# Alisah-Ozcan/HEonGPU

Measured on AMD Instinct MI355X. Metric: homomorphic mults/sec (CKKS N=2^16, L=16) + NTT GB/s vs HBM roofline, higher is better.
Workload: dtype u64

## Files before the change

### heongpu_amd/csrc/context.cpp

```cpp
#include "context.hpp"
#include <cerrno>
#include <climits>
#include <cstdlib>
#include "host_params.hpp"
#include <algorithm>
#include <cmath>
#include <cstdlib>
#include <cstring>
#include <stdexcept>

namespace hegpu {

using host::inv_mod_prime;
using host::mul_mod;

typedef std::vector<u64> vec;

static void append(vec& dst, const vec& src) { dst.insert(dst.end(), src.begin(), src.end()); }

void Context::build_host()
{
    n = ((u64) 1) << n_power;
    Qp_size = Q_size + P_size;
    const int Q = Q_size, P = P_size, Qp = Qp_size;
// ... 393 lines not shown
            host["plain_ntt_tables"] = host::power_table_bitrev(ppsi, t, n_power);
            host["plain_intt_tables"] = host::power_table_bitrev(inv_mod_prime(ppsi, t), t, n_power);
            host["n_plain_inverse"] = vec{inv_mod_prime(n % t, t)};
            vec loc;
            const u64 m = 2 * n;
            u64 pos = 1;
            auto brev = [&](u64 v) {
                u64 r = 0;
                for (int b = 0; b < n_power; b++) r |= ((v >> b) & 1) << (n_power - 1 - b);
                return r;
            };
            for (u64 i = 0; i < n / 2; i++) {
                loc.push_back(brev((pos - 1) >> 1));
                pos = (pos * 3) & (m - 1);
            }
            for (u64 i = n / 2; i < n; i++) {
                loc.push_back(brev((m - pos - 1) >> 1));
                pos = (pos * 3) & (m - 1);
            }
            host["encoding_location"] = loc;
        }

        {
            u64 Q_mod_t = 1;
            for (int i = 0; i < Q; i++) Q_mod_t = mul_mod(Q_mod_t, primes[i] % t, t);
            hv.Q_mod_t = Q_mod_t;
            hv.upper_threshold = (t + 1) >> 1;
            host["Q_mod_t"] = vec{hv.Q_mod_t};
            host["upper_threshold"] = vec{hv.upper_threshold};
            vec inc;
            for (int i = 0; i < Q; i++) inc.push_back(primes[i] - t);
            host["upper_halfincrement"] = inc;
            std::vector<u64> big{1};
            for (int i = 0; i < Q; i++) {
                unsigned __int128 carry = 0;
                for (u64& w : big) {
                    unsigned __int128 v = (unsigned __int128) w * primes[i] + carry;
                    w = (u64) v;
                    carry = v >> 64;
                }
                if (carry) big.push_back((u64) carry);
            }
            {
                unsigned __int128 rem = 0;
                for (size_t k = big.size(); k-- > 0;) {
                    unsigned __int128 cur = (rem << 64) | big[k];
                    big[k] = (u64) (cur / t);
                    rem = cur % t;
                }
            }
            vec cdiv;
            for (int i = 0; i < Q; i++) {
                unsigned __int128 rem = 0;
                for (size_t k = big.size(); k-- > 0;) rem = ((rem << 64) | big[k]) % primes[i];
                cdiv.push_back((u64) rem);
            }
            host["coeff_div_plain_modulus"] = cdiv;
            vec Qi_t, Qi_gamma, Qi_inverse;
            for (int i = 0; i < Q; i++) {
                u64 a = 1, b = 1, c = 1;
                for (int j = 0; j < Q; j++)
                    if (j != i) {
                        a = mul_mod(a, primes[j] % t, t);
                        b = mul_mod(b, primes[j] % gamma, gamma);
                        c = mul_mod(c, inv_mod_prime(primes[j] % primes[i], primes[i]), primes[i]);
                    }
                Qi_t.push_back(a);
                Qi_gamma.push_back(b);
                Qi_inverse.push_back(c);
            }
            host["Qi_t"] = Qi_t;
            host["Qi_gamma"] = Qi_gamma;
            host["Qi_inverse"] = Qi_inverse;
            u64 mt_ = 1, mg_ = 1;
            for (int i = 0; i < Q; i++) {
                mt_ = mul_mod(mt_, inv_mod_prime(primes[i] % t, t), t);
                mg_ = mul_mod(mg_, inv_mod_prime(primes[i] % gamma, gamma), gamma);
            }
            hv.mulq_inv_t = t - mt_;
            hv.mulq_inv_gamma = gamma - mg_;
            hv.inv_gamma = inv_mod_prime(gamma % t, t);
            host["mulq_inv_t"] = vec{hv.mulq_inv_t};
            host["mulq_inv_gamma"] = vec{hv.mulq_inv_gamma};
            host["inv_gamma"] = vec{hv.inv_gamma};
        }
    }
}

template <typename T>
static hipError_t to_device(const std::vector<T>& h, T** d)
{
    *d = nullptr;
    if (h.empty()) return hipSuccess;
    hipError_t e = hipMalloc((void**) d, h.size() * sizeof(T));
    if (e != hipSuccess) return e;
    return hipMemcpy(*d, h.data(), h.size() * sizeof(T), hipMemcpyHostToDevice);
}

static hipError_t build_plan(NttPlan& p, const vec& mods, const vec& fwd, const vec& inv, const vec& ninv,
                             int n_power, bool fp_on)
{
    const u64 n = ((u64) 1) << n_power;
    const int cnt = (int) mods.size();
    std::vector<Mod> hm(cnt);
    std::vector<ulonglong2> htw((size_t) cnt * n), hitw((size_t) cnt * n), hn(cnt), hw(cnt);
    const u64 rows = n / 256, perB = rows * 15 * 16;
    std::vector<ulonglong2> htwB((size_t) cnt * perB), hitwB((size_t) cnt * perB);
    std::vector<double> htwB8((size_t) cnt * perB, 0.0);
    for (int k = 0; k < cnt; k++) {
        const u64 q = mods[k];
        hm[k] = make_mod(q);
        static_assert(FP_MAX_MODULUS_BITS == 50, "the bounds in fpmod.cuh, ntt.hip and tests/fp_model.py are derived for q < 2^50");
        hm[k].fp = (fp_on && hm[k].bit <= FP_MAX_MODULUS_BITS && (q >> FP_MAX_MODULUS_BITS) == 0) ? 1 : 0;
        for (u64 j = 0; j < n; j++) {
            const u64 w = fwd[k * n + j], iw = inv[k * n + j];
            if (hm[k].fp) {
                const double wd = (double) w, wi = wd / (double) q;
                u64 a, b;
                memcpy(&a, &wd, 8);
                memcpy(&b, &wi, 8);
                htw[k * n + j] = make_ulonglong2(a, b);
            } else {
                htw[k * n + j] = make_ulonglong2(w, shoup_companion(w, q));
            }
            if (hm[k].fp) {
                const double wd = (double) iw, wi = wd / (double) q;
                u64 a, b;
                memcpy(&a, &wd, 8);
                memcpy(&b, &wi, 8);
                hitw[k * n + j] = make_ulonglong2(a, b);
            } else {
                hitw[k * n + j] = make_ulonglong2(iw, shoup_companion(iw, q));
            }
        }
        for (u64 c = 0; c < rows; c++)
            for (int st = 0; st < 4; st++)
                for (int b = 0; b < (1 << st); b++)
                    for (int j = 0; j < 16; j++) {
                        const u64 src = ((((rows + c) * 16 + j) << st) + b);
                        const u64 dst = k * perB + (c * 15 + ((1 << st) - 1 + b)) * 16 + j;
                        htwB[dst] = htw[k * n + src];
                        hitwB[dst] = hitw[k * n + src];
                        if (hm[k].fp) htwB8[dst] = (double) fwd[k * n + src];
                    }
        const u64 w1n = host::mul_mod(inv[k * n + 1], ninv[k], q);
        if (hm[k].fp) {
            auto pair = [&](u64 v) {
                const double vd = (double) v, vi = vd / (double) q;
                u64 a, b;
                memcpy(&a, &vd, 8);
                memcpy(&b, &vi, 8);
                return make_ulonglong2(a, b);
            };
            hn[k] = pair(ninv[k]);
            hw[k] = pair(w1n);
        } else {
            hn[k] = make_ulonglong2(ninv[k], shoup_companion(ninv[k], q));
            hw[k] = make_ulonglong2(w1n, shoup_companion(w1n, q));
        }
    }
    p.count = cnt;
    p.has_fp = p.has_int = 0;
    for (int k = 0; k < cnt; k++) (hm[k].fp ? p.has_fp : p.has_int) = 1;
    p.fp.assign(cnt, 0);
    for (int k = 0; k < cnt; k++) p.fp[k] = hm[k].fp ? 1 : 0;
    p.bits.assign(cnt, 0);
    for (int k = 0; k < cnt; k++) p.bits[k] = (unsigned char) hm[k].bit;
    u64 qmax = 0;
    for (int k = 0; k < cnt; k++) qmax = mods[k] > qmax ? mods[k] : qmax;
    p.lazy_q_max = (~0ull - 2 * qmax) / (4ull * (u64) n_power);
    hipError_t e;
    if ((e = to_device(hm, &p.mods)) != hipSuccess) return e;
    if ((e = to_device(htw, &p.tw)) != hipSuccess) return e;
    if ((e = to_device(hitw, &p.itw)) != hipSuccess) return e;
    if ((e = to_device(htwB, &p.twB)) != hipSuccess) return e;
    if ((e = to_device(hitwB, &p.itwB)) != hipSuccess) return e;
    if ((e = to_device(htwB8, &p.twB8)) != hipSuccess) return e;
    if ((e = to_device(hn, &p.ninv)) != hipSuccess) return e;
    return to_device(hw, &p.w1ninv);
}

static void free_plan(NttPlan& p)
{
    if (p.mods) (void) hipFree(p.mods);
    if (p.tw) (void) hipFree(p.tw);
    if (p.itw) (void) hipFree(p.itw);
    if (p.twB) (void) hipFree(p.twB);
    if (p.itwB) (void) hipFree(p.itwB);
    if (p.twB8) (void) hipFree(p.twB8);
    if (p.ninv) (void) hipFree(p.ninv);
    if (p.w1ninv) (void) hipFree(p.w1ninv);
    p = NttPlan();
}

hipError_t Context::upload()
{
    if (uploaded) return hipSuccess;
    for (int k = 0; k < DRBG_GAUSS_MAX; k++)
        gauss_cdt.t[k] = (u64) (erf(((double) k + 0.5) / (3.2 * 1.4142135623730951)) * 9223372036854775808.0);
    hipError_t e = hipGetDevice(&device);
    if (e != hipSuccess) return e;
    if ((e = build_plan(plan_qp, host["modulus"], host["ntt_table"], host["intt_table"], host["n_inverse"],
                        n_power, fp_ntt)) != hipSuccess)
        return e;
    const struct { const char* name; const u64** slot; const int** ints; } rows[] = {
        {"psi_half", &tab.psi_half}, {"last_q_modinv", &tab.last_q_modinv}, {"half", &tab.half},
        {"half_mod", &tab.half_mod}, {"factor", &tab.factor},
        {"m2_md_W0", &tab.m2_md_W0}, {"m2_md_G", &tab.m2_md_G}, {"m2_md_C", &tab.m2_md_C},
        {"rescaled_last_q_modinv", &tab.rescaled_last_q_modinv}, {"rescaled_half_mod", &tab.rescaled_half_mod},
        {"rescaled_half", &tab.rescaled_half}, {"mod_raise_half_mod", &tab.mod_raise_half_mod},
        {"base_change_matrix_Bsk", &behz.base_change_matrix_Bsk},
        {"inv_punctured_prod_mod_base_array", &behz.inv_punctured_prod_mod_base_array},
        {"base_change_matrix_m_tilde", &behz.base_change_matrix_m_tilde},
        {"inv_m_tilde_mod_Bsk", &behz.inv_m_tilde_mod_Bsk}, {"prod_q_mod_Bsk", &behz.prod_q_mod_Bsk},
        {"inv_prod_q_mod_Bsk", &behz.inv_prod_q_mod_Bsk}, {"base_change_matrix_q", &behz.base_change_matrix_q},
        {"base_change_matrix_msk", &behz.base_change_matrix_msk},
        {"inv_punctured_prod_mod_B_array", &behz.inv_punctured_prod_mod_B_array},
        {"behz_mtilde_inv_punct", &behz.mtilde_inv_punct}, {"behz_t_inv_punct", &behz.t_inv_punct},
        {"behz_invq_inv_punct_B", &behz.invq_inv_punct_B}, {"behz_msk_mod_q", &behz.msk_mod_q},
        {"behz_fc_matrix", &behz.fc_matrix}, {"behz_fc_c1", &behz.fc_c1}, {"behz_ff_matrix", &behz.ff_matrix},
        {"behz_ff_tc", &behz.ff_tc}, {"behz_ff_q_matrix", &behz.ff_q_matrix},
        {"behz_ff_msk_matrix", &behz.ff_msk_matrix}, {"behz_ff_prod_B", &behz.ff_prod_B},
        {"behz_ff_neg_prod_B", &behz.ff_neg_prod_B}, {"prod_B_mod_q", &behz.prod_B_mod_q},
        {"Mi", &tab.Mi}, {"Mi_inv", &tab.Mi_inv}, {"upper_half_threshold", &tab.upper_half_threshold},
        {"decryption_modulus", &tab.decryption_modulus}, {"special_fft_roots_table", &tab.special_fft_roots_table},
        {"special_ifft_roots_table", &tab.special_ifft_roots_table},
        {"coeff_div_plain_modulus", &tab.coeff_div_plain_modulus}, {"upper_halfincrement", &tab.upper_halfincrement},
        {"Qi_t", &tab.Qi_t}, {"Qi_gamma", &tab.Qi_gamma}, {"Qi_inverse", &tab.Qi_inverse},
        {"m2_Mi_inv", &tab.m2_Mi_inv}, {"m2_matrix", &tab.m2_matrix}, {"m2_prod", &tab.m2_prod},
        {"m2_matrix_mg", &tab.m2_matrix_mg}, {"m2_negprod_mg", &tab.m2_negprod_mg},
        {"new_prime_locations", nullptr, &tab.new_prime_locations},
        {"new_input_locations", nullptr, &tab.new_input_locations}, {"m2_I_j", nullptr, &tab.m2_I_j},
        {"m2_I_location", nullptr, &tab.m2_I_location}, {"encoding_location", nullptr, &tab.encoding_location},
        {"reverse_order", nullptr, &tab.reverse_order}, {"mpc_refresh_order", nullptr, &tab.mpc_refresh_order},
    };
    for (const auto& r : rows) {
        auto it = host.find(r.name);
        if (it == host.end()) continue;
        if (r.slot) {
            u64* d = nullptr;
            if ((e = to_device(it->second, &d)) != hipSuccess) return e;
            dev[r.name] = d;
            *r.slot = d;
        } else {
            std::vector<int> v(it->second.begin(), it->second.end());
            int* d = nullptr;
            if ((e = to_device(v, &d)) != hipSuccess) return e;
            dev[r.name] = d;
            *r.ints = d;
        }
    }
    if (scheme == SCHEME_BFV) {
        if ((e = build_plan(plan_merge, host["q_Bsk_merge_modulus"], host["q_Bsk_merge_ntt_tables"],
                            host["q_Bsk_merge_intt_tables"], host["q_Bsk_n_inverse"], n_power, fp_ntt)) != hipSuccess)
            return e;
        if (host.count("plain_modulus2") &&
            (e = build_plan(plan_plain, host["plain_modulus2"], host["plain_ntt_tables"], host["plain_intt_tables"],
                            host["n_plain_inverse"], n_power, fp_ntt)) != hipSuccess)
            return e;
        behz.ibase = plan_merge.mods;
        behz.obase = plan_merge.mods + Q_size;
        behz.m_tilde = make_mod(((u64) 1) << 32);
        behz.plain = make_mod(plain_modulus);
        behz.inv_prod_q_mod_m_tilde = hv.inv_prod_q_mod_m_tilde;
        behz.inv_prod_B_mod_m_sk = hv.inv_prod_B_mod_m_sk;
        behz.ibase_size = Q_size;
        behz.obase_size = bsk_size;
        behz.split = behz_split;
    }
    uploaded = true;
    return hipDeviceSynchronize();
}

namespace {
struct OptDesc {
    enum Rule { PLAIN, NOT_1_OR_3, BEFORE_UPLOAD, MIRROR_BEHZ };
    const char* name;
    const char* env;
    int lo, hi;
    int ContextHost::*i;
    bool ContextHost::*b;
    Rule rule;
    constexpr OptDesc(const char* nm, const char* ev, int l, int h, int ContextHost::*m, Rule r = PLAIN)
        : name(nm), env(ev), lo(l), hi(h), i(m), b(nullptr), rule(r) {}
    constexpr OptDesc(const char* nm, const char* ev, bool ContextHost::*m, Rule r = PLAIN)
        : name(nm), env(ev), lo(0), hi(1), i(nullptr), b(m), rule(r) {}
};
typedef ContextHost H;
const OptDesc kOptions[] = {
    {"fused_row_mac", "HEGPU_FUSED_ROW_MAC", -1, 1, &H::fused_row_mac},
    {"fused_moddown", "HEGPU_FUSED_MODDOWN", &H::fused_moddown},
    {"col_multi", "HEGPU_COL_MULTI", -1, 1, &H::col_multi},
    {"single_pass", "HEGPU_SINGLE_PASS", -1, 1, &H::single_pass},
    {"ntt_galois", "HEGPU_NTT_GALOIS", &H::ntt_galois},
    {"galois_scatter", "HEGPU_GALOIS_SCATTER", &H::galois_scatter},
    {"fuse_inverse", "HEGPU_FUSE_INVERSE", &H::fuse_inverse},
    {"copy_along", "HEGPU_COPY_ALONG", &H::copy_along},
    {"digit_split", "HEGPU_DIGIT_SPLIT", -1, 4, &H::digit_split, OptDesc::NOT_1_OR_3},
    {"fp_ntt", "HEGPU_FP_NTT", &H::fp_ntt, OptDesc::BEFORE_UPLOAD},
    {"behz_split", "HEGPU_BEHZ_SPLIT", -1, 1, &H::behz_split, OptDesc::MIRROR_BEHZ},
    {"fused_tensor", "HEGPU_FUSED_TENSOR", &H::fused_tensor},
    {"moddown_in_mac", "HEGPU_MODDOWN_IN_MAC", &H::moddown_in_mac},
    {"wide_access", "HEGPU_WIDE_ACCESS", &H::wide_access},
};
const OptDesc* find_option(const char* name)
{
    for (const OptDesc& o : kOptions)
        if (name && !strcmp(o.name, name)) return &o;
    return nullptr;
}
}

int Context::set_option(const char* name, int value)
{
    const OptDesc* d = find_option(name);
    if (!d) return 1;
    if (value < d->lo || value > d->hi || (d->rule == OptDesc::NOT_1_OR_3 && (value == 1 || value == 3))) return 2;
    if (d->rule == OptDesc::BEFORE_UPLOAD && uploaded) return 3;
    if (d->i) this->*d->i = value;
    else this->*d->b = value != 0;
    if (d->rule == OptDesc::MIRROR_BEHZ) behz.split = value;
    return 0;
}

int Context::get_option(const char* name, int* value) const
{
    const OptDesc* d = find_option(name);
    if (!d || !value) return 1;
    *value = d->i ? this->*d->i : (int) (this->*d->b);
    return 0;
}

bool env_long(const char* name, long* out)
{
    const char* e = getenv(name);
    if (!e || !*e) return false;
    char* end = nullptr;
    errno = 0;
    const long v = strtol(e, &end, 10);
    if (errno || end == e || *end) return false;
    *out = v;
    return true;
}

void Context::seed_options_from_env()
{
    for (const OptDesc& o : kOptions) {
        long v;
        if (env_long(o.env, &v) && v >= INT_MIN && v <= INT_MAX)
            (void) set_option(o.name, (int) v);
    }
}

void Context::release_device()
{
    free_plan(plan_qp);
    free_plan(plan_merge);
    free_plan(plan_plain);
    for (auto& kv : dev)
        if (kv.second) (void) hipFree(kv.second);
    dev.clear();
    uploaded = false;
}

Context::~Context()
{
    if (uploaded) release_device();
}

NttArgs Context::ntt_args(int table_set) const
{
    const NttPlan& p = table_set == 2 ? plan_plain : (table_set ? plan_merge : plan_qp);
    NttArgs a{};
    a.mods = p.mods;
    a.tw = p.tw;
    a.itw = p.itw;
    a.twB = p.twB;
    a.itwB = p.itwB;
    a.twB8 = p.twB8;
    a.ninv = p.ninv;
    a.w1ninv = p.w1ninv;
    a.n_power = n_power;
    a.mod_count = p.count;
    a.col_multi = col_multi;
    a.single_pass = single_pass;
    a.plan_has_fp = p.has_fp;
    a.plan_has_int = p.has_int;
    a.lazy_q_max = p.lazy_q_max;
    return a;
}

ModDown Context::moddown(int depth, bool rescale) const
{
    const int l = Q_size - depth;
    if (!rescale)
        return {plan_qp.mods, tab.half, tab.half_mod, tab.last_q_modinv, n_power, Qp_size - depth, l, Qp_size, Q_size,
                P_size};
    const int row = triangle_offset(Q_size - 1, depth);
    return {plan_qp.mods, tab.rescaled_half + depth, tab.rescaled_half_mod + row, tab.rescaled_last_q_modinv + row,
            n_power, l, l - 1, l, l - 1, 1};
}

}
```

### heongpu_amd/csrc/context.hpp

```cpp
#pragma once
#include "modarith.cuh"
#include "ntt.hpp"
#include "rns.hpp"
#include <map>
#include <string>
#include "drbg.hpp"
#include <vector>

namespace hegpu {

bool env_long(const char* name, long* out);


enum Scheme { SCHEME_BFV = 1, SCHEME_CKKS = 2 };

inline int triangle_offset(int first, int depth)
{
    int location = 0;
    for (int i = 0; i < depth; i++) location += first - i;
    return location;
}

struct NttPlan {
    Mod* mods = nullptr;
    ulonglong2* tw = nullptr;
    ulonglong2* itw = nullptr;
    ulonglong2* twB = nullptr;
    ulonglong2* itwB = nullptr;
    double* twB8 = nullptr;
    ulonglong2* ninv = nullptr;
    ulonglong2* w1ninv = nullptr;
    int count = 0;
    int has_fp = 0, has_int = 0;
    std::vector<unsigned char> fp;
    std::vector<unsigned char> bits;
    u64 lazy_q_max = 0;
};

struct DevTables {
    const u64 *psi_half, *last_q_modinv, *half, *half_mod, *factor;
    const u64 *m2_md_W0, *m2_md_G, *m2_md_C, *m2_Mi_inv, *m2_matrix, *m2_prod, *m2_matrix_mg, *m2_negprod_mg;
    const int *m2_I_j, *m2_I_location;
    const u64 *rescaled_last_q_modinv, *rescaled_half_mod, *rescaled_half;
    const u64* mod_raise_half_mod;
    const u64 *Mi, *Mi_inv, *upper_half_threshold, *decryption_modulus, *special_fft_roots_table, *special_ifft_roots_table;
    const int *new_prime_locations, *new_input_locations, *reverse_order, *mpc_refresh_order;
    const u64 *coeff_div_plain_modulus, *upper_halfincrement, *Qi_t, *Qi_gamma, *Qi_inverse;
    const int* encoding_location;
};

struct ContextHost {
    int scheme = 0;
    int n_power = 0;
    u64 n = 0;
    int Q_size = 0, P_size = 0, Qp_size = 0;
    int bsk_size = 0;
    u64 plain_modulus = 0;
    std::vector<u64> primes;
    std::map<std::string, std::vector<u64>> host;
    struct HostVals {
        u64 half = 0;
        std::vector<u64> rescaled_half;
        u64 mod_raise_half = 0;
        std::vector<u64> new_prime_locations;
        u64 Q_mod_t = 0, upper_threshold = 0, gamma = 0, mulq_inv_t = 0, mulq_inv_gamma = 0, inv_gamma = 0;
        u64 inv_prod_q_mod_m_tilde = 0, inv_prod_B_mod_m_sk = 0;
    } hv;
    struct M2Level {
        int d = 0, rc = 0;
        int off_digits = 0;
        int off_mi = 0;
        int off_matrix = 0;
        int off_prod = 0;
    };
    std::vector<M2Level> m2_levels;
    int m2_width = 0;
    int fused_row_mac = -1;
    bool fused_moddown = true;
    int col_multi = -1;
    int single_pass = -1;
    bool ntt_galois = true;
    bool galois_scatter = true;
    int digit_split = -1;
    bool copy_along = true;
    bool fuse_inverse = true;
    bool moddown_in_mac = true;
    bool wide_access = true;
    bool fused_tensor = true;
    bool fp_ntt = true;
    int behz_split = -1;
};

struct Context : ContextHost {
    void seed_options_from_env();
    int set_option(const char* name, int value);
    int get_option(const char* name, int* value) const;
    GaussCdt gauss_cdt{};

    bool uploaded = false;
    int device = -1;
    NttPlan plan_qp;
    NttPlan plan_merge;
    NttPlan plan_plain;
    std::map<std::string, void*> dev;
    DevTables tab{};
    BehzDev behz{};

    ~Context();
    void build_host();
    hipError_t upload();
    void release_device();

    NttArgs ntt_args(int table_set) const;
    ModDown moddown(int depth, bool rescale = false) const;
};

}
```

### heongpu_amd/csrc/ntt.hip

```cpp
#include "ntt.hpp"
#include <atomic>
#define HEGPU_FP_TU ntt
#include "fpmod.cuh"

namespace hegpu {

#define NTT_THREADS 256

#ifdef NTT_ABLATION_HEADER
#include NTT_ABLATION_HEADER
#else
__device__ __forceinline__ u64 gld(const u64* p) { return *p; }
__device__ __forceinline__ void gst(u64* p, u64 v) { *p = v; }
#define NTT_ABLATE_BFLY(x, y, w)
#define NTT_ABLATE_FPBFLY(x, y, w)
#define NTT_ABLATE_TW(load, root0, s) (load)
#define NTT_FP_TW(t, i, c) ((t)[i])
#endif

__device__ __forceinline__ u64 csub(u64 x, u64 m) { return (x >= m) ? x - m : x; }

typedef unsigned long long u64x2_t __attribute__((ext_vector_type(2)));
struct ConstTw {
    const u64x2_t __attribute__((address_space(4)))* p;
// ... 81 lines not shown
    return FpSched{m, b > b_out_max};
}
template <int LOGR, typename TW>
__device__ __forceinline__ void fp_ct_radix(double (&x)[1 << LOGR], TW tw, u32 root0,
                                            const FC& c, unsigned before, bool at_end)
{
#pragma unroll
    for (int s = 0; s < LOGR; s++) {
        FP_STAGE(c, 31 - __builtin_clz(root0) + s);
        if ((before >> s) & 1u) {
#pragma unroll
            for (int k = 0; k < (1 << LOGR); k++) x[k] = fp_reduce(x[k], c);
        }
        const int half = (1 << LOGR) >> (s + 1);
#pragma unroll
        for (int b = 0; b < (1 << s); b++) {
            const ulonglong2 w = NTT_ABLATE_TW(NTT_FP_TW(tw, (root0 << s) + b, c), root0, s);
#pragma unroll
            for (int j = 0; j < half; j++) fp_ct_bfly(x[b * 2 * half + j], x[b * 2 * half + j + half], w, c);
        }
    }
    FP_STAGE(c, 31 - __builtin_clz(root0) + LOGR);
    if (at_end) {
#pragma unroll
        for (int k = 0; k < (1 << LOGR); k++) x[k] = fp_reduce(x[k], c);
    }
}
template <int S1> struct FpColSched {
    static constexpr FpSched s = fp_sched(S1, FP_UNREDUCED_IN, FP_HANDOVER);
    static constexpr unsigned a_before = s.before & ((1u << (S1 - 4)) - 1u);
    static constexpr unsigned b_before = (s.before >> (S1 - 4)) & 15u;
    static constexpr bool b_at_end = s.at_end;
};
__device__ __forceinline__ void fp_ct_radix16_tb(double (&x)[16], const ulonglong2* __restrict__ tb, const FC& c)
{
#pragma unroll
    for (int s = 0; s < 4; s++) {
        const int half = 8 >> s;
        if (s > 0) FP_STAGE(c, (c).stage + 1);
#pragma unroll
        for (int b = 0; b < (1 << s); b++) {
            const ulonglong2 w = NTT_ABLATE_TW(NTT_FP_TW(tb, ((1 << s) - 1 + b) * 16, c), (u32) b, s);
#pragma unroll
            for (int j = 0; j < half; j++) fp_ct_bfly(x[b * 2 * half + j], x[b * 2 * half + j + half], w, c);
        }
    }
    FP_STAGE(c, (c).stage + 1);
#pragma unroll
    for (int k = 0; k < 16; k++) x[k] = fp_canon(x[k], c);
}

__device__ __forceinline__ void fp_ct_radix16_tb8(double (&x)[16], const double* __restrict__ tb, const FC& c)
{
#pragma unroll
    for (int s = 0; s < 4; s++) {
        const int half = 8 >> s;
        if (s > 0) __builtin_amdgcn_sched_barrier(0);
        if (s > 0) FP_STAGE(c, (c).stage + 1);
#pragma unroll
        for (int b = 0; b < (1 << s); b++) {
            const double wd = tb[((1 << s) - 1 + b) * 16];
            const ulonglong2 w = make_ulonglong2(as_bits(wd), as_bits(wd * c.qi));
#pragma unroll
            for (int j = 0; j < half; j++) fp_ct_bfly(x[b * 2 * half + j], x[b * 2 * half + j + half], w, c);
        }
    }
    FP_STAGE(c, (c).stage + 1);
#pragma unroll
    for (int k = 0; k < 16; k++) x[k] = fp_canon(x[k], c);
}

struct QC {
    u64 q;
    u64 q4;
    u32 nq0, nq1;
};
__device__ __forceinline__ QC make_qc(u64 q)
{
    QC c;
    c.q = q;
    c.q4 = 4 * q;
    u64 nq = 0 - q;
    c.nq0 = (u32) nq;
    c.nq1 = (u32) (nq >> 32);
    return c;
}

__device__ __forceinline__ u64 shoup_lazy(u64 y, ulonglong2 w, const QC& c)
{
    const u32 y0 = (u32) y, y1 = (u32) (y >> 32);
    const u32 w0 = (u32) w.x, w1 = (u32) (w.x >> 32), p0 = (u32) w.y, p1 = (u32) (w.y >> 32);
    const u64 A = (u64) y0 * p1;
    const u64 B = (u64) y1 * p0 + (u32) A;
    const u64 qh = (u64) y1 * p1 + (A >> 32) + (B >> 32);
    const u32 h0 = (u32) qh, h1 = (u32) (qh >> 32);
    u64 acc = (u64) y0 * w0;
    acc += (u64) h0 * c.nq0;
    const u32 hi = y0 * w1 + y1 * w0 + h0 * c.nq1 + h1 * c.nq0;
    return acc + ((u64) hi << 32);
}

__device__ __forceinline__ u64 shoup_full(u64 y, ulonglong2 w, const QC& c)
{
    u64 r = shoup_lazy(y, w, c);
    r = csub(r, 2 * c.q);
    return csub(r, c.q);
}

struct CsSched { unsigned c8, c4; };
__host__ __device__ constexpr CsSched cs_sched(int stages, int room, int exit_b = 8)
{
    CsSched r{0u, 0u};
    int b = 8;
    for (int s = 0; s < stages; s++) {
        const int need = (s == stages - 1 && exit_b < room) ? exit_b - 4 : room - 4;
        if (b > need && b > 8) {
            r.c8 |= 1u << s;
            b = 8;
        }
        if (b > need) {
            r.c4 |= 1u << s;
            b = 4;
        }
        b += 4;
    }
    return r;
}
static_assert(cs_sched(8, 8).c8 == 0u && cs_sched(8, 8).c4 == 0xFFu, "61-bit moduli: a correction in every stage");
static_assert(cs_sched(8, 16).c8 == 0xD4u && cs_sched(8, 16).c4 == 0x80u, "60-bit moduli: stages 2, 4, 6, 7 / 7");
static_assert(cs_sched(5, 16).c8 == 0x14u && cs_sched(5, 16).c4 == 0x10u, "N = 2^13 column pass: stages 2, 4 / 4");
static_assert(cs_sched(8, 16, 12).c8 == 0xD4u && cs_sched(8, 16, 12).c4 == 0u, "60-bit digit, exit 12 q: stages 2, 4, 6, 7 / none");
static_assert(cs_sched(8, 16, 16).c8 == 0x54u && cs_sched(8, 16, 16).c4 == 0u, "60-bit digit, exit 16 q: stages 2, 4, 6 / none");
static_assert(cs_sched(8, 8, 8).c8 == 0u && cs_sched(8, 8, 8).c4 == 0xFFu, "61-bit digit: the schedule has no slack, only the chain goes");
__device__ __forceinline__ void ct_bfly_cs(u64& x, u64& y, ulonglong2 w, const QC& c, int cs)
{
    NTT_ABLATE_BFLY(x, y, w);
    u64 u = x;
    if (cs & 2) u = csub(u, 2 * c.q4);
    if (cs & 1) u = csub(u, c.q4);
    u64 t = shoup_lazy(y, w, c);
    x = u + t;
    y = u + c.q4 - t;
}
#define NTT_CS_EVERY 0xFFFFFFFFu

__device__ __forceinline__ void gs_bfly(u64& x, u64& y, ulonglong2 w, const QC& c)
{
    NTT_ABLATE_BFLY(x, y, w);
    u64 s = x + y;
    u64 d = x + c.q4 - y;
    x = csub(s, c.q4);
    y = shoup_lazy(d, w, c);
}

template <int LOGR, bool LAZY, unsigned C8 = 0u, unsigned C4 = NTT_CS_EVERY, typename TW>
__device__ __forceinline__ void ct_radix(u64 (&x)[1 << LOGR], TW tw,
                                         u32 root0, const QC& c)
{
#pragma unroll
    for (int s = 0; s < LOGR; s++) {
        const int half = (1 << LOGR) >> (s + 1);
        const int cs = LAZY ? 0 : (int) (((C8 >> s) & 1u) * 2u + ((C4 >> s) & 1u));
#pragma unroll
        for (int b = 0; b < (1 << s); b++) {
            ulonglong2 w = NTT_ABLATE_TW(tw[(root0 << s) + b], root0, s);
#pragma unroll
            for (int j = 0; j < half; j++)
                ct_bfly_cs(x[b * 2 * half + j], x[b * 2 * half + j + half], w, c, cs);
        }
    }
}

template <bool LAZY, unsigned C8 = 0u, unsigned C4 = NTT_CS_EVERY>
__device__ __forceinline__ void ct_radix16_tb(u64 (&x)[16], const ulonglong2* __restrict__ tb, const QC& c)
{
#pragma unroll
    for (int s = 0; s < 4; s++) {
        const int half = 8 >> s;
        const int cs = LAZY ? 0 : (int) (((C8 >> s) & 1u) * 2u + ((C4 >> s) & 1u));
#pragma unroll
        for (int b = 0; b < (1 << s); b++) {
            ulonglong2 w = tb[((1 << s) - 1 + b) * 16];
#pragma unroll
            for (int j = 0; j < half; j++)
                ct_bfly_cs(x[b * 2 * half + j], x[b * 2 * half + j + half], w, c, cs);
        }
    }
}

template <int LOGR>
__device__ __forceinline__ void gs_radix(u64 (&x)[1 << LOGR], const ulonglong2* __restrict__ tw,
                                         u32 root0, const QC& c)
{
#pragma unroll
    for (int s = LOGR - 1; s >= 0; s--) {
        const int half = (1 << LOGR) >> (s + 1);
#pragma unroll
        for (int b = 0; b < (1 << s); b++) {
            ulonglong2 w = NTT_ABLATE_TW(tw[(root0 << s) + b], root0, s);
#pragma unroll
            for (int j = 0; j < half; j++)
                gs_bfly(x[b * 2 * half + j], x[b * 2 * half + j + half], w, c);
        }
    }
}

__device__ __forceinline__ void gs_radix16_tb(u64 (&x)[16], const ulonglong2* __restrict__ tb, const QC& c)
{
#pragma unroll
    for (int s = 3; s >= 0; s--) {
        const int half = 8 >> s;
#pragma unroll
        for (int b = 0; b < (1 << s); b++) {
            ulonglong2 w = tb[((1 << s) - 1 + b) * 16];
#pragma unroll
            for (int j = 0; j < half; j++)
                gs_bfly(x[b * 2 * half + j], x[b * 2 * half + j + half], w, c);
        }
    }
}

template <int LOGR>
__device__ __forceinline__ void gs_radix_last(u64 (&x)[1 << LOGR], const ulonglong2* __restrict__ tw,
                                              u32 root0, ulonglong2 ninv, ulonglong2 w1ninv, const QC& c)
{
#pragma unroll
    for (int s = LOGR - 1; s >= 1; s--) {
        const int half = (1 << LOGR) >> (s + 1);
#pragma unroll
        for (int b = 0; b < (1 << s); b++) {
            ulonglong2 w = NTT_ABLATE_TW(tw[(root0 << s) + b], root0, s);
#pragma unroll
            for (int j = 0; j < half; j++)
                gs_bfly(x[b * 2 * half + j], x[b * 2 * half + j + half], w, c);
        }
    }
    const int half = (1 << LOGR) >> 1;
#pragma unroll
    for (int j = 0; j < half; j++) {
        u64 s = x[j] + x[j + half];
        u64 d = x[j] + c.q4 - x[j + half];
        x[j] = shoup_full(s, ninv, c);
        x[j + half] = shoup_full(d, w1ninv, c);
    }
}

struct PolySel {
    u64 in_off, out_off;
    int mod;
    int digit;
    int item, j;
};

__device__ __forceinline__ int udiv16(int x, unsigned magic)
{
    return magic ? (int) __umulhi((unsigned) x, magic) : x;
}

__device__ __forceinline__ PolySel select_poly(const NttArgs& a, int poly)
{
    PolySel s;
    if (a.group_span) {
        const int k = udiv16(poly, a.mg_group_span), r = poly - k * a.group_span;
        if (a.polys_per_item) {
            const int per_item = udiv16(a.polys_per_item, a.mg_mod_count);
            const int it = udiv16(r, a.mg_per_item), d = r - it * per_item;
            poly = it * a.polys_per_item + d * a.mod_count + k;
        } else {
            poly = r * a.mod_count + k;
        }
    }
    int item = 0, j = poly;
    if (a.polys_per_item) {
        item = udiv16(poly, a.mg_polys_per_item);
        j = poly - item * a.polys_per_item;
    }
    int k = j - udiv16(j, a.mg_mod_count) * a.mod_count;
    if (a.mod_order) k = a.mod_order[k];
    s.mod = a.mod_offset + k;
    u64 slot = a.poly_order ? (u64) a.poly_order[j] : (u64) j;
    s.digit = a.decomp_mods ? udiv16(j, a.mg_decomp_mods) : -1;
    u64 in_slot = a.decomp_mods ? (u64) s.digit * (a.decomp_in_mul ? a.decomp_in_mul : 1) + a.decomp_in_add : slot;
    if (a.decomp_out_mul) slot = (u64) s.digit * a.decomp_out_mul + (u64) (j - s.digit * a.decomp_mods);
    s.in_off = (u64) item * a.in_item_stride + (in_slot << a.n_power);
    s.out_off = (u64) item * a.out_item_stride + (slot << a.n_power);
    s.item = item;
    s.j = j;
    return s;
}

__device__ __forceinline__ int col_phys(int e) { return e ^ (((e >> 8) & 1) << 4); }
__device__ __forceinline__ int row_phys(int e) { return e ^ (((e >> 5) & 7) << 1); }

__device__ __forceinline__ void wave_lds_fence()
{
    __builtin_amdgcn_fence(__ATOMIC_RELEASE, "wavefront");
    __builtin_amdgcn_wave_barrier();
    __builtin_amdgcn_fence(__ATOMIC_ACQUIRE, "wavefront");
}

#define COL_LDS_ELEMS 4096
#define ROW_LDS_ELEMS 4096

__device__ __forceinline__ bool fwd_stages_lazy(const Mod& md, u64 lazy_q_max) { return md.q <= lazy_q_max; }
#define NTT_ROW_LAZY_MAX_Q 0x0666666666666666ull
__device__ __forceinline__ bool row_stages_lazy(const Mod& md, u64 lazy_q_max) { return md.q <= lazy_q_max || md.q <= NTT_ROW_LAZY_MAX_Q; }
__device__ __forceinline__ bool stages_room16(const Mod& md) { return md.bit <= 60; }

template <int S1, bool DECOMP, bool LAZY, bool SREG = false, int ROOM = 8>
__device__ __forceinline__ void fwd_col_body(const NttArgs& a, const PolySel& ps, const Mod& md, u64* lds,
                                             const u64* sreg = nullptr, ulonglong2* twl = nullptr)
{
    constexpr CsSched CS = cs_sched(S1, ROOM);
    constexpr int R = 1 << S1;
    constexpr int CT = 4096 / R;
    constexpr int NSA = S1 - 4;
    constexpr int RA = 1 << NSA;
    constexpr int G = 16 / RA;
    int t = threadIdx.x;
    if constexpr (SREG) asm volatile("" : "+v"(t));
    const QC qc = make_qc(md.q);
    const ulonglong2* __restrict__ tw = a.tw + ((u64) ps.mod << a.n_power);
    const u64* __restrict__ src = a.in + ps.in_off + blockIdx.x * CT;
    u64* __restrict__ dst = a.out + ps.out_off + blockIdx.x * CT;

    const u64 half_qP = (a.half_on && !SREG) ? a.mods[a.half_src_mod].q : 0;
    const u64 half_hm = a.half_on ? (SREG ? ld_const_u64(a.half_mod + ps.mod) : a.half_mod[ps.mod]) : 0;
    auto digit_q = [&]() { return SREG ? ld_const_u64(&a.mods[ps.digit].q) : a.mods[ps.digit].q; };
    u64 x[16];
    const int col = t % CT, r1 = t / CT;
    u64 v[16];
    if constexpr (NSA > 0) {
#pragma unroll
        for (int g = 0; g < G; g++) {
            const int L = t + NTT_THREADS * g;
            const int c = L % CT, rb = L / CT;
#pragma unroll
            for (int k = 0; k < RA; k++) v[g * RA + k] = SREG ? sreg[g * RA + k] : gld(&src[(u64) (rb + 16 * k) * 256 + c]);
        }
    } else {
#pragma unroll
        for (int k = 0; k < 16; k++) v[k] = SREG ? sreg[k] : gld(&src[(u64) k * 256 + col]);
    }
    if (DECOMP && a.half_on) {
#pragma unroll
        for (int k = 0; k < 16; k++) v[k] = sub_mod(reduce64(SREG ? v[k] : add_mod(v[k], a.half, half_qP), md), half_hm, md.q);
    } else if (DECOMP && !LAZY && digit_q() > 8 * md.q) {
#pragma unroll
        for (int k = 0; k < 16; k++) v[k] = reduce64(v[k], md);
    }
    if constexpr (NSA > 0) {
        ulonglong2 mine;
        if constexpr (SREG) mine = tw[t];
#pragma unroll
        for (int g = 0; g < G; g++) {
            const int L = t + NTT_THREADS * g;
            const int c = L % CT, rb = L / CT;
            u64 y[RA];
#pragma unroll
            for (int k = 0; k < RA; k++) y[k] = v[g * RA + k];
            if constexpr (SREG) ct_radix<NSA, LAZY, CS.c8, CS.c4>(y, const_tw(tw), 1u, qc);
            else ct_radix<NSA, LAZY, CS.c8, CS.c4>(y, tw, 1u, qc);
#pragma unroll
            for (int k = 0; k < RA; k++) lds[col_phys((rb + 16 * k) * CT + c)] = y[k];
        }
        if constexpr (SREG) twl[t] = mine;
        __syncthreads();
#pragma unroll
        for (int k = 0; k < 16; k++) x[k] = lds[col_phys((16 * r1 + k) * CT + col)];
        if (SREG) __syncthreads();
    } else {
#pragma unroll
        for (int k = 0; k < 16; k++) x[k] = v[k];
    }
    if constexpr (SREG && NSA > 0) ct_radix<4, LAZY, (CS.c8 >> NSA), (CS.c4 >> NSA)>(x, twl, (u32) (RA + r1), qc);
    else ct_radix<4, LAZY, (CS.c8 >> NSA), (CS.c4 >> NSA)>(x, tw, (u32) (RA + r1), qc);
#pragma unroll
    for (int k = 0; k < 16; k++) gst(&dst[(u64) (16 * r1 + k) * 256 + col], x[k]);
}

template <int S1, bool DECOMP, bool WIDE, bool SREG = false>
__device__ __forceinline__ void fwd_col_body_fp(const NttArgs& a, const PolySel& ps, const Mod& md, u64* lds,
                                                ulonglong2* twl, const u64* sreg = nullptr)
{
    constexpr int R = 1 << S1;
    constexpr int CT = 4096 / R;
    constexpr int NSA = S1 - 4;
    constexpr int RA = 1 << NSA;
    constexpr int G = 16 / RA;
    const int t = threadIdx.x;
    const FC fc = make_fc(md.q, FP_SITE(DECOMP ? FPS_FWD_COL_DECOMP : FPS_FWD_COL, S1 - 4));
    const ulonglong2* __restrict__ tw = a.tw + ((u64) ps.mod << a.n_power);
    const u64* __restrict__ src = a.in + ps.in_off + blockIdx.x * CT;
    u64* __restrict__ dst = a.out + ps.out_off + blockIdx.x * CT;

    double c32 = 0.0, c32i = 0.0;
    if constexpr (DECOMP && WIDE) {
        c32 = (double) reduce64(1ull << 32, md);
        c32i = c32 * fc.qi;
    }
    const u64 half_qP = (DECOMP && a.half_on && !SREG) ? a.mods[a.half_src_mod].q : 0;
    const double half_hm =
        (DECOMP && a.half_on) ? fp_from_u64(SREG ? ld_const_u64(a.half_mod + ps.mod) : a.half_mod[ps.mod]) : 0.0;
    auto digit_q = [&]() { return SREG ? ld_const_u64(&a.mods[ps.digit].q) : a.mods[ps.digit].q; };
    const bool in_small = S1 != 7 && DECOMP && !WIDE && !a.half_on && digit_q() <= md.q + (md.q >> 6);
    typedef FpColSched<S1> CS;
    auto load_all = [&](auto& y, auto addr, int si0) {
        constexpr int CNT = sizeof(y) / sizeof(y[0]);
        FP_STAGE(fc, FP_STAGE_INPUT);
        if constexpr (SREG && !WIDE) {
            if (in_small) {
#pragma unroll
                for (int k = 0; k < CNT; k++) y[k] = as_f64(sreg[si0 + k]);
            } else {
#pragma unroll
                for (int k = 0; k < CNT; k++) y[k] = fp_reduce(as_f64(sreg[si0 + k]), fc);
            }
        } else {
            u64 v[CNT];
#pragma unroll
            for (int k = 0; k < CNT; k++) {
                v[k] = SREG ? sreg[si0 + k] : *addr(k);
                if constexpr (SREG) asm volatile("" : "+v"(v[k]));
            }
            if (!SREG && DECOMP && a.half_on) {
#pragma unroll
                for (int k = 0; k < CNT; k++) v[k] = add_mod(v[k], a.half, half_qP);
            }
#pragma unroll
            for (int k = 0; k < CNT; k++) {
                if constexpr (DECOMP && WIDE) y[k] = fp_mul(fp_from_u32((u32) (v[k] >> 32)), c32, c32i, fc) + fp_from_u32((u32) v[k]);
                else if constexpr (DECOMP) y[k] = in_small ? fp_from_u64(v[k]) : fp_reduce(fp_from_u64(v[k]), fc);
                else y[k] = fp_from_u64(v[k]);
            }
        }
        if (DECOMP && a.half_on) {
#pragma unroll
            for (int k = 0; k < CNT; k++) y[k] = fp_reduce(y[k] - half_hm, fc);
        }
#pragma unroll
        for (int k = 0; k < CNT; k++) FP_AUDIT_VAL(fc, FPM_SUM, y[k]);
    };

    double x[16];
    const int col = t % CT, r1 = t / CT;
    if constexpr (NSA > 0) {
        const ulonglong2 mine = tw[t];
#pragma unroll
        for (int g = 0; g < G; g++) {
            const int L = t + NTT_THREADS * g;
            const int c = L % CT, rb = L / CT;
            double y[RA];
            load_all(y, [&](int k) { return &src[(u64) (rb + 16 * k) * 256 + c]; }, g * RA);
            if constexpr (SREG) fp_ct_radix<NSA>(y, const_tw(tw), 1u, fc, CS::a_before, false);
            else fp_ct_radix<NSA>(y, tw, 1u, fc, CS::a_before, false);
#pragma unroll
            for (int k = 0; k < RA; k++) lds[col_phys((rb + 16 * k) * CT + c)] = as_bits(y[k]);
        }
        twl[t] = mine;
        __syncthreads();
#pragma unroll
        for (int k = 0; k < 16; k++) x[k] = as_f64(lds[col_phys((16 * r1 + k) * CT + col)]);
        if (SREG) __syncthreads();
        fp_ct_radix<4>(x, twl, (u32) (RA + r1), fc, CS::b_before, CS::b_at_end);
    } else {
        load_all(x, [&](int k) { return &src[(u64) k * 256 + col]; }, 0);
        fp_ct_radix<4>(x, tw, (u32) (RA + r1), fc, CS::b_before, CS::b_at_end);
    }
#pragma unroll
    for (int k = 0; k < 16; k++) {
        if constexpr (SREG) __builtin_nontemporal_store(as_bits(x[k]), &dst[(u64) (16 * r1 + k) * 256 + col]);
        else dst[(u64) (16 * r1 + k) * 256 + col] = as_bits(x[k]);
    }
}

template <int S1, bool DECOMP>
__global__ __launch_bounds__(NTT_THREADS) void ntt_fwd_col(NttArgs a)
{
    __shared__ u64 lds[(S1 > 4) ? COL_LDS_ELEMS : 1];
    __shared__ ulonglong2 twl[(S1 > 4) ? 256 : 1];
    int poly = blockIdx.y;
    if (DECOMP && a.only_int && a.int_slot_count > 0) {
        const int cnt = a.int_slot_count, digits = a.polys_per_item / a.decomp_mods;
        const int per_item = digits * cnt;
        const int item = poly / per_item, r = poly - item * per_item;
        const int digit = r / cnt, w = r - digit * cnt;
        poly = item * a.polys_per_item + digit * a.decomp_mods + a.int_slots[w];
    }
    const PolySel ps = select_poly(a, poly);
    if (DECOMP && a.skip_identity && ps.mod == ps.digit) return;
    const Mod md = a.mods[ps.mod];
    if (DECOMP && a.only_int && md.fp) return;
    if (DECOMP && a.copy_src) {
        constexpr int CT = 4096 >> S1;
        const int t = threadIdx.x, col = t % CT, r1 = t / CT;
        const u64 limb = ((u64) (ps.digit * a.copy_part_limbs + (ps.j - ps.digit * a.decomp_mods)) << a.n_power) +
                         blockIdx.x * CT;
        const u64* __restrict__ cs = a.copy_src + (u64) ps.item * a.copy_src_item_stride + limb;
        u64* __restrict__ cd = a.copy_dst + (u64) ps.item * a.copy_dst_item_stride + limb;
        u64 c[16];
#pragma unroll
        for (int k = 0; k < 16; k++) c[k] = cs[(u64) (16 * r1 + k) * 256 + col];
#pragma unroll
        for (int k = 0; k < 16; k++) cd[(u64) (16 * r1 + k) * 256 + col] = c[k];
    }
    if (md.fp) {
        if (DECOMP && a.mods[a.half_on ? a.half_src_mod : ps.digit].bit > 52)
            fwd_col_body_fp<S1, DECOMP, true>(a, ps, md, lds, twl);
        else fwd_col_body_fp<S1, DECOMP, false>(a, ps, md, lds, twl);
    } else if (fwd_stages_lazy(md, a.lazy_q_max)) fwd_col_body<S1, DECOMP, true>(a, ps, md, lds);
    else if (S1 > 4 && stages_room16(md)) fwd_col_body<S1, DECOMP, false, false, (S1 > 4 ? 16 : 8)>(a, ps, md, lds);
    else fwd_col_body<S1, DECOMP, false>(a, ps, md, lds);
}

__device__ __forceinline__ void row_store_all(const NttArgs& a, const PolySel& ps, const Mod& md, u64* __restrict__ p,
                                              u64 e0, const u64* lds, int row, int i0)
{
    if (!a.epi.on) {
#pragma unroll
        for (int k = 0; k < 16; k++) gst(&p[e0 + 16 * k], lds[row_phys(row * 256 + i0 + 16 * k)]);
        return;
    }
    const NttEpilogue& ep = a.epi;
    const int part = udiv16(ps.j, ep.mg_limbs), limb = ps.j - part * ep.limbs;
    const u64* __restrict__ ks = ep.ks + ep.ks_item_stride * ps.item + ((u64) (part * ep.ks_part_limbs + limb) << a.n_power) + e0;
    const u64 off = ((u64) (part * ep.limbs + limb) << a.n_power);
    const bool with_ct = ep.ct && (!ep.ct_parts || part < ep.ct_parts);
    const u64* ct = with_ct ? ep.ct + ep.ct_item_stride * ps.item + off + e0 : nullptr;
    u64* out = ep.out + ep.out_item_stride * ps.item + off;
    const u64 inv = ep.inv[ps.mod];
#pragma unroll
    for (int h = 0; h < 2; h++) {
        u64 kv[8], cv[8];
#pragma unroll
        for (int k = 0; k < 8; k++) kv[k] = ks[16 * (8 * h + k)];
        if (with_ct) {
#pragma unroll
            for (int k = 0; k < 8; k++) cv[k] = ct[16 * (8 * h + k)];
        }
        u64 r[8];
#pragma unroll
        for (int k = 0; k < 8; k++)
            r[k] = mul_barrett(sub_mod(kv[k], lds[row_phys(row * 256 + i0 + 16 * (8 * h + k))], md.q), inv, md);
        if (with_ct) {
#pragma unroll
            for (int k = 0; k < 8; k++) r[k] = add_mod(cv[k], r[k], md.q);
        }
        if (ep.galois_inv) {
#pragma unroll
            for (int k = 0; k < 8; k++) {
                const u32 e = (u32) e0 + 16 * (8 * h + k);
                const u32 ex = ((2u * (__brev(e) >> (32 - a.n_power)) + 1u) * ep.galois_inv) & ((2u << a.n_power) - 1u);
                out[__brev((ex - 1u) >> 1) >> (32 - a.n_power)] = r[k];
            }
        } else {
#pragma unroll
            for (int k = 0; k < 8; k++) out[e0 + 16 * (8 * h + k)] = r[k];
        }
    }
}

template <bool LAZY, int ROOM = 8>
__device__ __forceinline__ void fwd_row_body(const NttArgs& a, const PolySel& ps, const Mod& md, u64* lds)
{
    constexpr CsSched CS = cs_sched(8, ROOM);
    const int t = threadIdx.x;
    const QC qc = make_qc(md.q);
    const int s1 = a.n_power - 8;
    const ulonglong2* __restrict__ tw = a.tw + ((u64) ps.mod << a.n_power);
    u64* __restrict__ p = a.out + ps.out_off + (u64) blockIdx.x * 4096;

    const int row = t >> 4, i0 = t & 15;
    const u32 crow = blockIdx.x * 16 + row;
    u64 x[16];
#pragma unroll
    for (int k = 0; k < 16; k++) x[k] = gld(&p[row * 256 + i0 + 16 * k]);
    ct_radix<4, LAZY, CS.c8, CS.c4>(x, tw, (1u << s1) + crow, qc);
#pragma unroll
    for (int k = 0; k < 16; k++) lds[row_phys(row * 256 + i0 + 16 * k)] = x[k];
    wave_lds_fence();
#pragma unroll
    for (int k = 0; k < 8; k++) {
        ulonglong2 v = *reinterpret_cast<const ulonglong2*>(&lds[row_phys(row * 256 + 16 * i0 + 2 * k)]);
        x[2 * k] = v.x;
        x[2 * k + 1] = v.y;
    }
    ct_radix16_tb<LAZY, (CS.c8 >> 4), (CS.c4 >> 4)>(x, a.twB + ((u64) ps.mod * (15u << (a.n_power - 4))) + ((u64) crow * 15 * 16 + i0), qc);
    if (LAZY) {
#pragma unroll
        for (int k = 0; k < 16; k++) x[k] = reduce64(x[k], md);
    } else {
#pragma unroll
        for (int k = 0; k < 16; k++) x[k] = csub(csub(csub(x[k], qc.q4), 2 * qc.q), qc.q);
    }
    wave_lds_fence();
#pragma unroll
    for (int k = 0; k < 8; k++)
        *reinterpret_cast<ulonglong2*>(&lds[row_phys(row * 256 + 16 * i0 + 2 * k)]) =
            make_ulonglong2(x[2 * k], x[2 * k + 1]);
    wave_lds_fence();
    row_store_all(a, ps, md, a.out + ps.out_off, (u64) blockIdx.x * 4096 + row * 256 + i0, lds, row, i0);
}

__device__ __forceinline__ void fwd_row_body_fp(const NttArgs& a, const PolySel& ps, const Mod& md, u64* lds)
{
    const int t = threadIdx.x;
    const FC fc = make_fc(md.q, FP_SITE(FPS_FWD_ROW, a.n_power - 12));
    const int s1 = a.n_power - 8;
    const ulonglong2* __restrict__ tw = a.tw + ((u64) ps.mod << a.n_power);
    u64* __restrict__ p = a.out + ps.out_off + (u64) blockIdx.x * 4096;

    const int row = t >> 4, i0 = t & 15;
    const u32 crow = blockIdx.x * 16 + row;
    double x[16];
#pragma unroll
    for (int k = 0; k < 16; k++) x[k] = as_f64(p[row * 256 + i0 + 16 * k]);
    fp_ct_radix<4>(x, tw, (1u << s1) + crow, fc, 0u, true);
#pragma unroll
    for (int k = 0; k < 16; k++) lds[row_phys(row * 256 + i0 + 16 * k)] = as_bits(x[k]);
    wave_lds_fence();
#pragma unroll
    for (int k = 0; k < 8; k++) {
        ulonglong2 v = *reinterpret_cast<const ulonglong2*>(&lds[row_phys(row * 256 + 16 * i0 + 2 * k)]);
        x[2 * k] = as_f64(v.x);
        x[2 * k + 1] = as_f64(v.y);
    }
    fp_ct_radix16_tb8(x, a.twB8 + ((u64) ps.mod * (15u << (a.n_power - 4))) + ((u64) crow * 15 * 16 + i0), fc);
    wave_lds_fence();
#pragma unroll
    for (int k = 0; k < 8; k++)
        *reinterpret_cast<ulonglong2*>(&lds[row_phys(row * 256 + 16 * i0 + 2 * k)]) =
            make_ulonglong2(fp_to_u64(x[2 * k]), fp_to_u64(x[2 * k + 1]));
    wave_lds_fence();
    row_store_all(a, ps, md, a.out + ps.out_off, (u64) blockIdx.x * 4096 + row * 256 + i0, lds, row, i0);
}

__global__ __launch_bounds__(NTT_THREADS) void ntt_fwd_row(NttArgs a)
{
    __shared__ __attribute__((aligned(16))) u64 lds[ROW_LDS_ELEMS];
    const PolySel ps = select_poly(a, blockIdx.y);
    if (a.skip_identity && ps.mod == ps.digit) return;
    const Mod md = a.mods[ps.mod];
    if (md.fp) fwd_row_body_fp(a, ps, md, lds);
    else if (row_stages_lazy(md, a.lazy_q_max)) fwd_row_body<true>(a, ps, md, lds);
    else if (stages_room16(md)) fwd_row_body<false, 16>(a, ps, md, lds);
    else fwd_row_body<false>(a, ps, md, lds);
}

template <int S1>
__device__ __forceinline__ int single_pos(int row, int col)
{
    return (row >> 4) * 4096 + row_phys((row & 15) * 256 + col);
}

template <int S1, bool FP, bool LAZY, bool DECOMP = false>
__device__ __forceinline__ void fwd_single_body(const NttArgs& a, const PolySel& ps, const Mod& md, u64* limb)
{
    constexpr int R = 1 << S1;
    constexpr int CT = 4096 / R;
    constexpr int NSA = S1 - 4;
    constexpr int RA = 1 << NSA;
    constexpr int G = 16 / RA;
    const int t = threadIdx.x, g = t >> 8, tt = t & 255;
    const QC qc = make_qc(md.q);
    const FC fc = make_fc(md.q, FP_SITE(FPS_FWD_SINGLE, S1 - 4));
    const ulonglong2* __restrict__ tw = a.tw + ((u64) ps.mod << a.n_power);
    const u64* __restrict__ src = a.in + ps.in_off + g * CT;
    const int col = tt % CT, r1 = tt / CT;
    u64 dv[DECOMP ? 16 : 1];
    double dy[(DECOMP && FP) ? 16 : 1];
    if constexpr (DECOMP) {
        if constexpr (NSA > 0) {
#pragma unroll
            for (int gi = 0; gi < G; gi++) {
                const int L = tt + 256 * gi;
                const int c = L % CT, rb = L / CT;
#pragma unroll
                for (int k = 0; k < RA; k++) dv[gi * RA + k] = src[(u64) (rb + 16 * k) * 256 + c];
            }
        } else {
#pragma unroll
            for (int k = 0; k < 16; k++) dv[k] = src[(u64) k * 256 + col];
        }
        const u64 half_qP = a.half_on ? a.mods[a.half_src_mod].q : 0;
        if constexpr (FP) {
            FP_STAGE(fc, FP_STAGE_INPUT);
            if (a.half_on) {
#pragma unroll
                for (int k = 0; k < 16; k++) dv[k] = add_mod(dv[k], a.half, half_qP);
            }
            if (a.mods[a.half_on ? a.half_src_mod : ps.digit].bit > 52) {
                const double c32 = (double) reduce64(1ull << 32, md), c32i = c32 * fc.qi;
#pragma unroll
                for (int k = 0; k < 16; k++)
                    dy[k] = fp_mul(fp_from_u32((u32) (dv[k] >> 32)), c32, c32i, fc) + fp_from_u32((u32) dv[k]);
            } else {
#pragma unroll
                for (int k = 0; k < 16; k++) dy[k] = fp_reduce(fp_from_u64(dv[k]), fc);
            }
            if (a.half_on) {
                const double half_hm = fp_from_u64(a.half_mod[ps.mod]);
#pragma unroll
                for (int k = 0; k < 16; k++) dy[k] = fp_reduce(dy[k] - half_hm, fc);
            }
#pragma unroll
            for (int k = 0; k < 16; k++) FP_AUDIT_VAL(fc, FPM_SUM, dy[k]);
        } else {
            if (a.half_on) {
                const u64 half_hm = a.half_mod[ps.mod];
#pragma unroll
                for (int k = 0; k < 16; k++) dv[k] = sub_mod(reduce64(add_mod(dv[k], a.half, half_qP), md), half_hm, md.q);
            } else if (!LAZY && a.mods[ps.digit].q > 8 * md.q) {
#pragma unroll
                for (int k = 0; k < 16; k++) dv[k] = reduce64(dv[k], md);
            }
        }
    }
    if constexpr (FP) {
        double x[16];
        if constexpr (NSA > 0) {
#pragma unroll
            for (int gi = 0; gi < G; gi++) {
                const int L = tt + 256 * gi;
                const int c = L % CT, rb = L / CT;
                double y[RA];
#pragma unroll
                for (int k = 0; k < RA; k++) {
                    if constexpr (DECOMP) y[k] = dy[gi * RA + k];
                    else y[k] = fp_from_u64(gld(&src[(u64) (rb + 16 * k) * 256 + c]));
                }
                fp_ct_radix<NSA>(y, tw, 1u, fc, FpColSched<S1>::a_before, false);
#pragma unroll
                for (int k = 0; k < RA; k++) limb[single_pos<S1>(rb + 16 * k, g * CT + c)] = as_bits(y[k]);
            }
            __syncthreads();
#pragma unroll
            for (int k = 0; k < 16; k++) x[k] = as_f64(limb[single_pos<S1>(16 * r1 + k, g * CT + col)]);
        } else {
#pragma unroll
            for (int k = 0; k < 16; k++) {
                if constexpr (DECOMP) x[k] = dy[k];
                else x[k] = fp_from_u64(src[(u64) k * 256 + col]);
            }
        }
        fp_ct_radix<4>(x, tw, (u32) (RA + r1), fc, FpColSched<S1>::b_before, FpColSched<S1>::b_at_end);
#pragma unroll
        for (int k = 0; k < 16; k++) limb[single_pos<S1>(16 * r1 + k, g * CT + col)] = as_bits(x[k]);
    } else {
        u64 x[16];
        if constexpr (NSA > 0) {
#pragma unroll
            for (int gi = 0; gi < G; gi++) {
                const int L = tt + 256 * gi;
                const int c = L % CT, rb = L / CT;
                u64 y[RA];
#pragma unroll
                for (int k = 0; k < RA; k++) {
                    if constexpr (DECOMP) y[k] = dv[gi * RA + k];
                    else y[k] = gld(&src[(u64) (rb + 16 * k) * 256 + c]);
                }
                ct_radix<NSA, LAZY>(y, tw, 1u, qc);
#pragma unroll
                for (int k = 0; k < RA; k++) limb[single_pos<S1>(rb + 16 * k, g * CT + c)] = y[k];
            }
            __syncthreads();
#pragma unroll
            for (int k = 0; k < 16; k++) x[k] = limb[single_pos<S1>(16 * r1 + k, g * CT + col)];
        } else {
#pragma unroll
            for (int k = 0; k < 16; k++) {
                if constexpr (DECOMP) x[k] = dv[k];
                else x[k] = src[(u64) k * 256 + col];
            }
        }
        ct_radix<4, LAZY>(x, tw, (u32) (RA + r1), qc);
#pragma unroll
        for (int k = 0; k < 16; k++) limb[single_pos<S1>(16 * r1 + k, g * CT + col)] = x[k];
    }
    __syncthreads();
    u64* lds = limb + g * 4096;
    const int row = tt >> 4, i0 = tt & 15;
    const u32 crow = g * 16 + row;
    const ulonglong2* __restrict__ tb = a.twB + ((u64) ps.mod * (15u << (a.n_power - 4))) + ((u64) crow * 15 * 16 + i0);
    u64 r[16];
    if constexpr (FP) {
        double x[16];
#pragma unroll
        for (int k = 0; k < 16; k++) x[k] = as_f64(lds[row_phys(row * 256 + i0 + 16 * k)]);
        fp_ct_radix<4>(x, tw, (1u << S1) + crow, fc, 0u, true);
#pragma unroll
        for (int k = 0; k < 16; k++) lds[row_phys(row * 256 + i0 + 16 * k)] = as_bits(x[k]);
        wave_lds_fence();
#pragma unroll
        for (int k = 0; k < 8; k++) {
            ulonglong2 v = *reinterpret_cast<const ulonglong2*>(&lds[row_phys(row * 256 + 16 * i0 + 2 * k)]);
            x[2 * k] = as_f64(v.x);
            x[2 * k + 1] = as_f64(v.y);
        }
        fp_ct_radix16_tb8(x, a.twB8 + ((u64) ps.mod * (15u << (a.n_power - 4))) + ((u64) crow * 15 * 16 + i0), fc);
#pragma unroll
        for (int k = 0; k < 16; k++) r[k] = fp_to_u64(x[k]);
    } else {
        u64 x[16];
#pragma unroll
        for (int k = 0; k < 16; k++) x[k] = lds[row_phys(row * 256 + i0 + 16 * k)];
        ct_radix<4, LAZY>(x, tw, (1u << S1) + crow, qc);
#pragma unroll
        for (int k = 0; k < 16; k++) lds[row_phys(row * 256 + i0 + 16 * k)] = x[k];
        wave_lds_fence();
#pragma unroll
        for (int k = 0; k < 8; k++) {
            ulonglong2 v = *reinterpret_cast<const ulonglong2*>(&lds[row_phys(row * 256 + 16 * i0 + 2 * k)]);
            x[2 * k] = v.x;
            x[2 * k + 1] = v.y;
        }
        ct_radix16_tb<LAZY>(x, tb, qc);
        if (LAZY) {
#pragma unroll
            for (int k = 0; k < 16; k++) r[k] = reduce64(x[k], md);
        } else {
#pragma unroll
            for (int k = 0; k < 16; k++) r[k] = csub(csub(csub(x[k], qc.q4), 2 * qc.q), qc.q);
        }
    }
    wave_lds_fence();
#pragma unroll
    for (int k = 0; k < 8; k++)
        *reinterpret_cast<ulonglong2*>(&lds[row_phys(row * 256 + 16 * i0 + 2 * k)]) = make_ulonglong2(r[2 * k], r[2 * k + 1]);
    wave_lds_fence();
    row_store_all(a, ps, md, a.out + ps.out_off, (u64) g * 4096 + row * 256 + i0, lds, row, i0);
}

template <int S1, bool DECOMP = false>
__global__ __launch_bounds__(16 << S1, 4) void ntt_fwd_single(NttArgs a)
{
    extern __shared__ __attribute__((aligned(16))) u64 limb[];
    const PolySel ps = select_poly(a, blockIdx.x);
    if (DECOMP && a.skip_identity && ps.mod == ps.digit) return;
    const Mod md = a.mods[ps.mod];
    if (md.fp) fwd_single_body<S1, true, false, DECOMP>(a, ps, md, limb);
    else if (fwd_stages_lazy(md, a.lazy_q_max)) fwd_single_body<S1, false, true, DECOMP>(a, ps, md, limb);
    else fwd_single_body<S1, false, false, DECOMP>(a, ps, md, limb);
}

static_assert(ks_unreduced_exit(16, 60) == 16 && ks_unreduced_exit(17, 60) == 12 && ks_unreduced_exit(21, 60) == 12, "");
static_assert(ks_unreduced_exit(22, 60) == 8 && ks_unreduced_exit(32, 60) == 8 && ks_unreduced_exit(33, 60) == 0, "");
static_assert(ks_unreduced_exit(4, 61) == 16 && ks_unreduced_exit(8, 61) == 8 && ks_unreduced_exit(9, 61) == 0, "");

template <bool PAIR> __device__ __forceinline__ int ks_own0(int i0) { return PAIR ? 2 * i0 : i0; }
template <bool PAIR> __device__ __forceinline__ constexpr int ks_own(int k) { return PAIR ? 32 * (k >> 1) + (k & 1) : 16 * k; }
template <bool PAIR, bool NT = false>
__device__ __forceinline__ void ks_ld16(u64 (&v)[16], const u64* p)
{
    if constexpr (PAIR) {
#pragma unroll
        for (int m = 0; m < 8; m++) {
            const u64x2_t* q = reinterpret_cast<const u64x2_t*>(p + 32 * m);
            const u64x2_t w = NT ? __builtin_nontemporal_load(q) : *q;
            v[2 * m] = w.x;
            v[2 * m + 1] = w.y;
        }
    } else {
#pragma unroll
        for (int k = 0; k < 16; k++) v[k] = NT ? __builtin_nontemporal_load(&p[16 * k]) : p[16 * k];
    }
}
template <bool PAIR, bool NT = false>
__device__ __forceinline__ void ks_st16(u64* p, const u64 (&v)[16])
{
    if constexpr (PAIR) {
#pragma unroll
        for (int m = 0; m < 8; m++) {
            u64x2_t w;
            w.x = v[2 * m];
            w.y = v[2 * m + 1];
            u64x2_t* q = reinterpret_cast<u64x2_t*>(p + 32 * m);
            if constexpr (NT) __builtin_nontemporal_store(w, q);
            else *q = w;
        }
    } else {
#pragma unroll
        for (int k = 0; k < 16; k++) {
            if constexpr (NT) __builtin_nontemporal_store(v[k], &p[16 * k]);
            else p[16 * k] = v[k];
        }
    }
}
template <bool PAIR>
__device__ __forceinline__ void ks_own_read(u64 (&v)[16], const u64* lds, int row, int i0)
{
    if constexpr (PAIR) {
        int b = row * 256 + 2 * i0;
        asm volatile("" : "+v"(b));
#pragma unroll
        for (int m = 0; m < 8; m++) {
            const ulonglong2 w = *reinterpret_cast<const ulonglong2*>(&lds[(b ^ (2 * m)) + 32 * m]);
            v[2 * m] = w.x;
            v[2 * m + 1] = w.y;
        }
    } else {
#pragma unroll
        for (int k = 0; k < 16; k++) v[k] = lds[row_phys(row * 256 + i0 + 16 * k)];
    }
}

template <bool LAZY, int ROOM = 8, int EXIT = 0, bool PAIR = false>
__device__ __forceinline__ void ks_row_digit(u64 (&x)[16], const u64* __restrict__ p, u64* lds,
                                             const ulonglong2* twa, const ulonglong2* __restrict__ tb,
                                             const QC& qc, const Mod& md, int row, int i0)
{
    static_assert(EXIT == 0 || (!LAZY && (EXIT == 8 || ((EXIT == 12 || EXIT == 16) && ROOM == 16))), "exit bound");
    constexpr CsSched CS = cs_sched(8, ROOM, EXIT ? EXIT : 8);
#pragma unroll
    for (int k = 0; k < 16; k++) x[k] = gld(&p[row * 256 + i0 + 16 * k]);
#pragma unroll
    for (int s = 0; s < 4; s++) {
        const int half = 8 >> s;
        const int cs = LAZY ? 0 : (int) (((CS.c8 >> s) & 1u) * 2u + ((CS.c4 >> s) & 1u));
#pragma unroll
        for (int b = 0; b < (1 << s); b++) {
            const ulonglong2 w = twa[((1 << s) - 1 + b) * 16 + row];
#pragma unroll
            for (int j = 0; j < half; j++) ct_bfly_cs(x[b * 2 * half + j], x[b * 2 * half + j + half], w, qc, cs);
        }
    }
#pragma unroll
    for (int k = 0; k < 16; k++) lds[row_phys(row * 256 + i0 + 16 * k)] = x[k];
    wave_lds_fence();
#pragma unroll
    for (int k = 0; k < 8; k++) {
        ulonglong2 v = *reinterpret_cast<const ulonglong2*>(&lds[row_phys(row * 256 + 16 * i0 + 2 * k)]);
        x[2 * k] = v.x;
        x[2 * k + 1] = v.y;
    }
    ct_radix16_tb<LAZY, (CS.c8 >> 4), (CS.c4 >> 4)>(x, tb, qc);
    if (!LAZY && EXIT == 0) {
#pragma unroll
        for (int k = 0; k < 16; k++) x[k] = csub(csub(csub(x[k], qc.q4), 2 * qc.q), qc.q);
    }
    wave_lds_fence();
#pragma unroll
    for (int k = 0; k < 8; k++)
        *reinterpret_cast<ulonglong2*>(&lds[row_phys(row * 256 + 16 * i0 + 2 * k)]) =
            make_ulonglong2(x[2 * k], x[2 * k + 1]);
    wave_lds_fence();
    ks_own_read<PAIR>(x, lds, row, i0);
    wave_lds_fence();
}

struct KsIdx { int item, tile, slot; bool valid; int d0, d1; };
__host__ __device__ __forceinline__ unsigned ks_slots(const KsMacArgs& a, int kind)
{
    const int all = a.slot_count ? a.slot_count : a.rc;
    if (a.int_slot_count <= 0 || kind == 0) return (unsigned) all;
    return kind == 1 ? (unsigned) a.int_slot_count : (unsigned) (all - a.int_slot_count);
}
template <bool SPLIT, int KIND = 0>
__device__ __forceinline__ KsIdx ks_index(const KsMacArgs& a)
{
    const unsigned b = blockIdx.x, xcd = b & 7u, j = b >> 3;
    const unsigned splits = SPLIT ? (unsigned) a.splits : 1u;
    const unsigned units = (unsigned) a.items * splits;
    const unsigned tiles = 1u << (a.n_power - 12);
    const unsigned total = ks_slots(a, KIND) * tiles * units, chunk = (total + 7u) >> 3;
    const unsigned lin = xcd * chunk + j;
    const unsigned g = lin / units, unit = lin - g * units;
    const unsigned item = SPLIT ? unit / splits : unit, sp = SPLIT ? unit - item * splits : 0u;
    const unsigned nslots = ks_slots(a, KIND), gt = g / nslots;
    KsIdx r;
    r.valid = lin < total;
    r.item = (int) item;
    r.tile = (int) gt;
    int si = (int) (g - gt * nslots);
    if (KIND == 1 && a.int_slot_count > 0) {
        si = a.int_slots[r.valid ? si : 0];
    } else {
        si += a.slot_first;
        if (KIND == 2 && a.int_slot_count > 0) {
#pragma unroll
            for (int q = 0; q < 8; q++)
                if (q < a.int_slot_count && a.int_slots[q] <= si) si++;
        }
    }
    r.slot = si;
    r.d0 = SPLIT ? (int) (sp * (unsigned) a.digits / splits) : 0;
    r.d1 = SPLIT ? (int) ((sp + 1) * (unsigned) a.digits / splits) : a.digits;
    return r;
}

template <bool PAIR = false>
__device__ __forceinline__ void ks_tail_scatter(const KsMacArgs& a, int item, int slot, int p, u64 e0, const u64 (&r)[16])
{
    const KsMacArgs::Tail& e = a.tail;
    u64* out = e.out + e.out_item_stride * item + ((u64) (p * e.limbs + slot) << a.n_power);
    if (e.galois_inv) {
#pragma unroll
        for (int k = 0; k < 16; k++) {
            const u32 el = (u32) e0 + ks_own<PAIR>(k);
            const u32 ex = ((2u * (__brev(el) >> (32 - a.n_power)) + 1u) * e.galois_inv) & ((2u << a.n_power) - 1u);
            out[__brev((ex - 1u) >> 1) >> (32 - a.n_power)] = r[k];
        }
    } else {
        ks_st16<PAIR>(out + e0, r);
    }
}
template <bool PAIR = false>
__device__ __forceinline__ void ks_tail_store(const KsMacArgs& a, int item, int slot, int p, u64 e0, const Mod& md, u64 inv,
                                              const u64 (&acc)[16], const u64 (&tv)[16], bool with_ct, const u64 (&cv)[16])
{
    u64 r[16];
#pragma unroll
    for (int k = 0; k < 16; k++) r[k] = mul_barrett(sub_mod(acc[k], tv[k], md.q), inv, md);
    if (with_ct) {
#pragma unroll
        for (int k = 0; k < 16; k++) r[k] = add_mod(cv[k], r[k], md.q);
    }
    ks_tail_scatter<PAIR>(a, item, slot, p, e0, r);
}
template <bool PAIR = false>
__device__ __forceinline__ void ks_tail_store_fp(const KsMacArgs& a, int item, int slot, int p, u64 e0, const FC& fc, double inv,
                                                 const double (&acc)[16], const double (&tv)[16], bool with_ct,
                                                 const u64 (&cv)[16])
{
    double m[16];
#pragma unroll
    for (int k = 0; k < 16; k++) {
        FP_STAGE(fc, FP_STAGE_OUT);
        const double d = fp_reduce(acc[k], fc) - tv[k];
        FP_STAGE(fc, FP_STAGE_TAIL);
        FP_AUDIT_VAL(fc, FPM_SUM, d);
        m[k] = fp_mul_nc(d, inv, fc);
    }
    FP_STAGE(fc, FP_STAGE_OUT);
    if (with_ct) {
#pragma unroll
        for (int k = 0; k < 16; k++) m[k] += fp_from_u64(cv[k]);
    }
    u64 r[16];
#pragma unroll
    for (int k = 0; k < 16; k++) r[k] = fp_to_u64(fp_canon(m[k], fc));
    ks_tail_scatter<PAIR>(a, item, slot, p, e0, r);
}
__device__ __forceinline__ const u64* ks_tail_T(const KsMacArgs& a, int item, int slot, int tile, int p)
{
    return a.tail.T + a.tail.T_item_stride * item + ((u64) (p * a.rc + slot) << a.n_power) + (u64) tile * 4096;
}
template <bool PAIR = false>
__device__ __forceinline__ bool ks_tail_ct(const KsMacArgs& a, int item, int slot, int p, u64 e0, u64 (&cv)[16])
{
    const KsMacArgs::Tail& e = a.tail;
    if (!e.ct || (e.ct_parts && p >= e.ct_parts)) return false;
    const u64* c = e.ct + e.ct_item_stride * item + ((u64) (p * e.limbs + slot) << a.n_power) + e0;
    ks_ld16<PAIR>(cv, c);
    return true;
}

#define KS_TW_LDS_BYTES ((15 * 256 + 15 * 16) * 8)
template <bool SPLIT, bool MD = false, bool PAIR = false>
__device__ __forceinline__ void ks_row_mac_int_body(const KsMacArgs& a, const KsIdx& ki, const Mod& md, int midx,
                                                    u64* lds, void* twbuf)
{
    const int t = threadIdx.x;
    const int item = ki.item, tile = ki.tile, slot = ki.slot;
    const QC qc = make_qc(md.q);
    const int s1 = a.n_power - 8;
    const ulonglong2* __restrict__ tw = a.tw + ((u64) midx << a.n_power);
    const int row = t >> 4, i0 = t & 15;
    const u32 crow = tile * 16 + row;
    const ulonglong2* __restrict__ tb = a.twB + ((u64) midx * (15u << (a.n_power - 4))) + ((u64) crow * 15 * 16 + i0);
    const u64 n = (u64) 1 << a.n_power;
    const u64* __restrict__ pin = a.in + a.in_item_stride * item + ((u64) slot << a.n_power) + (u64) tile * 4096;
    const u64* __restrict__ pk = a.key + ((u64) midx << a.n_power) + (u64) tile * 4096 + row * 256 + ks_own0<PAIR>(i0);
    const u64 dig_off = (u64) a.rc << a.n_power;
    const u64 key_off1 = (u64) a.key_limbs << a.n_power, key_off2 = (u64) a.key_limbs << (a.n_power + 1);
    const bool lazy = row_stages_lazy(md, a.lazy_q_max) && md.q <= ~0ull / (u64) a.digits;
    const bool room16 = stages_room16(md);
    const int ex = a.unreduced_exit;
    ulonglong2* twa = reinterpret_cast<ulonglong2*>(twbuf);
    if (i0 < 15) {
        const int s = (i0 >= 7) ? 3 : (i0 >= 3) ? 2 : (i0 >= 1) ? 1 : 0;
        twa[i0 * 16 + row] = tw[((((u32) 1 << s1) + crow) << s) + (i0 - ((1 << s) - 1))];
    }
    wave_lds_fence();

    const int item_s = MD ? __builtin_amdgcn_readfirstlane(item) : 0, slot_s = MD ? __builtin_amdgcn_readfirstlane(slot) : 0;
    const int tile_s = MD ? __builtin_amdgcn_readfirstlane(tile) : 0, midx_s = MD ? __builtin_amdgcn_readfirstlane(midx) : 0;
    u64 h0[16], l0[16], h1[16], l1[16];
#pragma unroll
    for (int k = 0; k < 16; k++) h0[k] = l0[k] = h1[k] = l1[k] = 0;
    for (int i = ki.d0; i < ki.d1; i++) {
        u64 x[16];
        const u64* p = pin + dig_off * i;
        if (a.skip_identity && i == midx) {
            const u64* pi = a.ident + a.ident_item_stride * item + ((u64) i << a.n_power) + (u64) tile * 4096;
            if constexpr (PAIR) {
                ks_ld16<true>(x, pi + row * 256 + 2 * i0);
            } else {
#pragma unroll
                for (int k = 0; k < 16; k++) x[k] = gld(&pi[row * 256 + i0 + 16 * k]);
            }
        } else if (lazy) {
            ks_row_digit<true, 8, 0, PAIR>(x, p, lds, twa, tb, qc, md, row, i0);
        } else if (room16) {
            if (ex == 16) ks_row_digit<false, 16, 16, PAIR>(x, p, lds, twa, tb, qc, md, row, i0);
            else if (ex == 12) ks_row_digit<false, 16, 12, PAIR>(x, p, lds, twa, tb, qc, md, row, i0);
            else if (ex == 8) ks_row_digit<false, 16, 8, PAIR>(x, p, lds, twa, tb, qc, md, row, i0);
            else ks_row_digit<false, 16, 0, PAIR>(x, p, lds, twa, tb, qc, md, row, i0);
        } else {
            if (ex) ks_row_digit<false, 8, 8, PAIR>(x, p, lds, twa, tb, qc, md, row, i0);
            else ks_row_digit<false, 8, 0, PAIR>(x, p, lds, twa, tb, qc, md, row, i0);
        }
        const u64* k0 = pk + key_off2 * i;
        const u64* k1 = k0 + key_off1;
        if constexpr (PAIR) {
#pragma unroll
            for (int m = 0; m < 8; m++) {
                const ulonglong2 v0 = *reinterpret_cast<const ulonglong2*>(k0 + 32 * m);
                const ulonglong2 v1 = *reinterpret_cast<const ulonglong2*>(k1 + 32 * m);
                acc128(h0[2 * m], l0[2 * m], x[2 * m], v0.x);
                acc128(h1[2 * m], l1[2 * m], x[2 * m], v1.x);
                acc128(h0[2 * m + 1], l0[2 * m + 1], x[2 * m + 1], v0.y);
                acc128(h1[2 * m + 1], l1[2 * m + 1], x[2 * m + 1], v1.y);
            }
        } else {
#pragma unroll
            for (int k = 0; k < 16; k++) {
                acc128(h0[k], l0[k], x[k], k0[16 * k]);
                acc128(h1[k], l1[k], x[k], k1[16 * k]);
            }
        }
    }
    if constexpr (MD) {
        u64 acc0[16], acc1[16];
#pragma unroll
        for (int k = 0; k < 16; k++) {
            acc0[k] = reduce128(h0[k], l0[k], md);
            acc1[k] = reduce128(h1[k], l1[k], md);
        }
        int tt = threadIdx.x;
        asm volatile("" : "+v"(tt));
        const int trow = tt >> 4, ti0 = tt & 15;
        const u64 e0 = (u64) tile_s * 4096 + trow * 256 + ks_own0<PAIR>(ti0);
        const u64 inv = a.tail.inv[midx_s];
        const bool lazy_t = row_stages_lazy(md, a.lazy_q_max);
        const ulonglong2* __restrict__ ttb = a.twB + ((u64) midx_s * (15u << (a.n_power - 4))) + ((u64) (tile_s * 16 + trow) * 15 * 16 + ti0);
        auto part = [&](int p, const u64 (&acc)[16]) {
            u64 cv[16], x[16];
            const bool with_ct = ks_tail_ct<PAIR>(a, item_s, slot_s, p, e0, cv);
            const u64* pT = ks_tail_T(a, item_s, slot_s, tile_s, p);
            if (lazy_t) {
                ks_row_digit<true, 8, 0, PAIR>(x, pT, lds, twa, ttb, qc, md, trow, ti0);
#pragma unroll
                for (int k = 0; k < 16; k++) x[k] = reduce64(x[k], md);
            } else if (room16) {
                ks_row_digit<false, 16, 0, PAIR>(x, pT, lds, twa, ttb, qc, md, trow, ti0);
            } else {
                ks_row_digit<false, 8, 0, PAIR>(x, pT, lds, twa, ttb, qc, md, trow, ti0);
            }
            ks_tail_store<PAIR>(a, item_s, slot_s, p, e0, md, inv, acc, x, with_ct, cv);
        };
        __builtin_amdgcn_sched_barrier(0);
        part(0, acc0);
        __builtin_amdgcn_sched_barrier(0);
        part(1, acc1);
        return;
    }
    if constexpr (PAIR) {
        int tt = threadIdx.x;
        asm volatile("" : "+v"(tt));
        u64* pw = a.out + a.out_item_stride * item + ((u64) slot << a.n_power) + (u64) tile * 4096 + (tt >> 4) * 256 + 2 * (tt & 15);
#pragma unroll
        for (int m = 0; m < 8; m++) {
            *reinterpret_cast<ulonglong2*>(pw + 32 * m) =
                make_ulonglong2(reduce128(h0[2 * m], l0[2 * m], md), reduce128(h0[2 * m + 1], l0[2 * m + 1], md));
            *reinterpret_cast<ulonglong2*>(pw + dig_off + 32 * m) =
                make_ulonglong2(reduce128(h1[2 * m], l1[2 * m], md), reduce128(h1[2 * m + 1], l1[2 * m + 1], md));
        }
    } else {
        u64* po = (SPLIT ? const_cast<u64*>(pin) + dig_off * ki.d0 - (u64) tile * 4096
                         : a.out + a.out_item_stride * item + ((u64) slot << a.n_power)) +
                  (u64) tile * 4096 + row * 256 + i0;
#pragma unroll
        for (int k = 0; k < 16; k++) {
            po[16 * k] = reduce128(h0[k], l0[k], md);
            po[dig_off + 16 * k] = reduce128(h1[k], l1[k], md);
        }
    }
    (void) n;
}

template <bool SPLIT>
__global__ __launch_bounds__(NTT_THREADS, SPLIT ? 2 : 1) void ks_row_mac(KsMacArgs a)
{
    __shared__ __attribute__((aligned(16))) u64 lds[ROW_LDS_ELEMS];
    __shared__ ulonglong2 twa[15 * 16];
    const KsIdx ki = ks_index<SPLIT, SPLIT ? 0 : 1>(a);
    if (!ki.valid) return;
    const int midx = a.mod_order ? a.mod_order[ki.slot] : ki.slot;
    const Mod md = a.mods[midx];
    if (md.fp) return;
    ks_row_mac_int_body<SPLIT>(a, ki, md, midx, lds, twa);
}

template <bool SPLIT, bool PAIR = false>
__device__ __forceinline__ void ks_fp_row(double (&x)[16], const u64 (&xr)[16], const double* twl, u64* lds, const FC& fc,
                                          int s1, int row, int i0, int t)
{
    if constexpr (SPLIT) {
#pragma unroll
        for (int k = 0; k < 16; k++) x[k] = as_f64(xr[k]);
#pragma unroll
        for (int s = 0; s < 4; s++) {
            const int half = 8 >> s;
            FP_STAGE(fc, s1 + s);
#pragma unroll
            for (int b = 0; b < (1 << s); b++) {
                const double w = twl[15 * 256 + ((1 << s) - 1 + b) * 16 + row];
#pragma unroll
                for (int j = 0; j < half; j++) fp_ct_bfly(x[b * 2 * half + j], x[b * 2 * half + j + half], w, fc);
            }
        }
        FP_STAGE(fc, s1 + 4);
#pragma unroll
        for (int k = 0; k < 16; k++) x[k] = fp_reduce(x[k], fc);
#pragma unroll
        for (int k = 0; k < 16; k++) lds[row_phys(row * 256 + i0 + 16 * k)] = as_bits(x[k]);
        wave_lds_fence();
#pragma unroll
        for (int k = 0; k < 8; k++) {
            ulonglong2 v = *reinterpret_cast<const ulonglong2*>(&lds[row_phys(row * 256 + 16 * i0 + 2 * k)]);
            x[2 * k] = as_f64(v.x);
            x[2 * k + 1] = as_f64(v.y);
        }
#pragma unroll
        for (int s = 0; s < 4; s++) {
            const int half = 8 >> s;
            FP_STAGE(fc, s1 + 4 + s);
#pragma unroll
            for (int b = 0; b < (1 << s); b++) {
                const double w = twl[((1 << s) - 1 + b) * 256 + t];
#pragma unroll
                for (int j = 0; j < half; j++) fp_ct_bfly(x[b * 2 * half + j], x[b * 2 * half + j + half], w, fc);
            }
        }
    } else {
        int row_o = row, t_o = t;
        asm volatile("" : "+v"(row_o), "+v"(t_o));
        const double* twa = twl + 15 * 256 + row_o;
        const double* twb = twl + t_o;
        double wn[8], wc[8];
        wc[0] = twa[0];
        wn[0] = twa[16];
        wn[1] = twa[32];
        __builtin_amdgcn_sched_barrier(0);
#pragma unroll
        for (int k = 0; k < 16; k++) x[k] = as_f64(xr[k]);
#pragma unroll
        for (int s = 0; s < 4; s++) {
            const int half = 8 >> s;
            FP_STAGE(fc, s1 + s);
            if (s > 0) {
#pragma unroll
                for (int b = 0; b < (1 << s); b++) wc[b] = wn[b];
            }
            if (s < 3) {
                if (s > 0) {
#pragma unroll
                    for (int b = 0; b < (2 << s); b++) wn[b] = twa[((2 << s) - 1 + b) * 16];
                }
            } else {
                wn[0] = twb[0];
            }
            __builtin_amdgcn_sched_barrier(0);
#pragma unroll
            for (int b = 0; b < (1 << s); b++) {
                const double w = wc[b];
#pragma unroll
                for (int j = 0; j < half; j++) fp_ct_bfly(x[b * 2 * half + j], x[b * 2 * half + j + half], w, fc);
            }
        }
        FP_STAGE(fc, s1 + 4);
#pragma unroll
        for (int k = 0; k < 16; k++) x[k] = fp_reduce(x[k], fc);
#pragma unroll
        for (int k = 0; k < 16; k++) lds[row_phys(row * 256 + i0 + 16 * k)] = as_bits(x[k]);
        wave_lds_fence();
#pragma unroll
        for (int k = 0; k < 8; k++) {
            ulonglong2 v = *reinterpret_cast<const ulonglong2*>(&lds[row_phys(row * 256 + 16 * i0 + 2 * k)]);
            x[2 * k] = as_f64(v.x);
            x[2 * k + 1] = as_f64(v.y);
        }
#pragma unroll
        for (int s = 0; s < 4; s++) {
            const int half = 8 >> s;
            FP_STAGE(fc, s1 + 4 + s);
#pragma unroll
            for (int b = 0; b < (1 << s); b++) wc[b] = wn[b];
            if (s < 3) {
#pragma unroll
                for (int b = 0; b < (2 << s); b++) wn[b] = twb[((2 << s) - 1 + b) * 256];
            }
            __builtin_amdgcn_sched_barrier(0);
#pragma unroll
            for (int b = 0; b < (1 << s); b++) {
                const double w = wc[b];
#pragma unroll
                for (int j = 0; j < half; j++) fp_ct_bfly(x[b * 2 * half + j], x[b * 2 * half + j + half], w, fc);
            }
        }
    }
    wave_lds_fence();
#pragma unroll
    for (int k = 0; k < 8; k++)
        *reinterpret_cast<ulonglong2*>(&lds[row_phys(row * 256 + 16 * i0 + 2 * k)]) =
            make_ulonglong2(as_bits(x[2 * k]), as_bits(x[2 * k + 1]));
    wave_lds_fence();
    if constexpr (PAIR) {
        u64 xb[16];
        ks_own_read<true>(xb, lds, row, i0);
#pragma unroll
        for (int k = 0; k < 16; k++) x[k] = as_f64(xb[k]);
    } else {
#pragma unroll
        for (int k = 0; k < 16; k++) x[k] = as_f64(lds[row_phys(row * 256 + i0 + 16 * k)]);
    }
    wave_lds_fence();
}

template <bool SPLIT, bool MD = false, bool PAIR = false>
__device__ __forceinline__ void ks_row_mac_fp_body(const KsMacArgs& a, const KsIdx& ki, const Mod& md, int midx,
                                                   u64* lds, void* twbuf)
{
    const int t = threadIdx.x;
    const int item = ki.item, tile = ki.tile, slot = ki.slot;
    const FC fc = make_fc(md.q, FP_SITE(SPLIT ? FPS_KS_ROW_SPLIT : FPS_KS_ROW, a.n_power - 12));
    const int s1 = a.n_power - 8;
    const ulonglong2* __restrict__ tw = a.tw + ((u64) midx << a.n_power);
    const int row = t >> 4, i0 = t & 15;
    const u32 crow = tile * 16 + row;
    const double* __restrict__ tb8 = a.twB8 + ((u64) midx * (15u << (a.n_power - 4))) + ((u64) crow * 15 * 16 + i0);
    const u64* __restrict__ pin = a.in + a.in_item_stride * item + ((u64) slot << a.n_power) + (u64) tile * 4096;
    const u64* __restrict__ pk = a.key + ((u64) midx << a.n_power) + (u64) tile * 4096 + row * 256 + ks_own0<PAIR>(i0);
    const u64 dig_off = (u64) a.rc << a.n_power;
    const u64 key_off1 = (u64) a.key_limbs << a.n_power, key_off2 = (u64) a.key_limbs << (a.n_power + 1);

    double* twl = reinterpret_cast<double*>(twbuf);
#pragma unroll
    for (int k = 0; k < 15; k++) twl[k * 256 + t] = tb8[k * 16];
    if (i0 < 15) {
        const int s = (i0 >= 7) ? 3 : (i0 >= 3) ? 2 : (i0 >= 1) ? 1 : 0;
        const int b = i0 - ((1 << s) - 1);
        twl[15 * 256 + i0 * 16 + row] = as_f64(tw[((((u32) 1 << s1) + crow) << s) + b].x);
    }
    wave_lds_fence();

    const int item_s = MD ? __builtin_amdgcn_readfirstlane(item) : 0, slot_s = MD ? __builtin_amdgcn_readfirstlane(slot) : 0;
    const int tile_s = MD ? __builtin_amdgcn_readfirstlane(tile) : 0, midx_s = MD ? __builtin_amdgcn_readfirstlane(midx) : 0;
    double a0[16], a1[16];
#pragma unroll
    for (int k = 0; k < 16; k++) a0[k] = a1[k] = 0.0;
    int since = 0;
    for (int i = ki.d0; i < ki.d1; i++) {
        double x[16];
        const u64* p = pin + dig_off * i;
        const bool ident = a.skip_identity && i == midx;
        const u64* px = ident ? a.ident + a.ident_item_stride * item + ((u64) i << a.n_power) + (u64) tile * 4096 : p;
        u64 xr[16];
        if (PAIR && ident) {
            ks_ld16<PAIR, true>(xr, px + row * 256 + 2 * i0);
        } else {
#pragma unroll
            for (int k = 0; k < 16; k++) {
                if constexpr (!SPLIT) xr[k] = __builtin_nontemporal_load(&px[row * 256 + i0 + 16 * k]);
                else xr[k] = px[row * 256 + i0 + 16 * k];
            }
        }
        const u64* k0 = pk + key_off2 * i;
        const u64* k1 = k0 + key_off1;
        u64 kv0[16], kv1[16];
        if constexpr (PAIR) {
#pragma unroll
            for (int m = 0; m < 8; m++) {
                const ulonglong2 v0 = *reinterpret_cast<const ulonglong2*>(k0 + 32 * m);
                const ulonglong2 v1 = *reinterpret_cast<const ulonglong2*>(k1 + 32 * m);
                kv0[2 * m] = v0.x;
                kv0[2 * m + 1] = v0.y;
                kv1[2 * m] = v1.x;
                kv1[2 * m + 1] = v1.y;
            }
        } else {
#pragma unroll
            for (int k = 0; k < 16; k++) {
                kv0[k] = k0[16 * k];
                kv1[k] = k1[16 * k];
            }
        }
        if (ident) {
            FP_STAGE(fc, FP_STAGE_INPUT);
#pragma unroll
            for (int k = 0; k < 16; k++) x[k] = fp_reduce(fp_from_u64_ldexp(xr[k]), fc);
        } else {
            ks_fp_row<SPLIT, PAIR>(x, xr, twl, lds, fc, s1, row, i0, t);
        }
#pragma unroll
        for (int k = 0; k < 16; k++) {
            FP_STAGE(fc, FP_STAGE_PRODUCT);
            a0[k] += fp_mul_nc(fp_from_u64_ldexp(kv0[k]), x[k], fc);
            a1[k] += fp_mul_nc(fp_from_u64_ldexp(kv1[k]), x[k], fc);
            FP_STAGE(fc, FP_STAGE_SUMS + since);
            FP_AUDIT_VAL(fc, FPM_SUM, a0[k]);
            FP_AUDIT_VAL(fc, FPM_SUM, a1[k]);
        }
        if (++since == 3) {
            since = 0;
            FP_STAGE(fc, FP_STAGE_SUMS + 3);
#pragma unroll
            for (int k = 0; k < 16; k++) {
                a0[k] = fp_reduce(a0[k], fc);
                a1[k] = fp_reduce(a1[k], fc);
            }
        }
    }
    if constexpr (MD) {
        int tt = threadIdx.x;
        asm volatile("" : "+v"(tt));
        const int trow = tt >> 4, ti0 = tt & 15;
        const u64 e0 = (u64) tile_s * 4096 + trow * 256 + ks_own0<PAIR>(ti0);
        const double inv = fp_from_u64(a.tail.inv[midx_s]);
        auto part = [&](int p, const double (&acc)[16]) {
            const u64* pT = ks_tail_T(a, item_s, slot_s, tile_s, p);
            u64 tr[16], cv[16];
#pragma unroll
            for (int k = 0; k < 16; k++) tr[k] = __builtin_nontemporal_load(&pT[trow * 256 + ti0 + 16 * k]);
            const bool with_ct = ks_tail_ct<PAIR>(a, item_s, slot_s, p, e0, cv);
            double x[16];
            ks_fp_row<false, PAIR>(x, tr, twl, lds, fc, s1, trow, ti0, tt);
            ks_tail_store_fp<PAIR>(a, item_s, slot_s, p, e0, fc, inv, acc, x, with_ct, cv);
        };
        __builtin_amdgcn_sched_barrier(0);
        part(0, a0);
        __builtin_amdgcn_sched_barrier(0);
        part(1, a1);
        return;
    }
    u64* po = (SPLIT ? const_cast<u64*>(pin) + dig_off * ki.d0 - (u64) tile * 4096
                     : a.out + a.out_item_stride * item + ((u64) slot << a.n_power)) +
              (u64) tile * 4096 + row * 256 + ks_own0<PAIR>(i0);
    FP_STAGE(fc, FP_STAGE_OUT);
    if constexpr (PAIR) {
        u64 r0[16], r1[16];
#pragma unroll
        for (int k = 0; k < 16; k++) {
            r0[k] = fp_to_u64(fp_canon(a0[k], fc));
            r1[k] = fp_to_u64(fp_canon(a1[k], fc));
        }
        ks_st16<true, !SPLIT>(po, r0);
        ks_st16<true, !SPLIT>(po + dig_off, r1);
        return;
    }
#pragma unroll
    for (int k = 0; k < 16; k++) {
        if constexpr (!SPLIT) {
            __builtin_nontemporal_store(fp_to_u64(fp_canon(a0[k], fc)), &po[16 * k]);
            __builtin_nontemporal_store(fp_to_u64(fp_canon(a1[k], fc)), &po[dig_off + 16 * k]);
        } else {
            po[16 * k] = fp_to_u64(fp_canon(a0[k], fc));
            po[dig_off + 16 * k] = fp_to_u64(fp_canon(a1[k], fc));
        }
    }
}

template <bool SPLIT>
__global__ __launch_bounds__(NTT_THREADS) void ks_row_mac_fp(KsMacArgs a)
{
    __shared__ __attribute__((aligned(16))) u64 lds[ROW_LDS_ELEMS];
    __shared__ double twl[15 * 256 + 15 * 16];
    const KsIdx ki = ks_index<SPLIT, SPLIT ? 0 : 2>(a);
    if (!ki.valid) return;
    const int midx = a.mod_order ? a.mod_order[ki.slot] : ki.slot;
    const Mod md = a.mods[midx];
    if (!md.fp) return;
    ks_row_mac_fp_body<SPLIT>(a, ki, md, midx, lds, twl);
}

__global__ __launch_bounds__(NTT_THREADS) void ks_row_mac_fp_moddown(KsMacArgs a)
{
    __shared__ __attribute__((aligned(16))) u64 lds[ROW_LDS_ELEMS];
    __shared__ double twl[15 * 256 + 15 * 16];
    const KsIdx ki = ks_index<false, 2>(a);
    if (!ki.valid) return;
    const int midx = a.mod_order ? a.mod_order[ki.slot] : ki.slot;
    const Mod md = a.mods[midx];
    if (!md.fp) return;
    ks_row_mac_fp_body<false, true>(a, ki, md, midx, lds, twl);
}
__global__ __launch_bounds__(NTT_THREADS, 1) void ks_row_mac_moddown(KsMacArgs a)
{
    __shared__ __attribute__((aligned(16))) u64 lds[ROW_LDS_ELEMS];
    __shared__ ulonglong2 twa[15 * 16];
    const KsIdx ki = ks_index<false, 1>(a);
    if (!ki.valid) return;
    const int midx = a.mod_order ? a.mod_order[ki.slot] : ki.slot;
    const Mod md = a.mods[midx];
    if (md.fp) return;
    ks_row_mac_int_body<false, true>(a, ki, md, midx, lds, twa);
}

template <bool MD>
__global__ __launch_bounds__(NTT_THREADS, 2) void ks_pair_mac_fp(KsMacArgs a)
{
    __shared__ __attribute__((aligned(16))) u64 lds[ROW_LDS_ELEMS];
    __shared__ double twl[15 * 256 + 15 * 16];
    const KsIdx ki = ks_index<false, 2>(a);
    if (!ki.valid) return;
    const int midx = a.mod_order ? a.mod_order[ki.slot] : ki.slot;
    const Mod md = a.mods[midx];
    if (!md.fp) return;
    ks_row_mac_fp_body<false, MD, true>(a, ki, md, midx, lds, twl);
}
template <bool MD>
__global__ __launch_bounds__(NTT_THREADS, 2) void ks_pair_mac(KsMacArgs a)
{
    __shared__ __attribute__((aligned(16))) u64 lds[ROW_LDS_ELEMS];
    __shared__ ulonglong2 twa[15 * 16];
    const KsIdx ki = ks_index<false, 1>(a);
    if (!ki.valid) return;
    const int midx = a.mod_order ? a.mod_order[ki.slot] : ki.slot;
    const Mod md = a.mods[midx];
    if (md.fp) return;
    ks_row_mac_int_body<false, MD, true>(a, ki, md, midx, lds, twa);
}

__global__ __launch_bounds__(NTT_THREADS, 2) void ks_row_mac_split(KsMacArgs a)
{
    __shared__ __attribute__((aligned(16))) u64 lds[ROW_LDS_ELEMS];
    __shared__ double twl[15 * 256 + 15 * 16];
    const KsIdx ki = ks_index<true>(a);
    if (!ki.valid) return;
    const int midx = a.mod_order ? a.mod_order[ki.slot] : ki.slot;
    const Mod md = a.mods[midx];
    if (md.fp) ks_row_mac_fp_body<true>(a, ki, md, midx, lds, twl);
    else ks_row_mac_int_body<true>(a, ki, md, midx, lds, twl);
}

static std::atomic<unsigned long long> g_ks_forms[3];
void ks_row_mac_launch_counts(unsigned long long out[3])
{
    for (int i = 0; i < 3; i++) out[i] = g_ks_forms[i].load(std::memory_order_relaxed);
}

hipError_t ks_row_mac_launch(const KsMacArgs& a, int items, hipStream_t st)
{
    if (a.digits > 64 || items <= 0) return hipErrorInvalidValue;
    if (a.splits > 1 && a.digits < 2 * a.splits) return hipErrorInvalidValue;
    if (a.tail.on && (a.splits > 1 || !a.tail.out || !a.tail.T || !a.tail.inv)) return hipErrorInvalidValue;
    if (a.slot_first < 0 || a.slot_count < 0 || a.slot_first + (a.slot_count ? a.slot_count : a.rc) > a.rc)
        return hipErrorInvalidValue;
    KsMacArgs k = a;
    k.items = items;
    if (k.int_slot_count < 0 || k.int_slot_count > 8) k.int_slot_count = 0;
    const unsigned tiles = (1u << a.n_power) / 4096, units = (unsigned) items * (a.splits > 1 ? (unsigned) a.splits : 1u);
    auto grid_of = [&](int kind) { return dim3(8u * ((ks_slots(k, kind) * tiles * units + 7u) / 8u)); };
    auto pair_ok = [](const void* p, u64 stride) { return !(reinterpret_cast<uintptr_t>(p) & 15u) && !(stride & 1u); };
    const bool wide = a.wide && a.splits <= 1 && pair_ok(a.key, 0) &&
                      (a.tail.on ? pair_ok(a.tail.out, a.tail.out_item_stride) && pair_ok(a.tail.ct, a.tail.ct_item_stride)
                                 : pair_ok(a.out, a.out_item_stride)) &&
                      (!a.skip_identity || pair_ok(a.ident, a.ident_item_stride));
    g_ks_forms[a.splits > 1 ? 2 : wide ? 1 : 0].fetch_add(1, std::memory_order_relaxed);
    if (a.splits > 1) {
        hipLaunchKernelGGL(ks_row_mac_split, grid_of(0), dim3(NTT_THREADS), 0, st, k);
    } else if (wide) {
        if (!a.no_fp && ks_slots(k, 2) > 0) {
            if (a.tail.on) hipLaunchKernelGGL(ks_pair_mac_fp<true>, grid_of(2), dim3(NTT_THREADS), 0, st, k);
            else hipLaunchKernelGGL(ks_pair_mac_fp<false>, grid_of(2), dim3(NTT_THREADS), 0, st, k);
        }
        if (!a.no_int && ks_slots(k, 1) > 0) {
            if (a.tail.on) hipLaunchKernelGGL(ks_pair_mac<true>, grid_of(1), dim3(NTT_THREADS), 0, st, k);
            else hipLaunchKernelGGL(ks_pair_mac<false>, grid_of(1), dim3(NTT_THREADS), 0, st, k);
        }
    } else {
        if (!a.no_fp && ks_slots(k, 2) > 0) {
            if (a.tail.on) hipLaunchKernelGGL(ks_row_mac_fp_moddown, grid_of(2), dim3(NTT_THREADS), 0, st, k);
            else hipLaunchKernelGGL(ks_row_mac_fp<false>, grid_of(2), dim3(NTT_THREADS), 0, st, k);
        }
        if (!a.no_int && ks_slots(k, 1) > 0) {
            if (a.tail.on) hipLaunchKernelGGL(ks_row_mac_moddown, grid_of(1), dim3(NTT_THREADS), 0, st, k);
            else hipLaunchKernelGGL(ks_row_mac<false>, grid_of(1), dim3(NTT_THREADS), 0, st, k);
        }
    }
    return hipGetLastError();
}

__device__ __forceinline__ void fp_gs_bfly(double& x, double& y, ulonglong2 w, const FC& c)
{
    const double s = x + y, d = x - y;
    x = s;
    y = fp_mul(d, as_f64(w.x), as_f64(w.y), c);
    FP_AUDIT_VAL(c, FPM_SUM, s);
}

struct ArInt {
    typedef u64 T;
    QC qc;
    __device__ __forceinline__ explicit ArInt(const Mod& md) : qc(make_qc(md.q)) {}
    __device__ __forceinline__ T from_canon(u64 v) const { return v; }
    __device__ __forceinline__ T from_bits(u64 v) const { return v; }
    __device__ __forceinline__ u64 to_bits(T v) const { return v; }
    template <int LOGR>
    __device__ __forceinline__ void radix(T (&x)[1 << LOGR], const ulonglong2* __restrict__ tw, u32 root0) const
    {
        gs_radix<LOGR>(x, tw, root0, qc);
    }
    __device__ __forceinline__ void radix16_tb(T (&x)[16], const ulonglong2* __restrict__ tb) const { gs_radix16_tb(x, tb, qc); }
    template <int LOGR>
    __device__ __forceinline__ void radix_last(T (&x)[1 << LOGR], const ulonglong2* __restrict__ tw, ulonglong2 ninv,
                                               ulonglong2 w1ninv, u64 (&out)[1 << LOGR]) const
    {
        gs_radix_last<LOGR>(x, tw, 1u, ninv, w1ninv, qc);
#pragma unroll
        for (int k = 0; k < (1 << LOGR); k++) out[k] = x[k];
    }
};

struct ArFp {
    typedef double T;
    FC fc;
    int s1;
    __device__ __forceinline__ explicit ArFp(const Mod& md, int n_power) : fc(make_fc(md.q, FP_SITE(FPS_INV, n_power - 12))), s1(n_power - 8) {}
    __device__ __forceinline__ T from_canon(u64 v) const { return fp_from_u64(v); }
    __device__ __forceinline__ T from_bits(u64 v) const { return as_f64(v); }
    __device__ __forceinline__ u64 to_bits(T v) const { return as_bits(v); }
    template <int N>
    __device__ __forceinline__ void reduce_all(T (&x)[N]) const
    {
#pragma unroll
        for (int k = 0; k < N; k++) x[k] = fp_reduce(x[k], fc);
    }
    template <int LOGR>
    __device__ __forceinline__ void radix(T (&x)[1 << LOGR], const ulonglong2* __restrict__ tw, u32 root0) const
    {
        int done = 0;
#pragma unroll
        for (int s = LOGR - 1; s >= 0; s--) {
            const int half = (1 << LOGR) >> (s + 1);
            FP_STAGE(fc, 31 - __builtin_clz(root0) + s);
#pragma unroll
            for (int b = 0; b < (1 << s); b++) {
                const ulonglong2 w = tw[(root0 << s) + b];
#pragma unroll
                for (int j = 0; j < half; j++) fp_gs_bfly(x[b * 2 * half + j], x[b * 2 * half + j + half], w, fc);
            }
            if ((++done & 1) == 0 || s == 0) reduce_all(x);
        }
    }
    __device__ __forceinline__ void radix16_tb(T (&x)[16], const ulonglong2* __restrict__ tb) const
    {
#pragma unroll
        for (int s = 3; s >= 0; s--) {
            const int half = 8 >> s;
            FP_STAGE(fc, s1 + 4 + s);
#pragma unroll
            for (int b = 0; b < (1 << s); b++) {
                const ulonglong2 w = tb[((1 << s) - 1 + b) * 16];
#pragma unroll
                for (int j = 0; j < half; j++) fp_gs_bfly(x[b * 2 * half + j], x[b * 2 * half + j + half], w, fc);
            }
            if (s == 2 || s == 0) reduce_all(x);
        }
    }
    template <int LOGR>
    __device__ __forceinline__ void radix_last(T (&x)[1 << LOGR], const ulonglong2* __restrict__ tw, ulonglong2 ninv,
                                               ulonglong2 w1ninv, u64 (&out)[1 << LOGR]) const
    {
        int done = 0;
#pragma unroll
        for (int s = LOGR - 1; s >= 1; s--) {
            const int half = (1 << LOGR) >> (s + 1);
            FP_STAGE(fc, s);
#pragma unroll
            for (int b = 0; b < (1 << s); b++) {
                const ulonglong2 w = tw[(1u << s) + b];
#pragma unroll
                for (int j = 0; j < half; j++) fp_gs_bfly(x[b * 2 * half + j], x[b * 2 * half + j + half], w, fc);
            }
            if ((++done & 1) == 0) reduce_all(x);
        }
        constexpr int half = (1 << LOGR) >> 1;
        FP_STAGE(fc, 0);
#pragma unroll
        for (int j = 0; j < half; j++) {
            const double sum = x[j] + x[j + half], d = x[j] - x[j + half];
            out[j] = fp_to_u64(fp_canon(fp_mul(sum, as_f64(ninv.x), as_f64(ninv.y), fc), fc));
            out[j + half] = fp_to_u64(fp_canon(fp_mul(d, as_f64(w1ninv.x), as_f64(w1ninv.y), fc), fc));
        }
    }
};

template <typename AR, bool TO_LDS, bool TENSOR = false>
__device__ __forceinline__ void inv_row_part(const AR& ar, const NttArgs& a, int mod, int tt, u32 crow0,
                                             const u64* __restrict__ src, u64* __restrict__ dst, u64* lds,
                                             int tensor_part = 0)
{
    typedef typename AR::T T;
    const int s1 = a.n_power - 8;
    const ulonglong2* __restrict__ tw = a.itw + ((u64) mod << a.n_power);
    const int row = tt >> 4, i0 = tt & 15;
    const u32 crow = crow0 + row;
    if (TENSOR) {
        const Mod md = a.mods[mod];
        const u64 part_off = (u64) a.tensor_limbs << a.n_power;
        const u64* __restrict__ a0 = src, * __restrict__ a1 = src + part_off, * __restrict__ b0 = src + 2 * part_off,
                 * __restrict__ b1 = src + 3 * part_off;
#pragma unroll
        for (int k0 = 0; k0 < 16; k0 += 4) {
            u64 r[4];
            if (tensor_part == 1) {
                u64 va0[4], va1[4], vb0[4], vb1[4];
#pragma unroll
                for (int k = 0; k < 4; k++) {
                    const int e = row * 256 + i0 + 16 * (k0 + k);
                    va0[k] = a0[e]; va1[k] = a1[e]; vb0[k] = b0[e]; vb1[k] = b1[e];
                }
#pragma unroll
                for (int k = 0; k < 4; k++) {
                    u64 h1, l1, h2, l2;
                    mul64wide(va0[k], vb1[k], h1, l1);
                    mul64wide(va1[k], vb0[k], h2, l2);
                    const u64 lo = l1 + l2;
                    r[k] = reduce128(h1 + h2 + (lo < l1), lo, md);
                }
            } else {
                const u64* __restrict__ pa = tensor_part == 0 ? a0 : a1;
                const u64* __restrict__ pb = tensor_part == 0 ? b0 : b1;
                u64 va[4], vb[4];
#pragma unroll
                for (int k = 0; k < 4; k++) {
                    const int e = row * 256 + i0 + 16 * (k0 + k);
                    va[k] = pa[e]; vb[k] = pb[e];
                }
#pragma unroll
                for (int k = 0; k < 4; k++) r[k] = mul_barrett(va[k], vb[k], md);
            }
#pragma unroll
            for (int k = 0; k < 4; k++) lds[row_phys(row * 256 + i0 + 16 * (k0 + k))] = r[k];
        }
    } else {
#pragma unroll
        for (int k = 0; k < 16; k++) lds[row_phys(row * 256 + i0 + 16 * k)] = gld(&src[row * 256 + i0 + 16 * k]);
    }
    wave_lds_fence();
    T x[16];
#pragma unroll
    for (int k = 0; k < 8; k++) {
        ulonglong2 v = *reinterpret_cast<const ulonglong2*>(&lds[row_phys(row * 256 + 16 * i0 + 2 * k)]);
        x[2 * k] = ar.from_canon(v.x);
        x[2 * k + 1] = ar.from_canon(v.y);
    }
    ar.radix16_tb(x, a.itwB + ((u64) mod * (15u << (a.n_power - 4))) + ((u64) crow * 15 * 16 + i0));
    wave_lds_fence();
#pragma unroll
    for (int k = 0; k < 8; k++)
        *reinterpret_cast<ulonglong2*>(&lds[row_phys(row * 256 + 16 * i0 + 2 * k)]) =
            make_ulonglong2(ar.to_bits(x[2 * k]), ar.to_bits(x[2 * k + 1]));
    wave_lds_fence();
#pragma unroll
    for (int k = 0; k < 16; k++) x[k] = ar.from_bits(lds[row_phys(row * 256 + i0 + 16 * k)]);
    ar.template radix<4>(x, tw, (1u << s1) + crow);
    if constexpr (TO_LDS) {
#pragma unroll
        for (int k = 0; k < 16; k++) lds[row_phys(row * 256 + i0 + 16 * k)] = ar.to_bits(x[k]);
    } else {
#pragma unroll
        for (int k = 0; k < 16; k++) gst(&dst[row * 256 + i0 + 16 * k], ar.to_bits(x[k]));
    }
}

struct InvEpi {
    const u64* last;
    const u64* ct;
    u64* out;
    Mod md;
    u64 half, qP, hm, inv;
    int galois, n_power;
    bool pre;
};
__device__ __forceinline__ bool inv_epi_setup(const NttArgs& a, const PolySel& ps, InvEpi& e, bool& skip)
{
    skip = false;
    if (!a.iepi.on) return false;
    const NttInvEpilogue& ep = a.iepi;
    const int pc = ep.p_count ? ep.p_count : 1;
    const int part = udiv16(ps.j, ep.mg_slots), limb = ps.j - part * (ep.limbs + pc);
    if (limb >= ep.limbs) { skip = true; return true; }
    const u64 item_in = a.out_item_stride * ps.item;
    const u64 off = (u64) (part * ep.limbs + limb) << a.n_power;
    e.pre = ep.u != nullptr;
    e.last = e.pre ? ep.u + ep.u_item_stride * ps.item + off
                   : a.out + item_in + ((u64) (part * (ep.limbs + 1) + ep.limbs) << a.n_power);
    e.ct = (ep.ct && part < ep.add_parts) ? ep.ct + ep.ct_item_stride * ps.item + off : nullptr;
    e.out = ep.out + ep.out_item_stride * ps.item + off;
    e.md = a.mods[ps.mod];
    e.half = ep.half;
    e.qP = a.mods[ep.p_mod].q;
    e.hm = e.pre ? 0 : ep.half_mod[limb];
    e.inv = ep.inv[limb];
    e.galois = ep.galois_elt;
    e.n_power = a.n_power;
    return true;
}
template <int CNT, bool EPI, typename POS>
__device__ __forceinline__ void inv_store(const InvEpi& epr, u64* __restrict__ p, u32 e0, POS pos, const u64 (&o)[CNT])
{
    if constexpr (!EPI) {
#pragma unroll
        for (int k = 0; k < CNT; k++) gst(&p[pos(k)], o[k]);
        return;
    }
    const InvEpi* ep = &epr;
    u64 lv[CNT], cv[CNT], r[CNT];
#pragma unroll
    for (int k = 0; k < CNT; k++) lv[k] = ep->last[e0 + pos(k)];
    if (ep->ct) {
#pragma unroll
        for (int k = 0; k < CNT; k++) cv[k] = ep->ct[e0 + pos(k)];
    }
    if (!ep->pre) {
#pragma unroll
        for (int k = 0; k < CNT; k++) {
            u64 l = add_mod(lv[k], ep->half, ep->qP);
            l = reduce64(l, ep->md);
            lv[k] = sub_mod(l, ep->hm, ep->md.q);
        }
    }
#pragma unroll
    for (int k = 0; k < CNT; k++) r[k] = mul_barrett(sub_mod(o[k], lv[k], ep->md.q), ep->inv, ep->md);
    if (ep->ct) {
#pragma unroll
        for (int k = 0; k < CNT; k++) r[k] = add_mod(cv[k], r[k], ep->md.q);
    }
    if (ep->galois) {
#pragma unroll
        for (int k = 0; k < CNT; k++) {
            const u32 raw = (e0 + (u32) pos(k)) * (u32) ep->galois;
            ep->out[raw & ((1u << ep->n_power) - 1u)] = ((raw >> ep->n_power) & 1u) ? ep->md.q - r[k] : r[k];
        }
    } else {
#pragma unroll
        for (int k = 0; k < CNT; k++) ep->out[e0 + pos(k)] = r[k];
    }
}

template <int S1, typename AR, bool FROM_LDS, bool KEEP = false, bool EPI = false, bool STORE = true>
__device__ __forceinline__ void inv_col_part(const AR& ar, const NttArgs& a, int mod, int tt, int g, u64* __restrict__ p,
                                             u64* buf, u64 (&keep)[16], const InvEpi& ep = InvEpi(), u32 e0 = 0)
{
    typedef typename AR::T T;
    constexpr int R = 1 << S1;
    constexpr int CT = 4096 / R;
    constexpr int NSA = S1 - 4;
    constexpr int RA = 1 << NSA;
    constexpr int G = 16 / RA;
    const ulonglong2* __restrict__ tw = a.itw + ((u64) mod << a.n_power);
    const ulonglong2 ninv = a.ninv[mod], w1ninv = a.w1ninv[mod];
    const int col = tt % CT, r1 = tt / CT;
    auto pos = [&](int row, int c) -> int {
        if constexpr (FROM_LDS) return single_pos<S1>(row, g * CT + c);
        else return col_phys(row * CT + c);
    };
    T x[16];
#pragma unroll
    for (int k = 0; k < 16; k++)
        x[k] = ar.from_bits(FROM_LDS ? buf[pos(16 * r1 + k, col)] : gld(&p[(u64) (16 * r1 + k) * 256 + col]));
    if constexpr (NSA > 0) {
        ar.template radix<4>(x, tw, (u32) (RA + r1));
#pragma unroll
        for (int k = 0; k < 16; k++) buf[pos(16 * r1 + k, col)] = ar.to_bits(x[k]);
        __syncthreads();
#pragma unroll
        for (int gi = 0; gi < G; gi++) {
            const int L = tt + NTT_THREADS * gi;
            const int c = L % CT, rb = L / CT;
            T y[RA];
            u64 o[RA];
#pragma unroll
            for (int k = 0; k < RA; k++) y[k] = ar.from_bits(buf[pos(rb + 16 * k, c)]);
            ar.template radix_last<NSA>(y, tw, ninv, w1ninv, o);
            if constexpr (!STORE) {
            } else if constexpr (RA == 16) {
                u64 oa[8], ob[8];
#pragma unroll
                for (int k = 0; k < 8; k++) { oa[k] = o[k]; ob[k] = o[8 + k]; }
                inv_store<8, EPI>(ep, p, e0, [&](int k) { return (u32) ((rb + 16 * k) * 256 + c); }, oa);
                inv_store<8, EPI>(ep, p, e0, [&](int k) { return (u32) ((rb + 16 * (8 + k)) * 256 + c); }, ob);
            } else {
                inv_store<RA, EPI>(ep, p, e0, [&](int k) { return (u32) ((rb + 16 * k) * 256 + c); }, o);
            }
            if constexpr (KEEP) {
#pragma unroll
                for (int k = 0; k < RA; k++) keep[gi * RA + k] = o[k];
            }
        }
    } else {
        u64 o[16];
        ar.template radix_last<4>(x, tw, ninv, w1ninv, o);
        if constexpr (STORE) {
            u64 oa[8], ob[8];
#pragma unroll
            for (int k = 0; k < 8; k++) { oa[k] = o[k]; ob[k] = o[8 + k]; }
            inv_store<8, EPI>(ep, p, e0, [&](int k) { return (u32) (k * 256 + col); }, oa);
            inv_store<8, EPI>(ep, p, e0, [&](int k) { return (u32) ((8 + k) * 256 + col); }, ob);
        }
        if constexpr (KEEP) {
#pragma unroll
            for (int k = 0; k < 16; k++) keep[k] = o[k];
        }
    }
}

__global__ __launch_bounds__(NTT_THREADS) void ntt_inv_row(NttArgs a)
{
    __shared__ __attribute__((aligned(16))) u64 lds[ROW_LDS_ELEMS];
    const PolySel ps = select_poly(a, blockIdx.y);
    if (a.iepi.on && ps.j - udiv16(ps.j, a.iepi.mg_slots) * (a.iepi.limbs + (a.iepi.p_count ? a.iepi.p_count : 1)) >= a.iepi.limbs)
        return;
    const Mod md = a.mods[ps.mod];
    const u64* __restrict__ src = a.in + ps.in_off + (u64) blockIdx.x * 4096;
    u64* __restrict__ dst = a.out + ps.out_off + (u64) blockIdx.x * 4096;
    if (md.fp) inv_row_part<ArFp, false>(ArFp(md, a.n_power), a, ps.mod, threadIdx.x, blockIdx.x * 16, src, dst, lds);
    else inv_row_part<ArInt, false>(ArInt(md), a, ps.mod, threadIdx.x, blockIdx.x * 16, src, dst, lds);
}

__device__ __forceinline__ const u64* tensor_src(const NttArgs& a, const PolySel& ps, int& part)
{
    part = udiv16(ps.j, a.mg_tensor_limbs);
    const int limb = ps.j - part * a.tensor_limbs;
    return a.tensor_in + (u64) ps.item * a.tensor_item_stride + ((u64) limb << a.n_power);
}
__global__ __launch_bounds__(NTT_THREADS) void ntt_inv_row_tensor(NttArgs a)
{
    __shared__ __attribute__((aligned(16))) u64 lds[ROW_LDS_ELEMS];
    const PolySel ps = select_poly(a, blockIdx.y);
    const Mod md = a.mods[ps.mod];
    int part;
    const u64* __restrict__ src = tensor_src(a, ps, part) + (u64) blockIdx.x * 4096;
    u64* __restrict__ dst = a.out + ps.out_off + (u64) blockIdx.x * 4096;
    if (md.fp) inv_row_part<ArFp, false, true>(ArFp(md, a.n_power), a, ps.mod, threadIdx.x, blockIdx.x * 16, src, dst, lds, part);
    else inv_row_part<ArInt, false, true>(ArInt(md), a, ps.mod, threadIdx.x, blockIdx.x * 16, src, dst, lds, part);
}

template <int S1, bool EPI = false>
__global__ __launch_bounds__(NTT_THREADS) void ntt_inv_col(NttArgs a)
{
    constexpr int CT = 4096 >> S1;
    __shared__ u64 lds[(S1 > 4) ? COL_LDS_ELEMS : 1];
    const PolySel ps = select_poly(a, blockIdx.y);
    const Mod md = a.mods[ps.mod];
    if (a.only_int && md.fp) return;
    u64* __restrict__ p = a.out + ps.out_off + blockIdx.x * CT;
    u64 unused[16];
    if constexpr (EPI) {
        InvEpi epi;
        bool skip;
        inv_epi_setup(a, ps, epi, skip);
        if (skip) return;
        if (md.fp) inv_col_part<S1, ArFp, false, false, true>(ArFp(md, a.n_power), a, ps.mod, threadIdx.x, 0, p, lds, unused, epi, blockIdx.x * CT);
        else inv_col_part<S1, ArInt, false, false, true>(ArInt(md), a, ps.mod, threadIdx.x, 0, p, lds, unused, epi, blockIdx.x * CT);
    } else {
        if (md.fp) inv_col_part<S1, ArFp, false>(ArFp(md, a.n_power), a, ps.mod, threadIdx.x, 0, p, lds, unused);
        else inv_col_part<S1, ArInt, false>(ArInt(md), a, ps.mod, threadIdx.x, 0, p, lds, unused);
    }
}

template <int S1, bool EPI, bool TENSOR, typename AR>
__device__ __forceinline__ void inv_single_body(const AR& ar, const NttArgs& a, const PolySel& ps, u64* limb)
{
    constexpr int CT = 4096 >> S1;
    const int t = threadIdx.x, g = t >> 8, tt = t & 255;
    InvEpi epi;
    if constexpr (EPI) {
        bool skip;
        inv_epi_setup(a, ps, epi, skip);
        if (skip) return;
    }
    if constexpr (TENSOR) {
        int part;
        const u64* src = tensor_src(a, ps, part) + (u64) g * 4096;
        inv_row_part<AR, true, true>(ar, a, ps.mod, tt, g * 16, src, nullptr, limb + g * 4096, part);
    } else {
        inv_row_part<AR, true>(ar, a, ps.mod, tt, g * 16, a.in + ps.in_off + (u64) g * 4096, nullptr, limb + g * 4096);
    }
    __syncthreads();
    u64 unused[16];
    if constexpr (EPI) inv_col_part<S1, AR, true, false, true>(ar, a, ps.mod, tt, g, a.out + ps.out_off + g * CT, limb, unused, epi, g * CT);
    else inv_col_part<S1, AR, true>(ar, a, ps.mod, tt, g, a.out + ps.out_off + g * CT, limb, unused);
}

template <int S1, bool EPI = false, bool TENSOR = false>
__global__ __launch_bounds__(16 << S1, 4) void ntt_inv_single(NttArgs a)
{
    extern __shared__ __attribute__((aligned(16))) u64 limb[];
    const PolySel ps = select_poly(a, blockIdx.x);
    const Mod md = a.mods[ps.mod];
    if (md.fp) inv_single_body<S1, EPI, TENSOR>(ArFp(md, a.n_power), a, ps, limb);
    else inv_single_body<S1, EPI, TENSOR>(ArInt(md), a, ps, limb);
}

template <int S1, bool ALL>
__device__ __forceinline__ void fwd_col_multi_body(const NttArgs& a, u64* lds, ulonglong2* twl)
{
    constexpr int R = 1 << S1;
    constexpr int CT = 4096 / R;
    constexpr int NSA = S1 - 4;
    constexpr int RA = 1 << NSA;
    constexpr int G = 16 / RA;
    const int t = threadIdx.x;
    const int rc = a.decomp_mods;
    const int digits = udiv16(a.polys_per_item, a.mg_decomp_mods);
    const int item = udiv16(blockIdx.y, a.mg_per_item), digit = blockIdx.y - item * digits;
    const u64 in_slot = (u64) digit * (a.decomp_in_mul ? a.decomp_in_mul : 1) + a.decomp_in_add;
    const u64* __restrict__ src = a.in + (u64) item * a.in_item_stride + (in_slot << a.n_power) + blockIdx.x * CT;
    u64 sreg[16];
    const int smod = a.half_on ? a.half_src_mod : digit;
    if (a.src_inv && a.mods[smod].fp) {
        const Mod im = a.mods[smod];
        inv_col_part<S1, ArFp, false, true, false, !ALL>(ArFp(im, a.n_power), a, smod, t, 0, const_cast<u64*>(src), lds, sreg);
        __syncthreads();
    } else if constexpr (NSA > 0) {
#pragma unroll
        for (int g = 0; g < G; g++) {
            const int L = t + NTT_THREADS * g;
            const int c = L % CT, rb = L / CT;
#pragma unroll
            for (int k = 0; k < RA; k++) sreg[g * RA + k] = src[(u64) (rb + 16 * k) * 256 + c];
        }
    } else {
#pragma unroll
        for (int k = 0; k < 16; k++) sreg[k] = src[(u64) k * 256 + (t % CT)];
    }
    const Mod smd = a.mods[a.half_on ? a.half_src_mod : digit];
    if (a.half_on) {
#pragma unroll
        for (int k = 0; k < 16; k++) sreg[k] = add_mod(sreg[k], a.half, smd.q);
    }
    const bool wide = smd.bit > 52;
    if (!wide) {
#pragma unroll
        for (int k = 0; k < 16; k++) sreg[k] = as_bits(fp_from_u64(sreg[k]));
    } else {
#pragma unroll
        for (int k = 0; k < 16; k++) asm volatile("" : "+v"(sreg[k]));
    }
    auto target = [&](int k) {
        PolySel ps;
        ps.mod = a.mod_offset + (a.mod_order ? ld_const_i32(a.mod_order + k) : k);
        ps.digit = digit;
        ps.item = item;
        ps.j = digit * rc + k;
        ps.in_off = 0;
        ps.out_off = (u64) item * a.out_item_stride +
                     ((u64) (a.decomp_out_mul ? digit * a.decomp_out_mul + k : ps.j) << a.n_power);
        return ps;
    };
    int done = 0;
    for (int k = 0; k < rc; k++) {
        const PolySel ps = target(k);
        if (a.skip_identity && ps.mod == digit) continue;
        const Mod md = ld_const_mod(a.mods + ps.mod);
        if (!md.fp) continue;
        ulonglong2* tl = twl + ((S1 > 4) ? 256 * (done & 1) : 0);
        done++;
        if (wide) fwd_col_body_fp<S1, true, true, true>(a, ps, md, lds, tl, sreg);
        else fwd_col_body_fp<S1, true, false, true>(a, ps, md, lds, tl, sreg);
    }
    if constexpr (ALL) {
        if (!wide) {
#pragma unroll
            for (int k = 0; k < 16; k++) sreg[k] = fp_to_u64(as_f64(sreg[k]));
        }
        for (int w = 0; w < a.int_slot_count; w++) {
            const PolySel ps = target(a.int_slots[w]);
            if (a.skip_identity && ps.mod == digit) continue;
            const Mod md = ld_const_mod(a.mods + ps.mod);
            ulonglong2* tl = twl + 256 * (done & 1);
            done++;
            if (fwd_stages_lazy(md, a.lazy_q_max)) fwd_col_body<S1, true, true, true>(a, ps, md, lds, sreg, tl);
            else if (stages_room16(md)) fwd_col_body<S1, true, false, true, 16>(a, ps, md, lds, sreg, tl);
            else fwd_col_body<S1, true, false, true>(a, ps, md, lds, sreg, tl);
        }
    }
}

template <int S1>
__global__ __launch_bounds__(NTT_THREADS) void ntt_fwd_col_multi(NttArgs a)
{
    __shared__ u64 lds[(S1 > 4) ? COL_LDS_ELEMS : 1];
    __shared__ ulonglong2 twl[(S1 > 4) ? 512 : 1];
    fwd_col_multi_body<S1, false>(a, lds, twl);
}

template <int S1>
__global__ __launch_bounds__(NTT_THREADS) void ntt_fwd_col_decomp_all(NttArgs a)
{
    __shared__ u64 lds[COL_LDS_ELEMS];
    __shared__ ulonglong2 twl[512];
    fwd_col_multi_body<S1, true>(a, lds, twl);
}

template <int S1>
static bool use_col_multi(const NttArgs& a, int batch)
{
    constexpr int CT = 4096 >> S1;
    if (!a.decomp_mods || a.col_multi == 0 || batch % a.decomp_mods) return false;
    if (a.copy_src) return false;
    if (a.col_multi == 1) return true;
    return (long) (256 / CT) * (batch / a.decomp_mods) >= 2048;
}

template <int S1>
static void launch_col_multi(const NttArgs& a, int batch, hipStream_t st)
{
    constexpr int CT = 4096 >> S1;
    if constexpr (S1 == 8) {
        if (a.plan_has_fp && a.plan_has_int && a.int_slot_count > 0 && a.int_slot_count <= 8) {
            hipLaunchKernelGGL((ntt_fwd_col_decomp_all<S1>), dim3(256 / CT, batch / a.decomp_mods), dim3(NTT_THREADS), 0, st, a);
            return;
        }
    }
    if (a.plan_has_fp)
        hipLaunchKernelGGL((ntt_fwd_col_multi<S1>), dim3(256 / CT, batch / a.decomp_mods), dim3(NTT_THREADS), 0, st, a);
    if ((a.plan_has_int || !a.plan_has_fp) && !(a.plan_has_fp && a.int_slot_count < 0)) {
        NttArgs c = a;
        c.group_span = 0;
        c.mg_group_span = 0;
        c.only_int = a.plan_has_fp;
        int polys = batch;
        if (c.only_int && a.int_slot_count > 0) polys = batch / a.decomp_mods * a.int_slot_count;
        else c.int_slot_count = 0;
        hipLaunchKernelGGL((ntt_fwd_col<S1, true>), dim3(256 / CT, polys), dim3(NTT_THREADS), 0, st, c);
    }
}

static bool use_single_pass(const NttArgs& a, int batch)
{
    if (a.single_pass == 1) return true;
    if (a.single_pass == 0) return false;
    const int s1 = a.n_power - 8;
    if (s1 <= 4) return true;
    if (s1 == 5) return batch >= 64;
    if (batch < 48) return false;
    const long rounds = ((long) batch + 255) / 256;
    return (long) batch * 4 >= rounds * 256 * 3;
}

template <int S1>
static void launch_fwd_col_only(const NttArgs& a, int batch, hipStream_t st)
{
    constexpr int CT = 4096 >> S1;
    if (use_col_multi<S1>(a, batch)) launch_col_multi<S1>(a, batch, st);
    else if (a.decomp_mods)
        hipLaunchKernelGGL((ntt_fwd_col<S1, true>), dim3(256 / CT, batch), dim3(NTT_THREADS), 0, st, a);
    else
        hipLaunchKernelGGL((ntt_fwd_col<S1, false>), dim3(256 / CT, batch), dim3(NTT_THREADS), 0, st, a);
}

template <int S1>
static void launch_fwd(const NttArgs& a, int batch, hipStream_t st)
{
    constexpr int CT = 4096 >> S1;
    if constexpr (S1 <= 6) {
        if (!a.decomp_mods && use_single_pass(a, batch)) {
            static const hipError_t attr = hipFuncSetAttribute((const void*) ntt_fwd_single<S1>,
                                                               hipFuncAttributeMaxDynamicSharedMemorySize, 8 << (S1 + 8));
            (void) attr;
            hipLaunchKernelGGL((ntt_fwd_single<S1>), dim3(batch), dim3(16 << S1), (size_t) 8 << (S1 + 8), st, a);
            return;
        }
        if (a.decomp_mods && a.single_decomp_ok && !a.copy_src && !a.src_inv && !use_col_multi<S1>(a, batch) &&
            use_single_pass(a, batch)) {
            static const hipError_t attr_d = hipFuncSetAttribute((const void*) ntt_fwd_single<S1, true>,
                                                                 hipFuncAttributeMaxDynamicSharedMemorySize, 8 << (S1 + 8));
            (void) attr_d;
            NttArgs c = a;
            c.group_span = 0;
            c.mg_group_span = 0;
            hipLaunchKernelGGL((ntt_fwd_single<S1, true>), dim3(batch), dim3(16 << S1), (size_t) 8 << (S1 + 8), st, c);
            return;
        }
    }
    if (use_col_multi<S1>(a, batch)) {
        launch_col_multi<S1>(a, batch, st);
    } else if (a.decomp_mods) {
        NttArgs c = a;
        c.group_span = 0;
        c.mg_group_span = 0;
        hipLaunchKernelGGL((ntt_fwd_col<S1, true>), dim3(256 / CT, batch), dim3(NTT_THREADS), 0, st, c);
    } else
        hipLaunchKernelGGL((ntt_fwd_col<S1, false>), dim3(256 / CT, batch), dim3(NTT_THREADS), 0, st, a);
    NttArgs b = a;
    b.in = a.out;
    b.in_item_stride = a.out_item_stride;
    hipLaunchKernelGGL(ntt_fwd_row, dim3((1u << a.n_power) / 4096, batch), dim3(NTT_THREADS), 0, st, b);
}

template <int S1>
static void launch_inv(const NttArgs& a, int batch, hipStream_t st)
{
    constexpr int CT = 4096 >> S1;
    if constexpr (S1 <= 6) {
        if (use_single_pass(a, batch) && !a.poly_order) {
            static const hipError_t attr = hipFuncSetAttribute((const void*) ntt_inv_single<S1, false>,
                                                               hipFuncAttributeMaxDynamicSharedMemorySize, 8 << (S1 + 8));
            static const hipError_t attr_e = hipFuncSetAttribute((const void*) ntt_inv_single<S1, true>,
                                                                 hipFuncAttributeMaxDynamicSharedMemorySize, 8 << (S1 + 8));
            static const hipError_t attr_t = hipFuncSetAttribute((const void*) ntt_inv_single<S1, false, true>,
                                                                 hipFuncAttributeMaxDynamicSharedMemorySize, 8 << (S1 + 8));
            (void) attr;
            (void) attr_e;
            (void) attr_t;
            if (a.tensor_in)
                hipLaunchKernelGGL((ntt_inv_single<S1, false, true>), dim3(batch), dim3(16 << S1), (size_t) 8 << (S1 + 8), st, a);
            else if (a.iepi.on)
                hipLaunchKernelGGL((ntt_inv_single<S1, true>), dim3(batch), dim3(16 << S1), (size_t) 8 << (S1 + 8), st, a);
            else
                hipLaunchKernelGGL((ntt_inv_single<S1, false>), dim3(batch), dim3(16 << S1), (size_t) 8 << (S1 + 8), st, a);
            return;
        }
    }
    if (a.tensor_in) hipLaunchKernelGGL(ntt_inv_row_tensor, dim3((1u << a.n_power) / 4096, batch), dim3(NTT_THREADS), 0, st, a);
    else hipLaunchKernelGGL(ntt_inv_row, dim3((1u << a.n_power) / 4096, batch), dim3(NTT_THREADS), 0, st, a);
    NttArgs b = a;
    b.in = a.out;
    b.in_item_stride = a.out_item_stride;
    if (a.iepi.on) hipLaunchKernelGGL((ntt_inv_col<S1, true>), dim3(256 / CT, batch), dim3(NTT_THREADS), 0, st, b);
    else hipLaunchKernelGGL((ntt_inv_col<S1, false>), dim3(256 / CT, batch), dim3(NTT_THREADS), 0, st, b);
}

static unsigned magic16(int d) { return d <= 1 ? 0u : (unsigned) ((0x100000000ull + (unsigned) d - 1) / (unsigned) d); }
static void fill_magics(NttArgs& g)
{
    g.mg_group_span = magic16(g.group_span);
    g.mg_mod_count = magic16(g.mod_count);
    g.mg_per_item = magic16(g.mod_count ? g.polys_per_item / g.mod_count : 0);
    g.mg_polys_per_item = magic16(g.polys_per_item);
    g.mg_decomp_mods = magic16(g.decomp_mods);
    g.epi.mg_limbs = magic16(g.epi.limbs);
    g.iepi.mg_slots = magic16(g.iepi.limbs + (g.iepi.p_count ? g.iepi.p_count : 1));
    g.mg_tensor_limbs = magic16(g.tensor_limbs);
}

bool ntt_decomp_uses_multi(const NttArgs& a, int batch)
{
    if (!a.plan_has_fp) return false;
    switch (a.n_power - 8) {
        case 4: return use_col_multi<4>(a, batch);
        case 5: return use_col_multi<5>(a, batch);
        case 6: return use_col_multi<6>(a, batch);
        case 7: return use_col_multi<7>(a, batch);
        case 8: return use_col_multi<8>(a, batch);
    }
    return false;
}

hipError_t ntt_launch_inv_rows(const NttArgs& a, int batch, hipStream_t st)
{
    if (batch <= 0) return hipSuccess;
    if (a.n_power < 12 || a.n_power > 16 || batch > 65535) return hipErrorInvalidValue;
    NttArgs g = a;
    g.group_span = 0;
    if (!a.poly_order && a.mod_count > 1 && batch % a.mod_count == 0 &&
        (!a.polys_per_item || a.polys_per_item % a.mod_count == 0))
        g.group_span = batch / a.mod_count;
    fill_magics(g);
    hipLaunchKernelGGL(ntt_inv_row, dim3((1u << a.n_power) / 4096, batch), dim3(NTT_THREADS), 0, st, g);
    if (a.plan_has_int) {
        NttArgs b = g;
        b.in = g.out;
        b.in_item_stride = g.out_item_stride;
        b.only_int = 1;
        switch (a.n_power - 8) {
#define CASE(S) case S: hipLaunchKernelGGL((ntt_inv_col<S, false>), dim3(256 / (4096 >> S), batch), dim3(NTT_THREADS), 0, st, b); break;
            CASE(4) CASE(5) CASE(6) CASE(7) CASE(8)
#undef CASE
        }
    }
    return hipGetLastError();
}

hipError_t ntt_launch_fwd_col(const NttArgs& a, int batch, hipStream_t st)
{
    if (batch <= 0) return hipSuccess;
    if (a.n_power < 12 || a.n_power > 16 || batch > 65535 || a.poly_order) return hipErrorInvalidValue;
    if (a.src_inv && !ntt_decomp_uses_multi(a, batch)) return hipErrorInvalidValue;
    NttArgs g = a;
    g.group_span = 0;
    if (!a.decomp_mods && a.mod_count > 1 && batch % a.mod_count == 0 &&
        (!a.polys_per_item || a.polys_per_item % a.mod_count == 0))
        g.group_span = batch / a.mod_count;
    fill_magics(g);
    switch (a.n_power - 8) {
        case 4: launch_fwd_col_only<4>(g, batch, st); break;
        case 5: launch_fwd_col_only<5>(g, batch, st); break;
        case 6: launch_fwd_col_only<6>(g, batch, st); break;
        case 7: launch_fwd_col_only<7>(g, batch, st); break;
        case 8: launch_fwd_col_only<8>(g, batch, st); break;
    }
    return hipGetLastError();
}

hipError_t ntt_launch(const NttArgs& a, int batch, bool inverse, hipStream_t st)
{
    if (batch <= 0) return hipSuccess;
    if (a.n_power < 12 || a.n_power > 16) return hipErrorInvalidValue;
    if (a.decomp_mods && (inverse || a.poly_order || !a.polys_per_item)) return hipErrorInvalidValue;
    if (a.src_inv && (!a.decomp_mods || batch > 65535 || !ntt_decomp_uses_multi(a, batch))) return hipErrorInvalidValue;
    if (a.copy_src && (!a.decomp_mods || inverse)) return hipErrorInvalidValue;
    if (a.tensor_in && (!inverse || a.poly_order || a.iepi.on || a.polys_per_item != 3 * a.tensor_limbs || batch % a.polys_per_item))
        return hipErrorInvalidValue;
    if (a.iepi.on && (!inverse || a.poly_order || batch % a.polys_per_item ||
                      a.polys_per_item != 2 * (a.iepi.limbs + (a.iepi.p_count ? a.iepi.p_count : 1)) ||
                      ((a.iepi.p_count > 1) != (a.iepi.u != nullptr))))
        return hipErrorInvalidValue;
    if (batch > 65535) {
        const int unit = a.polys_per_item ? a.polys_per_item : a.mod_count;
        if ((!a.polys_per_item && a.poly_order) || (batch % unit) || unit > 65535) return hipErrorInvalidValue;
        int done = 0;
        while (done < batch) {
            int chunk = batch - done;
            int maxc = (65535 / unit) * unit;
            if (chunk > maxc) chunk = maxc;
            NttArgs c = a;
            if (a.polys_per_item) {
                const u64 items_done = (u64) (done / unit);
                c.in = a.in + items_done * a.in_item_stride;
                c.out = a.out + items_done * a.out_item_stride;
                if (a.epi.on) {
                    c.epi.ks = a.epi.ks + items_done * a.epi.ks_item_stride;
                    if (a.epi.ct) c.epi.ct = a.epi.ct + items_done * a.epi.ct_item_stride;
                    c.epi.out = a.epi.out + items_done * a.epi.out_item_stride;
                }
                if (a.iepi.on) {
                    if (a.iepi.ct) c.iepi.ct = a.iepi.ct + items_done * a.iepi.ct_item_stride;
                    c.iepi.out = a.iepi.out + items_done * a.iepi.out_item_stride;
                    if (a.iepi.u) c.iepi.u = a.iepi.u + items_done * a.iepi.u_item_stride;
                }
                if (a.copy_src) {
                    c.copy_src = a.copy_src + items_done * a.copy_src_item_stride;
                    c.copy_dst = a.copy_dst + items_done * a.copy_dst_item_stride;
                }
                if (a.tensor_in) c.tensor_in = a.tensor_in + items_done * a.tensor_item_stride;
            } else {
                c.in = a.in + ((u64) done << a.n_power);
                c.out = a.out + ((u64) done << a.n_power);
            }
            hipError_t e = ntt_launch(c, chunk, inverse, st);
            if (e != hipSuccess) return e;
            done += chunk;
        }
        return hipSuccess;
    }
    NttArgs g = a;
    g.group_span = 0;
    if (!a.poly_order && a.mod_count > 1 && batch % a.mod_count == 0 &&
        (!a.polys_per_item || a.polys_per_item % a.mod_count == 0))
        g.group_span = batch / a.mod_count;
    fill_magics(g);
    switch (a.n_power - 8) {
#define CASE(S)                                   \
    case S:                                       \
        if (inverse) launch_inv<S>(g, batch, st); \
        else launch_fwd<S>(g, batch, st);         \
        break;
        CASE(4) CASE(5) CASE(6) CASE(7) CASE(8)
#undef CASE
    }
    return hipGetLastError();
}

}
```

### heongpu_amd/csrc/ntt.hpp

```cpp
#pragma once
#include "modarith.cuh"

namespace hegpu {

struct NttEpilogue {
    const u64* ks;
    u64 ks_item_stride;
    int ks_part_limbs;
    const u64* ct;
    u64 ct_item_stride;
    int ct_parts;
    unsigned galois_inv;
    u64* out;
    u64 out_item_stride;
    const u64* inv;
    int limbs;
    int on;
    unsigned mg_limbs;
};

struct NttInvEpilogue {
    int on;
    int limbs;
    int add_parts;
    int p_mod;
    int galois_elt;
    unsigned mg_slots;
    u64 half;
    const u64* half_mod;
    const u64* inv;
    const u64* ct;
    u64 ct_item_stride;
    u64* out;
    u64 out_item_stride;
    int p_count;
    const u64* u;
    u64 u_item_stride;
};

struct NttArgs {
    const u64* in;
    u64* out;
    const Mod* mods;
    const ulonglong2* tw;
    const ulonglong2* itw;
    const ulonglong2* twB;
    const ulonglong2* itwB;
    const double* twB8;
    const ulonglong2* ninv;
    const ulonglong2* w1ninv;
    const int* mod_order;
    const int* poly_order;
    int n_power;
    int mod_count;
    int mod_offset;
    int polys_per_item;
    u64 in_item_stride;
    u64 out_item_stride;
    int decomp_mods;
    int skip_identity;
    int group_span;
    unsigned mg_group_span, mg_per_item, mg_polys_per_item, mg_mod_count, mg_decomp_mods;
    NttEpilogue epi;
    NttInvEpilogue iepi;
    int decomp_in_mul, decomp_in_add;
    int decomp_out_mul;
    int half_on, half_src_mod;
    u64 half;
    const u64* half_mod;
    int col_multi;
    int single_pass;
    int plan_has_fp, plan_has_int;
    u64 lazy_q_max;
    int only_int;
    int single_decomp_ok;
    int int_slot_count;
    int int_slots[8];
    int src_inv;
    const u64* copy_src;
    u64* copy_dst;
    u64 copy_src_item_stride, copy_dst_item_stride;
    int copy_part_limbs;
    const u64* tensor_in;
    u64 tensor_item_stride;
    int tensor_limbs;
    unsigned mg_tensor_limbs;
};

hipError_t ntt_launch(const NttArgs& a, int batch, bool inverse, hipStream_t st);
bool ntt_decomp_uses_multi(const NttArgs& a, int batch);
hipError_t ntt_launch_inv_rows(const NttArgs& a, int batch, hipStream_t st);
hipError_t ntt_launch_fwd_col(const NttArgs& a, int batch, hipStream_t st);

struct KsMacArgs {
    const u64* in;
    u64 in_item_stride;
    const u64* key;
    u64* out;
    u64 out_item_stride;
    const Mod* mods;
    const ulonglong2* tw;
    const ulonglong2* twB;
    const double* twB8;
    const int* mod_order;
    int n_power, digits, rc, key_limbs;
    u64 lazy_q_max;
    int skip_identity;
    const u64* ident;
    u64 ident_item_stride;
    int items;
    int splits;
    int no_fp, no_int;
    int int_slot_count;
    int int_slots[8];
    int slot_first, slot_count;
    int unreduced_exit;
    int wide;
    struct Tail {
        int on;
        const u64* T;
        u64 T_item_stride;
        const u64* ct;
        u64 ct_item_stride;
        int ct_parts;
        unsigned galois_inv;
        u64* out;
        u64 out_item_stride;
        const u64* inv;
        int limbs;
    } tail;
};
hipError_t ks_row_mac_launch(const KsMacArgs& a, int items, hipStream_t st);
void ks_row_mac_launch_counts(unsigned long long out[3]);
constexpr inline int ks_unreduced_exit(int digits, int q_bits)
{
    if (digits <= 0 || q_bits <= 0 || 2 * q_bits > 127) return 0;
    const unsigned __int128 room = ((unsigned __int128) 1 << (128 - 2 * q_bits));
    for (int b = 16; b >= 8; b -= 4)
        if ((unsigned __int128) digits * (unsigned) b <= room) return b;
    return 0;
}

}
```

### heongpu_amd/csrc/ops.cpp

```cpp
#include "ops.hpp"
#include <algorithm>
#include <vector>
#include <utility>

namespace hegpu {

#define TRY(x)                           \
    do {                                 \
        hipError_t e__ = (x);            \
        if (e__ != hipSuccess) return e__; \
    } while (0)

static u64 inv_mod_2n(u64 g, u64 two_n)
{
    u64 x = g;
    for (int i = 0; i < 6; i++) x *= 2 - g * x;
    return x & (two_n - 1);
}

static long fused_row_mac_need(const Context& c)
{
    size_t fp = 0;
    for (unsigned char f : c.plan_qp.fp) fp += f ? 1 : 0;
    return (2 * fp > c.plan_qp.fp.size()) ? 768 : 400;
}
static int fused_digit_splits(const Context& c, int rc, int digits, int batch)
{
    if (c.digit_split == 0) return 0;
    if (c.digit_split > 0) return digits >= 2 * c.digit_split ? c.digit_split : 0;
    if (c.fused_row_mac >= 0 || c.n_power < 16 || digits < 8) return 0;
    const long wgs = (long) batch * rc * (long) (c.n >> 12), need = fused_row_mac_need(c);
    return (need == 768 && wgs < 2 * need && 4 * wgs >= need) ? 4 : 0;
}
static bool use_fused_row_mac(const Context& c, int rc, int batch)
{
    if (c.fused_row_mac >= 0) return c.fused_row_mac != 0;
    return (long) batch * rc * (long) (c.n >> 12) >= fused_row_mac_need(c);
}
static bool use_moddown_in_mac(const Context& c, const u64* key, int l, int rc, int batch)
{
    return c.moddown_in_mac && c.fused_moddown && key && c.P_size == 1 && use_fused_row_mac(c, rc, batch) &&
           !fused_digit_splits(c, rc, l, batch) && (long) 2 * l * batch <= 65535;
}

static void fill_int_slots(const Context& c, NttArgs& a, const u64* order)
{
    int cnt = 0;
    for (int k = 0; k < a.decomp_mods; k++) {
        const int m = a.mod_offset + (order ? (int) order[k] : k);
        if (m < 0 || m >= (int) c.plan_qp.fp.size()) { a.int_slot_count = 0; return; }
        if (c.plan_qp.fp[m]) continue;
        if (cnt == 8) { a.int_slot_count = 0; return; }
        a.int_slots[cnt++] = k;
    }
    a.int_slot_count = cnt ? cnt : -1;
}

static int launch_int_q_bits(const Context& c, const int* order, int rc, int depth, int slot_first, int slot_count)
{
    const NttPlan& p = c.plan_qp;
    const u64* ho = nullptr;
    const size_t off = (size_t) triangle_offset(c.Qp_size, depth);
    if (order && order == c.tab.new_prime_locations + off && off + (size_t) rc <= c.hv.new_prime_locations.size())
        ho = c.hv.new_prime_locations.data() + off;
    int bits = 0;
    auto take = [&](size_t m) { if (m < p.bits.size() && !p.fp[m] && p.bits[m] > bits) bits = p.bits[m]; };
    if (order && !ho) {
        for (size_t m = 0; m < p.bits.size(); m++) take(m);
        return bits;
    }
    const int k0 = slot_count ? slot_first : 0, k1 = slot_count ? slot_first + slot_count : rc;
    for (int k = k0; k < k1; k++) take(ho ? (size_t) ho[k] : (size_t) k);
    return bits;
}

static hipError_t keyswitch_ntt_mac(const Context& c, NttArgs a, const u64* key, u64* acc, u64 acc_stride,
                                    int digits, int rc, int split, int level, const u64* ident, u64 ident_stride,
                                    int batch, hipStream_t st, int which = 3, int slot_first = 0, int slot_count = 0,
                                    const KsMacArgs::Tail* tail = nullptr)
{
    const int ppi = digits * rc;
    const int skip_identity = ident ? 1 : 0;
    a.skip_identity = skip_identity;
    const int splits = fused_digit_splits(c, rc, digits, batch);
    if (!splits && !use_fused_row_mac(c, rc, batch)) {
        if (slot_count || tail) return hipErrorInvalidValue;
        if (ident && c.fused_row_mac == 0)
            TRY(rns_copy_diag(ident, ident_stride, a.out, a.out_item_stride, c.n_power, digits, rc, batch, st));
        else a.skip_identity = 0;
        TRY(ntt_launch(a, ppi * batch, false, st));
        return rns_keyswitch_mac(a.out, a.out_item_stride, key, acc, acc_stride, c.plan_qp.mods, c.n_power, digits, rc,
                                 c.Qp_size, split, level, batch, st);
    }
    const int chunk = 65535 / ppi;
    if (chunk < 1) return hipErrorInvalidValue;
    for (int b0 = 0; b0 < batch; b0 += chunk) {
        const int nb = (batch - b0 < chunk) ? batch - b0 : chunk;
        NttArgs ca = a;
        ca.in = a.in + (u64) b0 * a.in_item_stride;
        ca.out = a.out + (u64) b0 * a.out_item_stride;
        if (which & 1) TRY(ntt_launch_fwd_col(ca, ppi * nb, st));
        if (!(which & 2)) continue;
        KsMacArgs k{};
        k.in = ca.out; k.in_item_stride = a.out_item_stride; k.key = key;
        k.out = acc + (u64) b0 * acc_stride; k.out_item_stride = acc_stride;
        k.mods = c.plan_qp.mods; k.tw = c.plan_qp.tw; k.twB = c.plan_qp.twB; k.twB8 = c.plan_qp.twB8; k.mod_order = a.mod_order;
        k.lazy_q_max = a.lazy_q_max; k.n_power = c.n_power; k.digits = digits; k.rc = rc; k.key_limbs = c.Qp_size; k.skip_identity = skip_identity;
        k.ident = ident ? ident + (u64) b0 * ident_stride : nullptr; k.ident_item_stride = ident_stride;
        k.splits = splits;
        k.wide = c.wide_access && splits <= 1;
        k.no_fp = !a.plan_has_fp;
        k.no_int = !a.plan_has_int || a.int_slot_count < 0;
        k.int_slot_count = a.int_slot_count > 0 ? a.int_slot_count : 0;
        for (int q = 0; q < 8; q++) k.int_slots[q] = a.int_slots[q];
        k.slot_first = slot_first; k.slot_count = slot_count;
        k.unreduced_exit = ks_unreduced_exit(splits > 1 ? (digits + splits - 1) / splits : digits,
                                             launch_int_q_bits(c, a.mod_order, rc, level, slot_first, slot_count));
        if (slot_count && a.int_slot_count > 0) {
            int cnt = 0;
            for (int q = 0; q < a.int_slot_count; q++)
                if (a.int_slots[q] >= slot_first && a.int_slots[q] < slot_first + slot_count) k.int_slots[cnt++] = a.int_slots[q];
            k.int_slot_count = cnt;
            k.no_int = cnt == 0;
            k.no_fp = k.no_fp || cnt == slot_count;
        }
        if (tail) {
            k.tail = *tail;
            k.tail.T += (u64) b0 * tail->T_item_stride;
            if (tail->ct) k.tail.ct += (u64) b0 * tail->ct_item_stride;
            k.tail.out += (u64) b0 * tail->out_item_stride;
        }
        TRY(ks_row_mac_launch(k, nb, st));
        if (splits > 1)
            TRY(rns_sum_partials(ca.out, a.out_item_stride, k.out, acc_stride, c.plan_qp.mods, a.mod_order, c.n_power,
                                 digits, rc, splits, nb, st));
    }
    return hipSuccess;
}


struct KeySwitchWs { u64 digits, acc, acc_words, per; };
static KeySwitchWs keyswitch_ws(const Context& c, int depth, bool copy, int accs)
{
    const u64 l = c.Q_size - depth, rc = c.Qp_size - depth;
    const u64 digits = copy ? 2 * l * c.n : 0, acc = digits + l * rc * c.n, acc_words = 2 * rc * c.n;
    return {digits, acc, acc_words, acc + accs * acc_words};
}
int ops_rotate_hoisted_accumulators(const Context& c, int depth, int batch, size_t ws_elems)
{
    return ws_elems >= keyswitch_ws(c, depth, true, 4).per * (u64) batch ? 4 : 1;
}

struct PairWs { u64 second, per; };
static PairWs rescale_ws(const Context& c, int depth)
{
    const u64 l = c.Q_size - depth;
    return {2 * (l - 1) * c.n, (2 * (l - 1) + 2 * l) * c.n};
}
static u64 mod_raise_ws(const Context& c) { return 2 * c.n; }
static PairWs bfv_multiply_ws(const Context& c)
{
    const u64 L = c.Q_size + c.bsk_size;
    return {4 * L * c.n, (4 + 3) * L * c.n};
}
static PairWs ckks_decode_ws(const Context& c, int depth) { const u64 l = c.Q_size - depth; return {l * c.n, (l + 1) * c.n}; }
static PairWs public_key_share_ws(const Context& c) { return {(u64) c.Qp_size * c.n, (u64) 2 * c.Qp_size * c.n}; }
static PairWs switch_key_share_ws(const Context& c, int errs)
{
    return {(u64) errs * switch_key_digits(c) * c.Qp_size * c.n, (u64) (errs + 1) * c.Q_size * c.Qp_size * c.n};
}
struct EncryptWs { u64 e, pku, per; };
static EncryptWs encrypt_ws(const Context& c)
{
    const u64 limb = (u64) c.Qp_size * c.n;
    return {limb, 3 * limb, 5 * limb};
}
struct RefreshMergeWs { u64 head_sum, total; };
static RefreshMergeWs bfv_refresh_merge_ws(const Context& c, int batch)
{
    return {(u64) batch * c.n, (u64) (c.Q_size + 1) * c.n * batch};
}
struct GateWs { u64 ps, ks, total; };
static GateWs gate_ws(const Context& c, bool bfv, int depth, int batch)
{
    const auto row = [&](int op) { return ops_workspace_elems(c, op, bfv ? 0 : depth, batch); };
    const size_t most = bfv ? std::max({row(OP_BFV_MULTIPLY), row(OP_BFV_RELIN), row(OP_BFV_MULTIPLY_PLAIN)})
                            : std::max(row(OP_CKKS_RELIN), row(OP_CKKS_RESCALE));
    const u64 ps = (u64) 3 * (bfv ? c.Q_size : c.Q_size - depth) * c.n, ks = ps * batch;
    return {ps, ks, ks + most};
}

size_t ops_workspace_elems(const Context& c, int op, int depth, int batch)
{
    const u64 n = c.n;
    u64 per = 0;
    switch (op) {
        case OP_CKKS_RELIN: per = keyswitch_ws(c, depth, false, 1).per; break;
        case OP_CKKS_RESCALE: per = rescale_ws(c, depth).per; break;
        case OP_CKKS_GALOIS: per = keyswitch_ws(c, depth, true, 1).per; break;
        case OP_CKKS_ROTATE_HOISTED: per = keyswitch_ws(c, depth, true, 4).per; break;
        case OP_BFV_MULTIPLY: per = bfv_multiply_ws(c).per; break;
        case OP_BFV_RELIN:
        case OP_BFV_GALOIS: per = keyswitch_ws(c, 0, false, 1).per; break;
        case OP_KEYGEN_SECRET: per = n; break;
        case OP_KEYGEN_PUBLIC: per = public_key_share_ws(c).per; break;
        case OP_KEYGEN_SWITCH: per = switch_key_share_ws(c, 1).per; break;
        case OP_CKKS_ENCRYPT:
        case OP_BFV_ENCRYPT: per = encrypt_ws(c).per; break;
        case OP_BFV_DECRYPT: per = (u64) c.Q_size * n; break;
        case OP_BFV_DECODE: per = n; break;
        case OP_BFV_MULTIPLY_PLAIN: per = (u64) c.Q_size * n; break;
        case OP_CKKS_ENCODE: per = n; break;
        case OP_CKKS_DECODE: per = ckks_decode_ws(c, depth).per; break;
        case OP_MPC_KEY_SHARE: per = switch_key_share_ws(c, 2).per; break;
        case OP_MPC_BFV_DECRYPT_MERGE: per = (u64) c.Q_size * n; break;
        case OP_MPC_REFRESH_SHARE: per = 0; break;
        case OP_MPC_REFRESH_MERGE:
            if (c.scheme != SCHEME_CKKS) return bfv_refresh_merge_ws(c, batch).total;
            per = (u64) (c.Q_size - depth) * n;
            break;
        case OP_CKKS_MOD_RAISE: per = mod_raise_ws(c); break;
        case OP_CKKS_BOOTSTRAP: per = 3 * mod_raise_ws(c); break;
        case OP_CKKS_LOGIC_GATE: return gate_ws(c, false, depth, batch).total;
        case OP_BFV_LOGIC_GATE: return gate_ws(c, true, depth, batch).total;
        default: return 0;
    }
    return per * (u64) batch;
}

hipError_t op_ckks_multiply(const Context& c, const u64* ct1, u64 s1, const u64* ct2, u64 s2, u64* out, u64 so,
                            int depth, int batch, hipStream_t st)
{
    if (batch <= 0) return hipSuccess;
    return rns_cross_multiplication(ct1, s1, ct2, s2, out, so, c.plan_qp.mods, c.n_power, c.Q_size - depth, batch,
                                    st);
}

static hipError_t ckks_keyswitch_core(const Context& c, const u64* src, u64 src_stride, const u64* add, u64 add_stride,
                                      int add_parts, u64* outp, u64 out_stride, const u64* key, int depth, int batch,
                                      u64* temp1, u64* temp2, u64 per, hipStream_t st, unsigned phases,
                                      int galois_elt = 0)
{
    const int Q = c.Q_size, Qp = c.Qp_size;
    const int l = Q - depth, rc = Qp - depth;

    NttArgs a = c.ntt_args(0);
    a.in = src; a.out = temp2; a.mod_count = l; a.polys_per_item = l;
    a.in_item_stride = src_stride; a.out_item_stride = per;
    NttArgs dgt = c.ntt_args(0);
    dgt.in = temp2; dgt.out = temp1; dgt.mod_count = rc; dgt.polys_per_item = l * rc; dgt.decomp_mods = rc;
    dgt.in_item_stride = per; dgt.out_item_stride = per;
    dgt.mod_order = c.tab.new_prime_locations + triangle_offset(Qp, depth);
    fill_int_slots(c, dgt, c.hv.new_prime_locations.data() + triangle_offset(Qp, depth));
    const bool fuse_inv = use_fused_row_mac(c, rc, batch) && c.fuse_inverse && (long) l * rc * batch <= 65535 &&
                          ntt_decomp_uses_multi(dgt, l * rc * batch);
    if (phases & RELIN_PHASE_INTT_C2) {
        if (fuse_inv) TRY(ntt_launch_inv_rows(a, l * batch, st));
        else TRY(ntt_launch(a, l * batch, true, st));
    }
    dgt.src_inv = fuse_inv ? 1 : 0;
    dgt.single_decomp_ok = 1;
    a = dgt;
    const int which = ((phases & RELIN_PHASE_COLUMN) ? 1 : 0) | ((phases & RELIN_PHASE_ROW_MAC) ? 2 : 0);
    const bool in_mac = use_moddown_in_mac(c, key, l, rc, batch);
    if (which)
        TRY(keyswitch_ntt_mac(c, a, key, temp2, per, l, rc, l, depth, src, src_stride, batch, st, which, in_mac ? l : 0,
                              in_mac ? 1 : 0));
    const NttArgs dgt_args = a;
    a = c.ntt_args(0);
    a.in = temp2; a.out = temp2; a.mod_count = 1; a.mod_offset = Q; a.polys_per_item = 2;
    a.in_item_stride = a.out_item_stride = per;
    a.poly_order = c.tab.new_input_locations + 2 * depth;
    NttArgs md = c.ntt_args(0);
    md.in = temp2; md.out = temp1; md.mod_count = l; md.polys_per_item = 2 * l;
    md.in_item_stride = md.out_item_stride = per;
    md.decomp_mods = l; md.decomp_in_mul = l + 1; md.decomp_in_add = l;
    md.half_on = 1; md.half_src_mod = Q;
    fill_int_slots(c, md, nullptr);
    const bool fuse_inv_p = c.fused_moddown && c.fuse_inverse && (long) 2 * l * batch <= 65535 &&
                            ntt_decomp_uses_multi(md, 2 * l * batch);
    if (phases & RELIN_PHASE_INTT_P) {
        if (fuse_inv_p) TRY(ntt_launch_inv_rows(a, 2 * batch, st));
        else TRY(ntt_launch(a, 2 * batch, true, st));
    }
    if (in_mac) {
        if (phases & RELIN_PHASE_MODDOWN) {
            a = md;
            a.out = temp2; a.decomp_out_mul = l + 1;
            a.half = c.hv.half; a.half_mod = c.tab.half_mod;
            a.src_inv = fuse_inv_p ? 1 : 0;
            TRY(ntt_launch_fwd_col(a, 2 * l * batch, st));
        }
        if (!(phases & RELIN_PHASE_ROW_MAC)) return hipSuccess;
        KsMacArgs::Tail t{};
        t.on = 1;
        t.T = temp2; t.T_item_stride = per;
        t.ct = add; t.ct_item_stride = add_stride; t.ct_parts = add_parts;
        t.out = outp; t.out_item_stride = out_stride;
        t.inv = c.tab.last_q_modinv;
        t.limbs = l;
        t.galois_inv = galois_elt ? (unsigned) inv_mod_2n((u64) galois_elt, 2 * c.n) : 0u;
        return keyswitch_ntt_mac(c, dgt_args, key, temp2, per, l, rc, l, depth, src, src_stride, batch, st, 2, 0, l, &t);
    }
    if (!(phases & RELIN_PHASE_MODDOWN)) return hipSuccess;
    if (!c.fused_moddown)
        TRY(rns_moddown_stage_one(temp2, per, temp1, per, c.moddown(depth), batch, st));
    a = c.ntt_args(0);
    a.in = temp1; a.out = temp1; a.mod_count = l; a.polys_per_item = 2 * l;
    a.in_item_stride = a.out_item_stride = per;
    if (c.fused_moddown) {
        a.in = temp2; a.decomp_mods = l; a.decomp_in_mul = l + 1; a.decomp_in_add = l;
        a.half_on = 1; a.half_src_mod = Q; a.half = c.hv.half; a.half_mod = c.tab.half_mod;
        a.epi.on = 1;
        a.epi.ks = temp2; a.epi.ks_item_stride = per; a.epi.ks_part_limbs = l + 1;
        a.epi.ct = add; a.epi.ct_item_stride = add_stride; a.epi.ct_parts = add_parts;
        a.epi.out = outp; a.epi.out_item_stride = out_stride;
        a.epi.inv = c.tab.last_q_modinv;
        a.epi.limbs = l;
        a.epi.galois_inv = galois_elt ? (unsigned) inv_mod_2n((u64) galois_elt, 2 * c.n) : 0u;
        a.src_inv = fuse_inv_p ? 1 : 0;
        a.single_decomp_ok = 1;
        fill_int_slots(c, a, nullptr);
        return ntt_launch(a, 2 * l * batch, false, st);
    }
    if (add_parts != 2 || galois_elt) return hipErrorInvalidValue;
    TRY(ntt_launch(a, 2 * l * batch, false, st));
    return rns_moddown_stage_two(temp1, per, temp2, per, add, add_stride, outp, out_stride, c.moddown(depth), 1, batch, st);
}

static hipError_t dtoq(const Context& c, int lvl, const u64* in, u64 in_stride, u64* out, u64 out_stride, int l,
                       int level, int batch, hipStream_t st)
{
    const Context::M2Level& L = c.m2_levels[lvl];
    return rns_base_conversion_DtoQtilde(in, in_stride, out, out_stride, c.plan_qp.mods,
                                         c.tab.m2_matrix_mg + L.off_matrix, c.tab.m2_Mi_inv + L.off_mi,
                                         c.tab.m2_negprod_mg + L.off_prod, c.tab.m2_I_j + L.off_digits,
                                         c.tab.m2_I_location + L.off_digits, c.n_power, L.d, L.rc, l, level,
                                         c.m2_width, batch, st);
}

static hipError_t ckks_moddown_multi(const Context& c, u64* acc, u64* scratch, u64 per, const u64* ct, u64 cs,
                                     int add_parts, u64* out, u64 so, int depth, int galois_elt, int batch,
                                     hipStream_t st)
{
    const u64 n = c.n;
    const int Q = c.Q_size, Qp = c.Qp_size, P = c.P_size;
    const int l = Q - depth, rc = Qp - depth;
    for (int part = 0; part < 2; part++) {
        NttArgs a = c.ntt_args(0);
        a.in = a.out = acc + (u64) (part * rc + l) * n;
        a.mod_count = P; a.mod_offset = Q; a.polys_per_item = P;
        a.in_item_stride = a.out_item_stride = per;
        TRY(ntt_launch(a, P * batch, true, st));
    }
    TRY(rns_moddown_multi_stage_one(acc, per, scratch, per, c.moddown(depth), c.tab.m2_md_G, c.tab.m2_md_C, batch, st));
    NttArgs a = c.ntt_args(0);
    a.in = a.out = scratch; a.mod_count = l; a.polys_per_item = 2 * l;
    a.in_item_stride = a.out_item_stride = per;
    a.epi.on = 1;
    a.epi.ks = acc; a.epi.ks_item_stride = per; a.epi.ks_part_limbs = rc;
    a.epi.ct = ct; a.epi.ct_item_stride = cs; a.epi.ct_parts = add_parts;
    a.epi.out = out; a.epi.out_item_stride = so;
    a.epi.inv = c.tab.m2_md_W0;
    a.epi.limbs = l;
    a.epi.galois_inv = galois_elt ? (unsigned) inv_mod_2n((u64) galois_elt, 2 * c.n) : 0u;
    return ntt_launch(a, 2 * l * batch, false, st);
}

static hipError_t ckks_rotate_tail(const Context& c, u64* acc, const u64* coef, u64 per, u64* out, u64 so, int galois_elt,
                                   int depth, int batch, hipStream_t st)
{
    const int Q = c.Q_size, Qp = c.Qp_size;
    const int l = Q - depth, rc = Qp - depth;
    NttArgs a = c.ntt_args(0);
    a.in = acc; a.out = acc; a.mod_count = rc; a.polys_per_item = 2 * rc;
    a.mod_order = c.tab.new_prime_locations + triangle_offset(Qp, depth);
    a.in_item_stride = a.out_item_stride = per;
    TRY(ntt_launch(a, 2 * rc * batch, true, st));
    TRY(rns_moddown_permute(acc, per, coef, per, out, so, c.moddown(depth), galois_elt, batch, st));
    a = c.ntt_args(0);
    a.in = out; a.out = out; a.mod_count = l; a.polys_per_item = 2 * l;
    a.in_item_stride = a.out_item_stride = so;
    return ntt_launch(a, 2 * l * batch, false, st);
}

static hipError_t ckks_keyswitch_II(const Context& c, const u64* ct, u64 cs, int add_parts, u64* out, u64 so,
                                    const u64* key, int galois_elt, int depth, int batch, u64* ws, hipStream_t st)
{
    const int np = c.n_power;
    const u64 n = c.n;
    const int Q = c.Q_size, Qp = c.Qp_size;
    const int l = Q - depth, rc = Qp - depth;
    const int d = c.m2_levels[depth].d;
    const bool relin = add_parts == 2;
    const bool ntt_domain = c.fused_moddown && (relin || c.ntt_galois);
    const KeySwitchWs w = keyswitch_ws(c, depth, !relin, 1);
    u64* coef = relin ? out : ws;
    const u64 coef_stride = relin ? so : w.per;
    u64* digits = ws + w.digits;
    u64* acc = ws + w.acc;
    const int first = (relin || ntt_domain) ? add_parts : 0;
    NttArgs a = c.ntt_args(0);
    a.in = ct + (u64) first * l * n; a.out = coef + (u64) first * l * n; a.mod_count = l;
    a.polys_per_item = (add_parts + 1 - first) * l;
    a.in_item_stride = cs; a.out_item_stride = coef_stride;
    TRY(ntt_launch(a, a.polys_per_item * batch, true, st));
    TRY(dtoq(c, depth, coef + (u64) add_parts * l * n, coef_stride, digits, w.per, l, depth, batch, st));
    a = c.ntt_args(0);
    a.in = digits; a.out = digits; a.mod_count = rc; a.polys_per_item = d * rc;
    a.mod_order = c.tab.new_prime_locations + triangle_offset(Qp, depth);
    a.in_item_stride = a.out_item_stride = w.per;
    TRY(keyswitch_ntt_mac(c, a, key, acc, w.per, d, rc, l, depth, nullptr, 0, batch, st));
    if (ntt_domain)
        return ckks_moddown_multi(c, acc, ws, w.per, ct, cs, relin ? 0 : add_parts, out, so, depth, galois_elt, batch, st);
    if (!relin) return ckks_rotate_tail(c, acc, ws, w.per, out, so, galois_elt, depth, batch, st);
    a.in = acc; a.out = acc; a.polys_per_item = 2 * rc;
    TRY(ntt_launch(a, 2 * rc * batch, true, st));
    TRY(rns_moddown_extended(acc, w.per, nullptr, 0, ws, w.per, c.moddown(depth), 0, batch, st));
    a = c.ntt_args(0);
    a.in = ws; a.out = ws; a.mod_count = l; a.polys_per_item = 2 * l;
    a.in_item_stride = a.out_item_stride = w.per;
    TRY(ntt_launch(a, 2 * l * batch, false, st));
    return rns_addition_strided(ws, w.per, ct, cs, out, so, c.plan_qp.mods, np, l, 2, batch, st);
}

hipError_t op_ckks_relinearize(const Context& c, u64* ct, u64 cs, const u64* key, int depth, int batch, u64* ws,
                               hipStream_t st, unsigned phases)
{
    if (batch <= 0) return hipSuccess;
    if (c.P_size > 1) return ckks_keyswitch_II(c, ct, cs, 2, ct, cs, key, 0, depth, batch, ws, st);
    const int l = c.Q_size - depth;
    const KeySwitchWs w = keyswitch_ws(c, depth, false, 1);
    u64* temp1 = ws + w.digits;
    u64* temp2 = ws + w.acc;
    return ckks_keyswitch_core(c, ct + ((u64) l << (c.n_power + 1)), cs, ct, cs, 2, ct, cs, key, depth, batch, temp1,
                               temp2, w.per, st, phases);
}

hipError_t op_ckks_rescale(const Context& c, u64* ct, u64 cs, int depth, int batch, u64* ws, hipStream_t st)
{
    if (batch <= 0) return hipSuccess;
    const int np = c.n_power;
    const u64 n = c.n;
    const int Q = c.Q_size, P = c.P_size;
    const int l = Q - depth;
    const ModDown md = c.moddown(depth, true);
    const PairWs w = rescale_ws(c, depth);
    u64* temp1 = ws;
    u64* temp2 = ws + w.second;

    NttArgs a = c.ntt_args(0);
    a.in = ct; a.out = ct; a.mod_count = 1; a.mod_offset = l - 1; a.polys_per_item = 2;
    a.in_item_stride = a.out_item_stride = cs;
    a.poly_order = c.tab.new_input_locations + (depth + P) * 2;
    TRY(ntt_launch(a, 2 * batch, true, st));
    if (c.fused_moddown) {
        a = c.ntt_args(0);
        a.in = ct; a.out = temp1; a.mod_count = l - 1; a.polys_per_item = 2 * (l - 1);
        a.in_item_stride = cs; a.out_item_stride = w.per;
        a.decomp_mods = l - 1; a.decomp_in_mul = l; a.decomp_in_add = l - 1;
        a.half_on = 1; a.half_src_mod = l - 1; a.half = c.hv.rescaled_half[depth];
        a.half_mod = md.half_mod;
        if (c.copy_along && !ntt_decomp_uses_multi(a, 2 * (l - 1) * batch)) {
            a.copy_src = ct; a.copy_src_item_stride = cs;
            a.copy_dst = temp2; a.copy_dst_item_stride = w.per;
            a.copy_part_limbs = l;
        } else {
            TRY(rns_copy_limbs(ct, (u64) l * n, cs, temp2, (u64) l * n, w.per, np, l - 1, 2, batch, st));
        }
        a.epi.on = 1;
        a.epi.ks = temp2; a.epi.ks_item_stride = w.per; a.epi.ks_part_limbs = l;
        a.epi.ct = nullptr; a.epi.ct_item_stride = 0;
        a.epi.out = ct; a.epi.out_item_stride = cs;
        a.epi.inv = md.last_q_modinv;
        a.epi.limbs = l - 1;
        return ntt_launch(a, 2 * (l - 1) * batch, false, st);
    }
    TRY(rns_moddown_stage_one(ct, cs, temp1, w.per, md, batch, st));
    a = c.ntt_args(0);
    a.in = temp1; a.out = temp1; a.mod_count = l - 1; a.polys_per_item = 2 * (l - 1);
    a.in_item_stride = a.out_item_stride = w.per;
    TRY(ntt_launch(a, 2 * (l - 1) * batch, false, st));
    TRY(rns_copy_limbs(ct, (u64) l * n, cs, temp2, (u64) l * n, w.per, np, l - 1, 2, batch, st));
    return rns_moddown_stage_two(temp1, w.per, temp2, w.per, nullptr, 0, ct, cs, md, 0, batch, st);
}

static hipError_t mod_raise_scaled(const Context& c, const u64* ct, u64 cs, u64 k1, u64* out, u64 so, int out_depth,
                                   int batch, u64* ws, hipStream_t st)
{
    if (batch <= 0) return hipSuccess;
    const u64 n = c.n, per = mod_raise_ws(c);
    const int L = c.Q_size - out_depth, t = L - 1;
    if (k1 == 1) TRY(rns_copy_limbs(ct, n, cs, out, (u64) L * n, so, c.n_power, 1, 2, batch, st));
    else TRY(rns_scale_q0(ct, cs, k1, out, (u64) L * n, so, t < 1 ? nullptr : ws, per, c.plan_qp.mods, c.n_power, batch, st));
    if (t < 1) return hipSuccess;
    NttArgs inv = c.ntt_args(0);
    inv.in = k1 == 1 ? ct : ws; inv.out = ws; inv.mod_count = 1; inv.polys_per_item = 2;
    inv.in_item_stride = k1 == 1 ? cs : per; inv.out_item_stride = per;
    NttArgs a = c.ntt_args(0);
    a.in = ws; a.out = out + n;
    a.mod_count = t; a.mod_offset = 1; a.polys_per_item = 2 * t;
    a.in_item_stride = per; a.out_item_stride = so;
    a.decomp_mods = t; a.decomp_out_mul = L;
    a.half_on = 1; a.half_src_mod = 0; a.half = c.hv.mod_raise_half; a.half_mod = c.tab.mod_raise_half_mod;
    a.single_decomp_ok = 1;
    fill_int_slots(c, a, nullptr);
    const bool fuse_inv = c.fuse_inverse && (long) 2 * t * batch <= 65535 && ntt_decomp_uses_multi(a, 2 * t * batch);
    if (fuse_inv) TRY(ntt_launch_inv_rows(inv, 2 * batch, st));
    else TRY(ntt_launch(inv, 2 * batch, true, st));
    a.src_inv = fuse_inv ? 1 : 0;
    return ntt_launch(a, 2 * t * batch, false, st);
}

hipError_t op_ckks_mod_raise(const Context& c, const u64* ct, u64 cs, u64* out, u64 so, int out_depth, int batch, u64* ws,
                             hipStream_t st)
{
    return mod_raise_scaled(c, ct, cs, 1, out, so, out_depth, batch, ws, st);
}

hipError_t op_ckks_apply_galois(const Context& c, const u64* ct, u64 cs, u64* out, u64 so, const u64* key,
                                int galois_elt, int depth, int batch, u64* ws, hipStream_t st)
{
    if (batch <= 0) return hipSuccess;
    if (c.P_size > 1) return ckks_keyswitch_II(c, ct, cs, 1, out, so, key, galois_elt, depth, batch, ws, st);
    const int np = c.n_power;
    const u64 n = c.n;
    const int Q = c.Q_size, Qp = c.Qp_size;
    const int l = Q - depth, rc = Qp - depth;
    const KeySwitchWs w = keyswitch_ws(c, depth, true, 1);
    u64* temp0 = ws;
    u64* temp2 = ws + w.digits;
    u64* temp3 = ws + w.acc;

    if (c.fused_moddown && c.ntt_galois) {
        if (c.galois_scatter)
            return ckks_keyswitch_core(c, ct + (u64) l * n, cs, ct, cs, 1, out, so, key, depth, batch, temp2, temp3, w.per, st,
                                       RELIN_PHASE_ALL, galois_elt);
        TRY(ckks_keyswitch_core(c, ct + (u64) l * n, cs, ct, cs, 1, temp0, w.per, key, depth, batch, temp2, temp3, w.per, st,
                                RELIN_PHASE_ALL));
        return rns_permute_ntt(temp0, w.per, out, so, galois_elt, np, 2 * l, batch, st);
    }
    NttArgs a = c.ntt_args(0);
    a.in = ct; a.out = temp0; a.mod_count = l; a.polys_per_item = 2 * l;
    a.in_item_stride = cs; a.out_item_stride = w.per;
    TRY(ntt_launch(a, 2 * l * batch, true, st));
    a = c.ntt_args(0);
    a.in = temp0 + (u64) l * n; a.out = temp2; a.mod_count = rc; a.polys_per_item = l * rc; a.decomp_mods = rc;
    a.in_item_stride = a.out_item_stride = w.per;
    a.mod_order = c.tab.new_prime_locations + triangle_offset(Qp, depth);
    TRY(keyswitch_ntt_mac(c, a, key, temp3, w.per, l, rc, l, depth, ct + (u64) l * n, cs, batch, st));
    return ckks_rotate_tail(c, temp3, temp0, w.per, out, so, galois_elt, depth, batch, st);
}

hipError_t op_bfv_multiply(const Context& c, const u64* ct1, u64 s1, const u64* ct2, u64 s2, u64* out, u64 so,
                           int batch, u64* ws, hipStream_t st)
{
    if (batch <= 0) return hipSuccess;
    const int np = c.n_power;
    const u64 n = c.n;
    const int L = c.Q_size + c.bsk_size;
    const PairWs w = bfv_multiply_ws(c);
    u64* temp1 = ws;
    u64* temp2 = ws + w.second;
    TRY(rns_fast_convertion(ct1, s1, ct2, s2, temp1, w.per, c.behz, np, batch, st));
    NttArgs a = c.ntt_args(1);
    a.in = temp1; a.out = temp1; a.mod_count = L; a.polys_per_item = 4 * L;
    a.in_item_stride = a.out_item_stride = w.per;
    TRY(ntt_launch(a, 4 * L * batch, false, st));
    a.in = temp2; a.out = temp2; a.polys_per_item = 3 * L;
    if (c.fused_tensor) {
        a.tensor_in = temp1; a.tensor_item_stride = w.per; a.tensor_limbs = L;
    } else {
        TRY(rns_cross_multiplication(temp1, w.per, temp1 + (u64) 2 * L * n, w.per, temp2, w.per, c.plan_merge.mods, np, L,
                                     batch, st));
    }
    TRY(ntt_launch(a, 3 * L * batch, true, st));
    return rns_fast_floor(temp2, w.per, out, so, c.behz, np, batch, st);
}

static hipError_t bfv_intt_moddown(const Context& c, u64* acc, u64 per, const u64* ct, u64 cs, int add_parts, u64* out,
                                   u64 so, int galois_elt, int batch, hipStream_t st)
{
    const u64 n = c.n;
    const int Q = c.Q_size, Qp = c.Qp_size;
    for (int part = 0; part < 2; part++) {
        NttArgs a = c.ntt_args(0);
        a.in = a.out = acc + (u64) (part * Qp + Q) * n;
        a.mod_count = 1; a.mod_offset = Q; a.polys_per_item = 1;
        a.in_item_stride = a.out_item_stride = per;
        TRY(ntt_launch(a, batch, true, st));
    }
    NttArgs a = c.ntt_args(0);
    a.in = a.out = acc; a.mod_count = Qp; a.polys_per_item = 2 * Qp;
    a.in_item_stride = a.out_item_stride = per;
    a.iepi.on = 1; a.iepi.limbs = Q; a.iepi.add_parts = add_parts; a.iepi.p_mod = Q; a.iepi.galois_elt = galois_elt;
    a.iepi.half = c.hv.half; a.iepi.half_mod = c.tab.half_mod; a.iepi.inv = c.tab.last_q_modinv;
    a.iepi.ct = ct; a.iepi.ct_item_stride = cs;
    a.iepi.out = out; a.iepi.out_item_stride = so;
    return ntt_launch(a, 2 * Qp * batch, true, st);
}

static hipError_t bfv_intt_moddown_multi(const Context& c, u64* acc, u64* scratch, u64 per, const u64* ct, u64 cs,
                                         int add_parts, u64* out, u64 so, int galois_elt, int batch, hipStream_t st)
{
    const u64 n = c.n;
// ... 1073 lines not shown
```

Baseline: 9142.

## Store column-NTT digit outputs in row-tile blocks for keyswitch row MAC

Adds a blocked intermediate layout for the N=2^16 keyswitch path. The multi-modulus forward column kernels write each 16x256 row tile contiguously, and new row-MAC kernels read these tiles with scalar-base, lane-contiguous loads. The goal is more coalesced, cache-friendly access between the column and row NTT passes. It only applies to CKKS with P=1, unsplit and in-MAC moddown paths, and it adds kernel variants plus validation checks that the producer and consumer agree on the layout.

```diff
diff --git a/heongpu_amd/csrc/context.cpp b/heongpu_amd/csrc/context.cpp
--- a/heongpu_amd/csrc/context.cpp
+++ b/heongpu_amd/csrc/context.cpp
@@ -719,6 +719,7 @@
     {"fused_tensor", "HEGPU_FUSED_TENSOR", &H::fused_tensor},
     {"moddown_in_mac", "HEGPU_MODDOWN_IN_MAC", &H::moddown_in_mac},
     {"wide_access", "HEGPU_WIDE_ACCESS", &H::wide_access},
+    {"digit_blocks", "HEGPU_DIGIT_BLOCKS", &H::digit_blocks},
 };
 const OptDesc* find_option(const char* name)
 {
diff --git a/heongpu_amd/csrc/context.hpp b/heongpu_amd/csrc/context.hpp
--- a/heongpu_amd/csrc/context.hpp
+++ b/heongpu_amd/csrc/context.hpp
@@ -86,6 +86,7 @@
     bool fuse_inverse = true;
     bool moddown_in_mac = true;
     bool wide_access = true;
+    bool digit_blocks = true;
     bool fused_tensor = true;
     bool fp_ntt = true;
     int behz_split = -1;
diff --git a/heongpu_amd/csrc/ntt.hip b/heongpu_amd/csrc/ntt.hip
--- a/heongpu_amd/csrc/ntt.hip
+++ b/heongpu_amd/csrc/ntt.hip
@@ -407,15 +407,43 @@
 #define COL_LDS_ELEMS 4096
 #define ROW_LDS_ELEMS 4096
 
+template <bool BLK> __device__ __forceinline__ constexpr u64 col_out_pos(int r1, int k, int col)
+{
+    return BLK ? (u64) r1 * 4096 + 16 * k + col : (u64) (16 * r1 + k) * 256 + col;
+}
+template <bool BLK> __device__ __forceinline__ constexpr int row_in_pos(int row, int i0, int k)
+{
+    return BLK ? k * 256 + row * 16 + i0 : row * 256 + i0 + 16 * k;
+}
+template <bool NT>
+__device__ __forceinline__ void blk_ld16(u64 (&v)[16], const u64* tile, int row, int i0)
+{
+    static_assert(row_in_pos<true>(1, 1, 2) == 2 * 256 + 17, "element k at k * 256 + (row * 16 + i0)");
+    int lane = row * 16 + i0;
+    asm volatile("" : "+v"(lane));
+    typedef const __attribute__((address_space(1))) u64* gptr;
+    const u64 tb = reinterpret_cast<u64>(tile);
+    const u64 hi = (u32) __builtin_amdgcn_readfirstlane((u32) (tb >> 32)), lo = (u32) __builtin_amdgcn_readfirstlane((u32) tb);
+    const gptr t0 = (gptr) ((hi << 32) | lo);
+#pragma unroll
+    for (int m = 0; m < 8; m++) {
+        gptr b = t0 + 512 * m;
+        asm volatile("" : "+s"(b));
+        v[2 * m] = NT ? __builtin_nontemporal_load(&b[lane]) : b[lane];
+        v[2 * m + 1] = NT ? __builtin_nontemporal_load(&b[lane + 256]) : b[lane + 256];
+    }
+}
+
 __device__ __forceinline__ bool fwd_stages_lazy(const Mod& md, u64 lazy_q_max) { return md.q <= lazy_q_max; }
 #define NTT_ROW_LAZY_MAX_Q 0x0666666666666666ull
 __device__ __forceinline__ bool row_stages_lazy(const Mod& md, u64 lazy_q_max) { return md.q <= lazy_q_max || md.q <= NTT_ROW_LAZY_MAX_Q; }
 __device__ __forceinline__ bool stages_room16(const Mod& md) { return md.bit <= 60; }
 
-template <int S1, bool DECOMP, bool LAZY, bool SREG = false, int ROOM = 8>
+template <int S1, bool DECOMP, bool LAZY, bool SREG = false, int ROOM = 8, bool BLK = false>
 __device__ __forceinline__ void fwd_col_body(const NttArgs& a, const PolySel& ps, const Mod& md, u64* lds,
                                              const u64* sreg = nullptr, ulonglong2* twl = nullptr)
 {
+    static_assert(!BLK || (S1 == 8 && SREG), "row-tile blocks: the multi-modulus column kernels at N = 2^16");
     constexpr CsSched CS = cs_sched(S1, ROOM);
     constexpr int R = 1 << S1;
     constexpr int CT = 4096 / R;
@@ -427,7 +455,7 @@
     const QC qc = make_qc(md.q);
     const ulonglong2* __restrict__ tw = a.tw + ((u64) ps.mod << a.n_power);
     const u64* __restrict__ src = a.in + ps.in_off + blockIdx.x * CT;
-    u64* __restrict__ dst = a.out + ps.out_off + blockIdx.x * CT;
+    u64* __restrict__ dst = a.out + ps.out_off + blockIdx.x * (BLK ? 256 : CT);
 
     const u64 half_qP = (a.half_on && !SREG) ? a.mods[a.half_src_mod].q : 0;
     const u64 half_hm = a.half_on ? (SREG ? ld_const_u64(a.half_mod + ps.mod) : a.half_mod[ps.mod]) : 0;
@@ -481,13 +509,14 @@
     if constexpr (SREG && NSA > 0) ct_radix<4, LAZY, (CS.c8 >> NSA), (CS.c4 >> NSA)>(x, twl, (u32) (RA + r1), qc);
     else ct_radix<4, LAZY, (CS.c8 >> NSA), (CS.c4 >> NSA)>(x, tw, (u32) (RA + r1), qc);
 #pragma unroll
-    for (int k = 0; k < 16; k++) gst(&dst[(u64) (16 * r1 + k) * 256 + col], x[k]);
-}
-
-template <int S1, bool DECOMP, bool WIDE, bool SREG = false>
+    for (int k = 0; k < 16; k++) gst(&dst[col_out_pos<BLK>(r1, k, col)], x[k]);
+}
+
+template <int S1, bool DECOMP, bool WIDE, bool SREG = false, bool BLK = false>
 __device__ __forceinline__ void fwd_col_body_fp(const NttArgs& a, const PolySel& ps, const Mod& md, u64* lds,
                                                 ulonglong2* twl, const u64* sreg = nullptr)
 {
+    static_assert(!BLK || (S1 == 8 && SREG), "row-tile blocks: the multi-modulus column kernels at N = 2^16");
     constexpr int R = 1 << S1;
     constexpr int CT = 4096 / R;
     constexpr int NSA = S1 - 4;
@@ -497,7 +526,7 @@
     const FC fc = make_fc(md.q, FP_SITE(DECOMP ? FPS_FWD_COL_DECOMP : FPS_FWD_COL, S1 - 4));
     const ulonglong2* __restrict__ tw = a.tw + ((u64) ps.mod << a.n_power);
     const u64* __restrict__ src = a.in + ps.in_off + blockIdx.x * CT;
-    u64* __restrict__ dst = a.out + ps.out_off + blockIdx.x * CT;
+    u64* __restrict__ dst = a.out + ps.out_off + blockIdx.x * (BLK ? 256 : CT);
 
     double c32 = 0.0, c32i = 0.0;
     if constexpr (DECOMP && WIDE) {
@@ -574,7 +603,7 @@
     }
 #pragma unroll
     for (int k = 0; k < 16; k++) {
-        if constexpr (SREG) __builtin_nontemporal_store(as_bits(x[k]), &dst[(u64) (16 * r1 + k) * 256 + col]);
+        if constexpr (SREG) __builtin_nontemporal_store(as_bits(x[k]), &dst[col_out_pos<BLK>(r1, k, col)]);
         else dst[(u64) (16 * r1 + k) * 256 + col] = as_bits(x[k]);
     }
 }
@@ -1009,15 +1038,19 @@
     }
 }
 
-template <bool LAZY, int ROOM = 8, int EXIT = 0, bool PAIR = false>
+template <bool LAZY, int ROOM = 8, int EXIT = 0, bool PAIR = false, bool BLK = false>
 __device__ __forceinline__ void ks_row_digit(u64 (&x)[16], const u64* __restrict__ p, u64* lds,
                                              const ulonglong2* twa, const ulonglong2* __restrict__ tb,
                                              const QC& qc, const Mod& md, int row, int i0)
 {
     static_assert(EXIT == 0 || (!LAZY && (EXIT == 8 || ((EXIT == 12 || EXIT == 16) && ROOM == 16))), "exit bound");
     constexpr CsSched CS = cs_sched(8, ROOM, EXIT ? EXIT : 8);
-#pragma unroll
-    for (int k = 0; k < 16; k++) x[k] = gld(&p[row * 256 + i0 + 16 * k]);
+    if constexpr (BLK) {
+        blk_ld16<false>(x, p, row, i0);
+    } else {
+#pragma unroll
+        for (int k = 0; k < 16; k++) x[k] = gld(&p[row * 256 + i0 + 16 * k]);
+    }
 #pragma unroll
     for (int s = 0; s < 4; s++) {
         const int half = 8 >> s;
@@ -1161,7 +1194,7 @@
 }
 
 #define KS_TW_LDS_BYTES ((15 * 256 + 15 * 16) * 8)
-template <bool SPLIT, bool MD = false, bool PAIR = false>
+template <bool SPLIT, bool MD = false, bool PAIR = false, bool BLK = false>
 __device__ __forceinline__ void ks_row_mac_int_body(const KsMacArgs& a, const KsIdx& ki, const Mod& md, int midx,
                                                     u64* lds, void* twbuf)
 {
@@ -1205,15 +1238,15 @@
                 for (int k = 0; k < 16; k++) x[k] = gld(&pi[row * 256 + i0 + 16 * k]);
             }
         } else if (lazy) {
-            ks_row_digit<true, 8, 0, PAIR>(x, p, lds, twa, tb, qc, md, row, i0);
+            ks_row_digit<true, 8, 0, PAIR, BLK>(x, p, lds, twa, tb, qc, md, row, i0);
         } else if (room16) {
-            if (ex == 16) ks_row_digit<false, 16, 16, PAIR>(x, p, lds, twa, tb, qc, md, row, i0);
-            else if (ex == 12) ks_row_digit<false, 16, 12, PAIR>(x, p, lds, twa, tb, qc, md, row, i0);
-            else if (ex == 8) ks_row_digit<false, 16, 8, PAIR>(x, p, lds, twa, tb, qc, md, row, i0);
-            else ks_row_digit<false, 16, 0, PAIR>(x, p, lds, twa, tb, qc, md, row, i0);
+            if (ex == 16) ks_row_digit<false, 16, 16, PAIR, BLK>(x, p, lds, twa, tb, qc, md, row, i0);
+            else if (ex == 12) ks_row_digit<false, 16, 12, PAIR, BLK>(x, p, lds, twa, tb, qc, md, row, i0);
+            else if (ex == 8) ks_row_digit<false, 16, 8, PAIR, BLK>(x, p, lds, twa, tb, qc, md, row, i0);
+            else ks_row_digit<false, 16, 0, PAIR, BLK>(x, p, lds, twa, tb, qc, md, row, i0);
         } else {
-            if (ex) ks_row_digit<false, 8, 8, PAIR>(x, p, lds, twa, tb, qc, md, row, i0);
-            else ks_row_digit<false, 8, 0, PAIR>(x, p, lds, twa, tb, qc, md, row, i0);
+            if (ex) ks_row_digit<false, 8, 8, PAIR, BLK>(x, p, lds, twa, tb, qc, md, row, i0);
+            else ks_row_digit<false, 8, 0, PAIR, BLK>(x, p, lds, twa, tb, qc, md, row, i0);
         }
         const u64* k0 = pk + key_off2 * i;
         const u64* k1 = k0 + key_off1;
@@ -1254,13 +1287,13 @@
             const bool with_ct = ks_tail_ct<PAIR>(a, item_s, slot_s, p, e0, cv);
             const u64* pT = ks_tail_T(a, item_s, slot_s, tile_s, p);
             if (lazy_t) {
-                ks_row_digit<true, 8, 0, PAIR>(x, pT, lds, twa, ttb, qc, md, trow, ti0);
+                ks_row_digit<true, 8, 0, PAIR, BLK>(x, pT, lds, twa, ttb, qc, md, trow, ti0);
 #pragma unroll
                 for (int k = 0; k < 16; k++) x[k] = reduce64(x[k], md);
             } else if (room16) {
-                ks_row_digit<false, 16, 0, PAIR>(x, pT, lds, twa, ttb, qc, md, trow, ti0);
+                ks_row_digit<false, 16, 0, PAIR, BLK>(x, pT, lds, twa, ttb, qc, md, trow, ti0);
             } else {
-                ks_row_digit<false, 8, 0, PAIR>(x, pT, lds, twa, ttb, qc, md, trow, ti0);
+                ks_row_digit<false, 8, 0, PAIR, BLK>(x, pT, lds, twa, ttb, qc, md, trow, ti0);
             }
             ks_tail_store<PAIR>(a, item_s, slot_s, p, e0, md, inv, acc, x, with_ct, cv);
         };
@@ -1433,7 +1466,7 @@
     wave_lds_fence();
 }
 
-template <bool SPLIT, bool MD = false, bool PAIR = false>
+template <bool SPLIT, bool MD = false, bool PAIR = false, bool BLK = false>
 __device__ __forceinline__ void ks_row_mac_fp_body(const KsMacArgs& a, const KsIdx& ki, const Mod& md, int midx,
                                                    u64* lds, void* twbuf)
 {
@@ -1474,6 +1507,8 @@
         u64 xr[16];
         if (PAIR && ident) {
             ks_ld16<PAIR, true>(xr, px + row * 256 + 2 * i0);
+        } else if (BLK && !ident) {
+            blk_ld16<true>(xr, p, row, i0);
         } else {
 #pragma unroll
             for (int k = 0; k < 16; k++) {
@@ -1536,8 +1571,12 @@
         auto part = [&](int p, const double (&acc)[16]) {
             const u64* pT = ks_tail_T(a, item_s, slot_s, tile_s, p);
             u64 tr[16], cv[16];
-#pragma unroll
-            for (int k = 0; k < 16; k++) tr[k] = __builtin_nontemporal_load(&pT[trow * 256 + ti0 + 16 * k]);
+            if constexpr (BLK) {
+                blk_ld16<true>(tr, pT, trow, ti0);
+            } else {
+#pragma unroll
+                for (int k = 0; k < 16; k++) tr[k] = __builtin_nontemporal_load(&pT[trow * 256 + ti0 + 16 * k]);
+            }
             const bool with_ct = ks_tail_ct<PAIR>(a, item_s, slot_s, p, e0, cv);
             double x[16];
             ks_fp_row<false, PAIR>(x, tr, twl, lds, fc, s1, trow, ti0, tt);
@@ -1637,6 +1676,31 @@
     ks_row_mac_int_body<false, MD, true>(a, ki, md, midx, lds, twa);
 }
 
+template <bool MD, bool PAIR>
+__global__ __launch_bounds__(NTT_THREADS, 2) void ks_blk_mac_fp(KsMacArgs a)
+{
+    __shared__ __attribute__((aligned(16))) u64 lds[ROW_LDS_ELEMS];
+    __shared__ double twl[15 * 256 + 15 * 16];
+    const KsIdx ki = ks_index<false, 2>(a);
+    if (!ki.valid) return;
+    const int midx = a.mod_order ? a.mod_order[ki.slot] : ki.slot;
+    const Mod md = a.mods[midx];
+    if (!md.fp) return;
+    ks_row_mac_fp_body<false, MD, PAIR, true>(a, ki, md, midx, lds, twl);
+}
+template <bool MD, bool PAIR>
+__global__ __launch_bounds__(NTT_THREADS, 2) void ks_blk_mac(KsMacArgs a)
+{
+    __shared__ __attribute__((aligned(16))) u64 lds[ROW_LDS_ELEMS];
+    __shared__ ulonglong2 twa[15 * 16];
+    const KsIdx ki = ks_index<false, 1>(a);
+    if (!ki.valid) return;
+    const int midx = a.mod_order ? a.mod_order[ki.slot] : ki.slot;
+    const Mod md = a.mods[midx];
+    if (md.fp) return;
+    ks_row_mac_int_body<false, MD, PAIR, true>(a, ki, md, midx, lds, twa);
+}
+
 __global__ __launch_bounds__(NTT_THREADS, 2) void ks_row_mac_split(KsMacArgs a)
 {
     __shared__ __attribute__((aligned(16))) u64 lds[ROW_LDS_ELEMS];
@@ -1660,6 +1724,7 @@
     if (a.digits > 64 || items <= 0) return hipErrorInvalidValue;
     if (a.splits > 1 && a.digits < 2 * a.splits) return hipErrorInvalidValue;
     if (a.tail.on && (a.splits > 1 || !a.tail.out || !a.tail.T || !a.tail.inv)) return hipErrorInvalidValue;
+    if (a.blocks && (a.splits > 1 || a.n_power != 16)) return hipErrorInvalidValue;
     if (a.slot_first < 0 || a.slot_count < 0 || a.slot_first + (a.slot_count ? a.slot_count : a.rc) > a.rc)
         return hipErrorInvalidValue;
     KsMacArgs k = a;
@@ -1675,6 +1740,26 @@
     g_ks_forms[a.splits > 1 ? 2 : wide ? 1 : 0].fetch_add(1, std::memory_order_relaxed);
     if (a.splits > 1) {
         hipLaunchKernelGGL(ks_row_mac_split, grid_of(0), dim3(NTT_THREADS), 0, st, k);
+    } else if (a.blocks) {
+        const bool md = a.tail.on != 0;
+        if (!a.no_fp && ks_slots(k, 2) > 0) {
+            if (wide) {
+                if (md) hipLaunchKernelGGL((ks_blk_mac_fp<true, true>), grid_of(2), dim3(NTT_THREADS), 0, st, k);
+                else hipLaunchKernelGGL((ks_blk_mac_fp<false, true>), grid_of(2), dim3(NTT_THREADS), 0, st, k);
+            } else {
+                if (md) hipLaunchKernelGGL((ks_blk_mac_fp<true, false>), grid_of(2), dim3(NTT_THREADS), 0, st, k);
+                else hipLaunchKernelGGL((ks_blk_mac_fp<false, false>), grid_of(2), dim3(NTT_THREADS), 0, st, k);
+            }
+        }
+        if (!a.no_int && ks_slots(k, 1) > 0) {
+            if (wide) {
+                if (md) hipLaunchKernelGGL((ks_blk_mac<true, true>), grid_of(1), dim3(NTT_THREADS), 0, st, k);
+                else hipLaunchKernelGGL((ks_blk_mac<false, true>), grid_of(1), dim3(NTT_THREADS), 0, st, k);
+            } else {
+                if (md) hipLaunchKernelGGL((ks_blk_mac<true, false>), grid_of(1), dim3(NTT_THREADS), 0, st, k);
+                else hipLaunchKernelGGL((ks_blk_mac<false, false>), grid_of(1), dim3(NTT_THREADS), 0, st, k);
+            }
+        }
     } else if (wide) {
         if (!a.no_fp && ks_slots(k, 2) > 0) {
             if (a.tail.on) hipLaunchKernelGGL(ks_pair_mac_fp<true>, grid_of(2), dim3(NTT_THREADS), 0, st, k);
@@ -2111,7 +2196,7 @@
     else inv_single_body<S1, EPI, TENSOR>(ArInt(md), a, ps, limb);
 }
 
-template <int S1, bool ALL>
+template <int S1, bool ALL, bool BLK = false>
 __device__ __forceinline__ void fwd_col_multi_body(const NttArgs& a, u64* lds, ulonglong2* twl)
 {
     constexpr int R = 1 << S1;
@@ -2175,8 +2260,8 @@
         if (!md.fp) continue;
         ulonglong2* tl = twl + ((S1 > 4) ? 256 * (done & 1) : 0);
         done++;
-        if (wide) fwd_col_body_fp<S1, true, true, true>(a, ps, md, lds, tl, sreg);
-        else fwd_col_body_fp<S1, true, false, true>(a, ps, md, lds, tl, sreg);
+        if (wide) fwd_col_body_fp<S1, true, true, true, BLK>(a, ps, md, lds, tl, sreg);
+        else fwd_col_body_fp<S1, true, false, true, BLK>(a, ps, md, lds, tl, sreg);
     }
     if constexpr (ALL) {
         if (!wide) {
@@ -2189,9 +2274,9 @@
             const Mod md = ld_const_mod(a.mods + ps.mod);
             ulonglong2* tl = twl + 256 * (done & 1);
             done++;
-            if (fwd_stages_lazy(md, a.lazy_q_max)) fwd_col_body<S1, true, true, true>(a, ps, md, lds, sreg, tl);
-            else if (stages_room16(md)) fwd_col_body<S1, true, false, true, 16>(a, ps, md, lds, sreg, tl);
-            else fwd_col_body<S1, true, false, true>(a, ps, md, lds, sreg, tl);
+            if (fwd_stages_lazy(md, a.lazy_q_max)) fwd_col_body<S1, true, true, true, 8, BLK>(a, ps, md, lds, sreg, tl);
+            else if (stages_room16(md)) fwd_col_body<S1, true, false, true, 16, BLK>(a, ps, md, lds, sreg, tl);
+            else fwd_col_body<S1, true, false, true, 8, BLK>(a, ps, md, lds, sreg, tl);
         }
     }
 }
@@ -2210,6 +2295,19 @@
     __shared__ u64 lds[COL_LDS_ELEMS];
     __shared__ ulonglong2 twl[512];
     fwd_col_multi_body<S1, true>(a, lds, twl);
+}
+
+__global__ __launch_bounds__(NTT_THREADS) void ntt_fwd_col_blk_multi(NttArgs a)
+{
+    __shared__ u64 lds[COL_LDS_ELEMS];
+    __shared__ ulonglong2 twl[512];
+    fwd_col_multi_body<8, false, true>(a, lds, twl);
+}
+__global__ __launch_bounds__(NTT_THREADS) void ntt_fwd_col_blk_all(NttArgs a)
+{
+    __shared__ u64 lds[COL_LDS_ELEMS];
+    __shared__ ulonglong2 twl[512];
+    fwd_col_multi_body<8, true, true>(a, lds, twl);
 }
 
 template <int S1>
@@ -2228,7 +2326,14 @@
     constexpr int CT = 4096 >> S1;
     if constexpr (S1 == 8) {
         if (a.plan_has_fp && a.plan_has_int && a.int_slot_count > 0 && a.int_slot_count <= 8) {
-            hipLaunchKernelGGL((ntt_fwd_col_decomp_all<S1>), dim3(256 / CT, batch / a.decomp_mods), dim3(NTT_THREADS), 0, st, a);
+            if (a.out_blocks)
+                hipLaunchKernelGGL(ntt_fwd_col_blk_all, dim3(256 / CT, batch / a.decomp_mods), dim3(NTT_THREADS), 0, st, a);
+            else
+                hipLaunchKernelGGL((ntt_fwd_col_decomp_all<S1>), dim3(256 / CT, batch / a.decomp_mods), dim3(NTT_THREADS), 0, st, a);
+            return;
+        }
+        if (a.out_blocks) {
+            hipLaunchKernelGGL(ntt_fwd_col_blk_multi, dim3(256 / CT, batch / a.decomp_mods), dim3(NTT_THREADS), 0, st, a);
             return;
         }
     }
@@ -2367,6 +2472,13 @@
     return false;
 }
 
+bool ntt_decomp_all_multi(const NttArgs& a, int batch)
+{
+    if (a.n_power != 16 || !ntt_decomp_uses_multi(a, batch)) return false;
+    if (a.plan_has_int && a.int_slot_count > 0 && a.int_slot_count <= 8) return true;
+    return !a.plan_has_int || a.int_slot_count < 0;
+}
+
 hipError_t ntt_launch_inv_rows(const NttArgs& a, int batch, hipStream_t st)
 {
     if (batch <= 0) return hipSuccess;
@@ -2397,6 +2509,7 @@
     if (batch <= 0) return hipSuccess;
     if (a.n_power < 12 || a.n_power > 16 || batch > 65535 || a.poly_order) return hipErrorInvalidValue;
     if (a.src_inv && !ntt_decomp_uses_multi(a, batch)) return hipErrorInvalidValue;
+    if (a.out_blocks && !ntt_decomp_all_multi(a, batch)) return hipErrorInvalidValue;
     NttArgs g = a;
     g.group_span = 0;
     if (!a.decomp_mods && a.mod_count > 1 && batch % a.mod_count == 0 &&
@@ -2420,6 +2533,7 @@
     if (a.decomp_mods && (inverse || a.poly_order || !a.polys_per_item)) return hipErrorInvalidValue;
     if (a.src_inv && (!a.decomp_mods || batch > 65535 || !ntt_decomp_uses_multi(a, batch))) return hipErrorInvalidValue;
     if (a.copy_src && (!a.decomp_mods || inverse)) return hipErrorInvalidValue;
+    if (a.out_blocks) return hipErrorInvalidValue;
     if (a.tensor_in && (!inverse || a.poly_order || a.iepi.on || a.polys_per_item != 3 * a.tensor_limbs || batch % a.polys_per_item))
         return hipErrorInvalidValue;
     if (a.iepi.on && (!inverse || a.poly_order || batch % a.polys_per_item ||
diff --git a/heongpu_amd/csrc/ntt.hpp b/heongpu_amd/csrc/ntt.hpp
--- a/heongpu_amd/csrc/ntt.hpp
+++ b/heongpu_amd/csrc/ntt.hpp
@@ -65,6 +65,7 @@
     NttInvEpilogue iepi;
     int decomp_in_mul, decomp_in_add;
     int decomp_out_mul;
+    int out_blocks;
     int half_on, half_src_mod;
     u64 half;
     const u64* half_mod;
@@ -89,6 +90,7 @@
 
 hipError_t ntt_launch(const NttArgs& a, int batch, bool inverse, hipStream_t st);
 bool ntt_decomp_uses_multi(const NttArgs& a, int batch);
+bool ntt_decomp_all_multi(const NttArgs& a, int batch);
 hipError_t ntt_launch_inv_rows(const NttArgs& a, int batch, hipStream_t st);
 hipError_t ntt_launch_fwd_col(const NttArgs& a, int batch, hipStream_t st);
 
@@ -116,6 +118,7 @@
     int slot_first, slot_count;
     int unreduced_exit;
     int wide;
+    int blocks;
     struct Tail {
         int on;
         const u64* T;
diff --git a/heongpu_amd/csrc/ops.cpp b/heongpu_amd/csrc/ops.cpp
--- a/heongpu_amd/csrc/ops.cpp
+++ b/heongpu_amd/csrc/ops.cpp
@@ -74,10 +74,16 @@
     return bits;
 }
 
+static bool ks_region_blocked(const Context& c, const NttArgs& a, int batch, int splits)
+{
+    return c.digit_blocks && c.scheme == SCHEME_CKKS && c.P_size == 1 && c.n_power == 16 && splits <= 1 &&
+           a.decomp_mods > 0 && ntt_decomp_all_multi(a, batch);
+}
+
 static hipError_t keyswitch_ntt_mac(const Context& c, NttArgs a, const u64* key, u64* acc, u64 acc_stride,
                                     int digits, int rc, int split, int level, const u64* ident, u64 ident_stride,
                                     int batch, hipStream_t st, int which = 3, int slot_first = 0, int slot_count = 0,
-                                    const KsMacArgs::Tail* tail = nullptr)
+                                    const KsMacArgs::Tail* tail = nullptr, int blocks = -1)
 {
     const int ppi = digits * rc;
     const int skip_identity = ident ? 1 : 0;
@@ -99,6 +105,9 @@
         NttArgs ca = a;
         ca.in = a.in + (u64) b0 * a.in_item_stride;
         ca.out = a.out + (u64) b0 * a.out_item_stride;
+        const bool blk = blocks < 0 ? ks_region_blocked(c, ca, ppi * nb, splits) : blocks != 0;
+        if (tail && blocks < 0) return hipErrorInvalidValue;
+        ca.out_blocks = blk ? 1 : 0;
         if (which & 1) TRY(ntt_launch_fwd_col(ca, ppi * nb, st));
         if (!(which & 2)) continue;
         KsMacArgs k{};
@@ -109,6 +118,7 @@
         k.ident = ident ? ident + (u64) b0 * ident_stride : nullptr; k.ident_item_stride = ident_stride;
         k.splits = splits;
         k.wide = c.wide_access && splits <= 1;
+        k.blocks = blk ? 1 : 0;
         k.no_fp = !a.plan_has_fp;
         k.no_int = !a.plan_has_int || a.int_slot_count < 0;
         k.int_slot_count = a.int_slot_count > 0 ? a.int_slot_count : 0;
@@ -263,20 +273,23 @@
     a = dgt;
     const int which = ((phases & RELIN_PHASE_COLUMN) ? 1 : 0) | ((phases & RELIN_PHASE_ROW_MAC) ? 2 : 0);
     const bool in_mac = use_moddown_in_mac(c, key, l, rc, batch);
-    if (which)
-        TRY(keyswitch_ntt_mac(c, a, key, temp2, per, l, rc, l, depth, src, src_stride, batch, st, which, in_mac ? l : 0,
-                              in_mac ? 1 : 0));
-    const NttArgs dgt_args = a;
-    a = c.ntt_args(0);
-    a.in = temp2; a.out = temp2; a.mod_count = 1; a.mod_offset = Q; a.polys_per_item = 2;
-    a.in_item_stride = a.out_item_stride = per;
-    a.poly_order = c.tab.new_input_locations + 2 * depth;
     NttArgs md = c.ntt_args(0);
     md.in = temp2; md.out = temp1; md.mod_count = l; md.polys_per_item = 2 * l;
     md.in_item_stride = md.out_item_stride = per;
     md.decomp_mods = l; md.decomp_in_mul = l + 1; md.decomp_in_add = l;
     md.half_on = 1; md.half_src_mod = Q;
     fill_int_slots(c, md, nullptr);
+    const int blocks = !in_mac ? -1
+                       : ((long) l * rc * batch <= 65535 && ks_region_blocked(c, dgt, l * rc * batch, 0) &&
+                          ks_region_blocked(c, md, 2 * l * batch, 0)) ? 1 : 0;
+    if (which)
+        TRY(keyswitch_ntt_mac(c, a, key, temp2, per, l, rc, l, depth, src, src_stride, batch, st, which, in_mac ? l : 0,
+                              in_mac ? 1 : 0, nullptr, blocks));
+    const NttArgs dgt_args = a;
+    a = c.ntt_args(0);
+    a.in = temp2; a.out = temp2; a.mod_count = 1; a.mod_offset = Q; a.polys_per_item = 2;
+    a.in_item_stride = a.out_item_stride = per;
+    a.poly_order = c.tab.new_input_locations + 2 * depth;
     const bool fuse_inv_p = c.fused_moddown && c.fuse_inverse && (long) 2 * l * batch <= 65535 &&
                             ntt_decomp_uses_multi(md, 2 * l * batch);
     if (phases & RELIN_PHASE_INTT_P) {
@@ -289,6 +302,7 @@
             a.out = temp2; a.decomp_out_mul = l + 1;
             a.half = c.hv.half; a.half_mod = c.tab.half_mod;
             a.src_inv = fuse_inv_p ? 1 : 0;
+            a.out_blocks = blocks;
             TRY(ntt_launch_fwd_col(a, 2 * l * batch, st));
         }
         if (!(phases & RELIN_PHASE_ROW_MAC)) return hipSuccess;
@@ -300,7 +314,8 @@
         t.inv = c.tab.last_q_modinv;
         t.limbs = l;
         t.galois_inv = galois_elt ? (unsigned) inv_mod_2n((u64) galois_elt, 2 * c.n) : 0u;
-        return keyswitch_ntt_mac(c, dgt_args, key, temp2, per, l, rc, l, depth, src, src_stride, batch, st, 2, 0, l, &t);
+        return keyswitch_ntt_mac(c, dgt_args, key, temp2, per, l, rc, l, depth, src, src_stride, batch, st, 2, 0, l, &t,
+                                 blocks);
     }
     if (!(phases & RELIN_PHASE_MODDOWN)) return hipSuccess;
     if (!c.fused_moddown)
```

Result: no change. 9150 (median of 2 runs) (+0.1%).
